# mario-linov/graphs4cfd

Hardware: AMD Instinct MI355X
Metric: rollout timesteps/s (100k-node 2D mesh) (higher is better)
Workload: dtype f32 (MLP products: two-way fp16 split of both operands, 22 significand bits each, 3 partial products on the f16 MFMA pipe, fp32 accumulate; error vs fp64 within that of an fp32 GEMM)

## Files before the change

graphs4cfd_amd/_lib.py:

```python
from __future__ import annotations

import ctypes as C
import os
from typing import Optional

import torch

_HERE = os.path.dirname(os.path.abspath(__file__))
LIB_PATH = os.environ.get("G4C_LIB_PATH") or os.path.join(_HERE, "lib", "libg4c.so")

OK, EINVAL, ELAUNCH, EUNSUPPORTED = 0, -1, -2, -3
ACT_NONE, ACT_SELU, ACT_TANH = 0, 1, 2
MAX_SRC, MAX_LAYERS = 4, 4
MAX_HEADS = 2
NARROW_MAX = 8
KERNEL_MLP_RS = 5
KERNEL_MLP_RS2 = 6
KERNEL_MLP_BX6, KERNEL_MLP_WS = 2, 4
KERNEL_MLP_BX6_CERT, KERNEL_MLP_WS_CERT = 7, 8
KERNEL_MLP_WS_PRE = 9
KERNEL_NAMES = {0: "none", 1: "mlp_split_kernel", 2: "mlp_bx6_kernel", 3: "mlp_bx6i_kernel", 4: "mlp_ws_kernel", 5: "mlp_rs1_kernel", 6: "mlp_rs2_kernel",
                7: "mlp_bx6_kernel", 8: "mlp_ws_kernel", 9: "mlp_ws_kernel"}

TILE_SHAPE_GENERIC, TILE_SHAPE_NODE, TILE_SHAPE_UP, TILE_SHAPE_DOWN = 0, 1, 2, 3

_ACT_CODES = {None: ACT_NONE, "none": ACT_NONE, "selu": ACT_SELU, "tanh": ACT_TANH}


def act_code(activation) -> Optional[int]:
    if activation is None or isinstance(activation, str):
        return _ACT_CODES[activation]
    if activation is torch.tanh or activation is torch.nn.functional.tanh:
        return ACT_TANH
    if activation is torch.nn.functional.selu or activation is torch.selu:
        return ACT_SELU
    return None


class g4c_src_t(C.Structure):
    _fields_ = [("ptr", C.c_void_p), ("idx", C.c_void_p), ("width", C.c_int32), ("ld", C.c_int32),
                ("col0", C.c_int32), ("pre_act", C.c_int32), ("additive", C.c_int32), ("seg_mean", C.c_int32),
                ("w", C.c_void_p), ("seg_off", C.c_void_p), ("seg_perm", C.c_void_p), ("dtype", C.c_int32)]


class g4c_mlp_t(C.Structure):
    _fields_ = [("n_layers", C.c_int32), ("k_pad", C.c_int32 * MAX_LAYERS), ("n_pad", C.c_int32 * MAX_LAYERS),
                ("w", C.c_void_p * MAX_LAYERS), ("b", C.c_void_p * MAX_LAYERS),
                ("ln_gamma", C.c_void_p), ("ln_beta", C.c_void_p), ("ln_eps", C.c_float), ("n_out", C.c_int32), ("w_format", C.c_int32),
                ("range_slot", C.c_int32), ("range_certified", C.c_int32)]


WFMT_FP32, WFMT_F16X2, WFMT_BF16X3, WFMT_BF16_RS, WFMT_BF16_RS2, WFMT_BF16_RS2N, WFMT_BF16 = 0, 1, 2, 3, 4, 5, 6
DTYPE_F32, DTYPE_BF16 = 0, 1


class g4c_mlp_io_t(C.Structure):
    _fields_ = [("size", C.c_int32), ("act", C.c_int32), ("row_begin", C.c_int64), ("row_count", C.c_int64),
                ("out", C.c_void_p), ("out_ld", C.c_int32), ("out_dtype", C.c_int32), ("out_idx", C.c_void_p),
                ("resid", C.c_void_p), ("resid_ld", C.c_int32), ("resid_col0", C.c_int32),
                ("n_heads", C.c_int32), ("head_ld", C.c_int32), ("head_dtype", C.c_int32), ("head_out", C.c_void_p * MAX_HEADS),
                ("tile_rows", C.c_void_p), ("tile_seg", C.c_void_p), ("seg_off", C.c_void_p), ("n_tiles", C.c_int32),
                ("agg", C.c_void_p), ("agg_ld", C.c_int32), ("agg_mode", C.c_int32),
                ("n_save", C.c_int32), ("save", C.c_void_p * MAX_LAYERS), ("save_ld", C.c_int32),
                ("mul", C.c_void_p * MAX_LAYERS), ("mul_ld", C.c_int32),
                ("upd", C.POINTER(g4c_mlp_t)), ("v", C.c_void_p), ("v_ld", C.c_int32), ("v_act", C.c_int32),
                ("v_out", C.c_void_p), ("v_out_ld", C.c_int32), ("range_flag", C.c_void_p),
                ("save_dtype", C.c_int32), ("mul_dtype", C.c_int32)]

    def __init__(self, **kw):
        super().__init__(size=C.sizeof(g4c_mlp_io_t), **kw)


REC_SQ_ERR, REC_ABS_ERR, REC_MAX_ABS_ERR, REC_TGT_SUM, REC_TGT_SQ_SUM, REC_ABS_ERR_MASK, REC_NSTAT = range(7)
REC_MAX_NF = 8


class g4c_rollout_rec_t(C.Structure):
    _fields_ = [("max_steps", C.c_int32), ("snap", C.c_void_p), ("every", C.c_int32), ("n_snap", C.c_int32),
                ("probe_rows", C.c_void_p), ("n_probe", C.c_int32), ("probe_out", C.c_void_p),
                ("target", C.c_void_p), ("target_ld", C.c_int32), ("mask", C.c_void_p), ("stats", C.c_void_p),
                ("scratch", C.c_void_p)]


class g4c_rollout_moments_t(C.Structure):
    _fields_ = [("max_steps", C.c_int32), ("stride", C.c_int32), ("window", C.c_void_p), ("sub", C.c_void_p), ("sub_ld", C.c_int32),
                ("plane_ld", C.c_int64), ("pivot", C.c_void_p), ("sum", C.c_void_p), ("sum2", C.c_void_p), ("lo", C.c_void_p),
                ("hi", C.c_void_p)]


SPECTRUM_MAX_BINS = 64


class g4c_rollout_spectrum_t(C.Structure):
    _fields_ = [("max_steps", C.c_int32), ("stride", C.c_int32), ("n_samples", C.c_int32), ("n_bins", C.c_int32), ("window", C.c_void_p),
                ("tw", C.c_void_p), ("x_ld", C.c_int32), ("x_step", C.c_int32), ("plane_ld", C.c_int64), ("pivot", C.c_void_p),
                ("sum", C.c_void_p), ("re", C.c_void_p), ("im", C.c_void_p)]


DERIVED_MAX_COLS, DERIVED_MAX_TERMS = 8, 3
DERIVED_SQ, DERIVED_ABS, DERIVED_MAX_ABS, DERIVED_NSTAT = range(4)


class g4c_derived_program_t(C.Structure):
    _fields_ = [("nd", C.c_int32), ("n_terms", C.c_int32 * DERIVED_MAX_COLS),
                ("field", (C.c_int32 * DERIVED_MAX_TERMS) * DERIVED_MAX_COLS), ("axis", (C.c_int32 * DERIVED_MAX_TERMS) * DERIVED_MAX_COLS),
                ("coef", (C.c_float * DERIVED_MAX_TERMS) * DERIVED_MAX_COLS)]


class g4c_mesh_derived_t(C.Structure):
    _fields_ = [("dim", C.c_int32), ("nf", C.c_int32), ("x_ld", C.c_int32), ("g", C.c_void_p), ("src", C.c_void_p), ("off", C.c_void_p),
                ("cur", C.c_void_p), ("step", C.c_void_p), ("every", C.c_int32), ("n_snap", C.c_int32), ("max_steps", C.c_int32),
                ("snap", C.c_void_p), ("stats", C.c_void_p), ("scratch", C.c_void_p)]


_SIGNATURES = {
    "g4c_version": (C.c_int, []),
    "g4c_device_info": (C.c_int, [C.c_void_p, C.POINTER(C.c_int32), C.POINTER(C.c_int32)]),
    "g4c_last_error": (C.c_char_p, []),
    "g4c_plan_csr": (C.c_int, [C.c_void_p, C.c_int64, C.c_int64, C.c_void_p, C.c_void_p]),
    "g4c_plan_pool_edge": (C.c_int64, [C.c_void_p, C.c_int64, C.c_void_p, C.c_int64, C.c_void_p, C.c_void_p,
                                       C.c_void_p, C.c_void_p]),
    "g4c_plan_pool_edge_ordered": (C.c_int64, [C.c_void_p, C.c_int64, C.c_void_p, C.c_int64, C.c_int32, C.c_void_p, C.c_void_p,
                                               C.c_void_p, C.c_void_p]),
    "g4c_segment_reduce": (C.c_int, [C.c_void_p, C.c_int32, C.c_void_p, C.c_void_p, C.c_int32, C.c_int32, C.c_int32,
                                     C.c_int32, C.c_int32, C.c_void_p, C.c_int32, C.c_void_p]),
    "g4c_weighted_segment_mean": (C.c_int, [C.c_void_p, C.c_int32, C.c_void_p, C.c_void_p, C.c_void_p, C.c_int32,
                                            C.c_int32, C.c_void_p, C.c_int32, C.c_void_p, C.c_void_p]),
    "g4c_mlp_pack_layer": (C.c_int, [C.c_void_p, C.c_int32, C.c_int32, C.c_void_p, C.c_void_p, C.c_int32, C.c_int32, C.c_void_p,
                                     C.c_int32, C.c_int32, C.c_void_p]),
    "g4c_mlp_run": (C.c_int, [C.POINTER(g4c_mlp_t), C.POINTER(g4c_src_t), C.c_int32, C.c_int64, C.POINTER(g4c_mlp_io_t), C.c_void_p]),
    "g4c_plan_tiles": (C.c_int64, [C.c_void_p, C.c_int32, C.c_int32, C.c_void_p, C.c_void_p, C.c_int64]),
    "g4c_mlp_bx6i_enable": (C.c_int, [C.c_int]),
    "g4c_mlp_ws_enable": (C.c_int, [C.c_int]),
    "g4c_mlp_small_launch_tiles": (C.c_int, [C.c_int]),
    "g4c_layer_norm": (C.c_int, [C.c_void_p, C.c_int32, C.c_int64, C.c_int32, C.c_void_p, C.c_void_p, C.c_float, C.c_int32, C.c_void_p, C.c_int32, C.c_void_p]),
    "g4c_debug_mean_div": (C.c_int, [C.c_void_p, C.c_void_p, C.c_void_p, C.c_int64, C.c_void_p]),
    "g4c_mlp_last_kernel": (C.c_int, []),
    "g4c_mlp_shapes_enable": (C.c_int, [C.c_int]),
    "g4c_mlp_last_shape": (C.c_int, []),
    "g4c_project_to_edges": (C.c_int, [C.c_void_p, C.c_int32, C.c_void_p, C.c_void_p, C.c_int64, C.c_int32,
                                       C.c_void_p, C.c_int32, C.c_void_p]),
    "g4c_edge_scalar_to_node_vector": (C.c_int, [C.c_void_p, C.c_int32, C.c_void_p, C.c_int32, C.c_int64, C.c_int32,
                                                 C.c_void_p, C.c_int32, C.c_void_p]),
    "g4c_knn_grid": (C.c_int, [C.c_void_p, C.c_void_p, C.c_void_p, C.c_void_p, C.c_int64, C.c_int32, C.c_void_p,
                               C.c_void_p, C.c_float, C.c_int32, C.c_void_p, C.c_void_p]),
    "g4c_knn_grid_query": (C.c_int, [C.c_void_p, C.c_void_p, C.c_void_p, C.c_int64, C.c_int32, C.c_void_p, C.c_void_p,
                                     C.c_float, C.c_void_p, C.c_void_p, C.c_int64, C.c_int32, C.c_void_p, C.c_void_p]),
    "g4c_rollout_advance": (C.c_int, [C.c_void_p, C.c_int32, C.c_void_p, C.c_int32, C.c_void_p, C.c_int32,
                                      C.c_void_p, C.c_int64, C.c_void_p]),
    "g4c_rollout_record_scratch_doubles": (C.c_int64, [C.c_int64, C.c_int32]),
    "g4c_rollout_advance_record": (C.c_int, [C.c_void_p, C.c_int32, C.c_void_p, C.c_int32, C.POINTER(g4c_rollout_rec_t),
                                             C.c_void_p, C.c_int64, C.c_void_p]),
    "g4c_rollout_moments": (C.c_int, [C.c_void_p, C.c_int32, C.POINTER(g4c_rollout_moments_t), C.c_void_p, C.c_int64, C.c_void_p]),
    "g4c_rollout_spectrum": (C.c_int, [C.c_void_p, C.c_int32, C.POINTER(g4c_rollout_spectrum_t), C.c_void_p, C.c_int64, C.c_void_p]),
    "g4c_mesh_gradient_weights": (C.c_int, [C.c_void_p, C.c_void_p, C.c_void_p, C.c_void_p, C.c_int32, C.c_int32, C.c_int64, C.c_int64,
                                            C.c_void_p, C.c_void_p, C.c_void_p, C.c_void_p]),
    "g4c_mesh_derived_scratch_doubles": (C.c_int64, [C.c_int64, C.c_int32]),
    "g4c_mesh_derived": (C.c_int, [C.c_void_p, C.POINTER(g4c_mesh_derived_t), C.POINTER(g4c_derived_program_t), C.c_int64, C.c_void_p]),
    "g4c_activation_inplace": (C.c_int, [C.c_void_p, C.c_int64, C.c_int32, C.c_void_p]),
    "g4c_add_cols": (C.c_int, [C.c_void_p, C.c_int32, C.c_int32, C.c_void_p, C.c_int32, C.c_void_p, C.c_int32,
                               C.c_int32, C.c_int64, C.c_void_p]),
    "g4c_copy_cols": (C.c_int, [C.c_void_p, C.c_int32, C.c_int32, C.c_void_p, C.c_void_p, C.c_int32, C.c_int32,
                                C.c_int32, C.c_int64, C.c_void_p]),
    "g4c_train_gather": (C.c_int, [C.c_void_p, C.c_int32, C.c_int32, C.c_void_p, C.c_int32, C.c_int32, C.c_void_p, C.c_int32,
                                   C.c_int32, C.c_int32, C.c_int64, C.c_int32, C.c_void_p]),
    "g4c_act_grad": (C.c_int, [C.c_void_p, C.c_int32, C.c_void_p, C.c_int32, C.c_int32, C.c_int32, C.c_void_p, C.c_int32,
                               C.c_int32, C.c_int64, C.c_void_p]),
    "g4c_act_grad_ref16": (C.c_int, [C.c_void_p, C.c_int32, C.c_void_p, C.c_int32, C.c_int32, C.c_int32, C.c_void_p, C.c_int32,
                                     C.c_int32, C.c_int64, C.c_void_p]),
    "g4c_layernorm_grad_partials": (C.c_int32, [C.c_int64]),
    "g4c_layernorm_grad": (C.c_int, [C.c_void_p, C.c_int32, C.c_void_p, C.c_void_p, C.c_int32, C.c_void_p, C.c_int32,
                                     C.c_void_p, C.c_int32, C.c_int64, C.c_float, C.c_void_p]),
    "g4c_layernorm_grad_z16": (C.c_int, [C.c_void_p, C.c_int32, C.c_void_p, C.c_void_p, C.c_int32, C.c_void_p, C.c_int32,
                                         C.c_void_p, C.c_int32, C.c_int64, C.c_float, C.c_void_p]),
    "g4c_colsum_partials": (C.c_int32, [C.c_int64]),
    "g4c_colsum": (C.c_int, [C.c_void_p, C.c_int32, C.c_int32, C.c_int64, C.c_void_p, C.c_void_p, C.c_void_p]),
    "g4c_weight_grad_partials": (C.c_int32, [C.c_int64]),
    "g4c_weight_grad_scratch_floats": (C.c_int64, [C.c_int64]),
    "g4c_weight_grad": (C.c_int, [C.c_void_p, C.c_int32, C.c_void_p, C.c_int32, C.c_int64, C.c_void_p, C.c_void_p, C.c_int32,
                                  C.c_void_p]),
    "g4c_weight_grad_bf16": (C.c_int, [C.c_void_p, C.c_int32, C.c_void_p, C.c_int32, C.c_int64, C.c_void_p, C.c_void_p, C.c_int32,
                                       C.c_void_p]),
    "g4c_weight_grad_bf16_a16": (C.c_int, [C.c_void_p, C.c_int32, C.c_void_p, C.c_int32, C.c_int64, C.c_void_p, C.c_void_p, C.c_int32,
                                           C.c_void_p]),
    "g4c_segment_broadcast": (C.c_int, [C.c_void_p, C.c_int32, C.c_void_p, C.c_void_p, C.c_int32, C.c_int32, C.c_int32,
                                        C.c_void_p, C.c_int32, C.c_void_p]),
}

EXPORTED_SYMBOLS = tuple(_SIGNATURES)

_lib = None


def load() -> C.CDLL:
    global _lib
    if _lib is None:
        if not os.path.exists(LIB_PATH):
            raise RuntimeError(
                f"graphs4cfd_amd: HIP library not found at {LIB_PATH}. Build it with "
                "`python -c 'import __graft_entry__ as g; g.build()'` (hipcc --offload-arch=gfx950). "
                "There is no CPU fallback.")
        lib = C.CDLL(LIB_PATH)
        for name, (res, args) in _SIGNATURES.items():
            fn = getattr(lib, name)
            fn.restype, fn.argtypes = res, args
        _lib = lib
    return _lib


def check(code: int) -> None:
    if code == OK:
        return
    msg = load().g4c_last_error().decode("utf-8", "replace")
    if code == EINVAL:
        raise ValueError(msg)
    if code == EUNSUPPORTED:
        raise NotImplementedError(msg)
    raise RuntimeError(msg)


# ... 22 lines not shown
```

graphs4cfd_amd/csrc/error.cpp:

```cpp
#include "g4c_common.h"
#include <atomic>

namespace g4c {
static thread_local char g_err[512] = "";

void set_error(const char *fmt, ...) {
    va_list ap;
    va_start(ap, fmt);
    vsnprintf(g_err, sizeof(g_err), fmt, ap);
    va_end(ap);
}

int visible_devices() {
    static const int n = [] {
        int c = 0;
        if (hipGetDeviceCount(&c) != hipSuccess) { (void)hipGetLastError(); c = 0; }
        return c;
    }();
    return n;
}

int cu_count() {
    constexpr int MAXD = 64;
    static std::atomic<int> cached[MAXD];
    int dev = 0;
    if (hipGetDevice(&dev) != hipSuccess) { (void)hipGetLastError(); return 256; }
    int n = (dev >= 0 && dev < MAXD) ? cached[dev].load(std::memory_order_relaxed) : 0;
    if (n > 0) return n;
    if (hipDeviceGetAttribute(&n, hipDeviceAttributeMultiprocessorCount, dev) != hipSuccess || n <= 0) { (void)hipGetLastError(); n = 256; }
    if (dev >= 0 && dev < MAXD) cached[dev].store(n, std::memory_order_relaxed);
    return n;
}
}

extern "C" int g4c_version(void) { return 3; }
extern "C" int g4c_device_info(const void *device_ptr, int32_t *device, int32_t *cu_count) {
    G4C_REQUIRE(device_ptr && device && cu_count, G4C_EINVAL, "g4c_device_info: null pointer");
    g4c::DeviceGuard on_device(device_ptr);
    int dev = -1;
    if (hipGetDevice(&dev) != hipSuccess) { (void)hipGetLastError(); g4c::set_error("g4c_device_info: hipGetDevice failed"); return G4C_ELAUNCH; }
    *device = dev;
    *cu_count = g4c::cu_count();
    return G4C_OK;
}
extern "C" const char *g4c_last_error(void) { return g4c::g_err; }
```

graphs4cfd_amd/csrc/g4c_common.h:

```cpp
#pragma once
#include <hip/hip_runtime.h>
#include <cstdarg>
#include <cstdio>
#include <cstdint>

#include "../../include/g4c.h"

namespace g4c {

void set_error(const char *fmt, ...);

inline int check_launch(const char *what) {
    hipError_t e = hipGetLastError();
    if (e != hipSuccess) {
        set_error("%s: %s", what, hipGetErrorString(e));
        return G4C_ELAUNCH;
    }
    return G4C_OK;
}

int visible_devices();
int cu_count();
struct DeviceGuard {
    int prev = -1;
    explicit DeviceGuard(const void *device_ptr) {
        if (visible_devices() <= 1 || !device_ptr) return;
        hipPointerAttribute_t attr;
        int cur = 0;
        if (hipPointerGetAttributes(&attr, device_ptr) != hipSuccess || hipGetDevice(&cur) != hipSuccess) {
            (void)hipGetLastError();
            return;
        }
        if (attr.device != cur && hipSetDevice(attr.device) == hipSuccess) prev = cur;
    }
    ~DeviceGuard() {
        if (prev >= 0) (void)hipSetDevice(prev);
    }
    DeviceGuard(const DeviceGuard &) = delete;
    DeviceGuard &operator=(const DeviceGuard &) = delete;
};

#define G4C_REQUIRE(cond, code, ...)      \
    do {                                  \
        if (!(cond)) {                    \
            g4c::set_error(__VA_ARGS__);  \
            return (code);                \
        }                                 \
    } while (0)

constexpr int MEAN_DIV_MAX_COUNT = 4096;
typedef float mean_f32x4 __attribute__((ext_vector_type(4)));
__device__ __forceinline__ mean_f32x4 mean_div4(mean_f32x4 a, int count) {
    const float c = (float)count;
    const float y0 = __builtin_amdgcn_rcpf(c);
    const float y = fmaf(fmaf(-c, y0, 1.f), y0, y0);
    mean_f32x4 q;
    bool rare = count > MEAN_DIV_MAX_COUNT;
#pragma unroll
    for (int e = 0; e < 4; ++e) {
        const float q0 = a[e] * y;
        q[e] = fmaf(fmaf(-c, q0, a[e]), y, q0);
        rare |= (__builtin_bit_cast(unsigned, a[e]) != 0u) && !(fabsf(q[e]) >= 0x1p-100f);
    }
    if (__builtin_amdgcn_ballot_w64(rare) != 0ull) {
#pragma unroll
        for (int e = 0; e < 4; ++e) q[e] = a[e] / c;
    }
    return q;
}

__device__ __forceinline__ float selu_f(float x) {
    const float alpha = 1.6732632423543772848170429916717f;
    const float scale = 1.0507009873554804934193349852946f;
    const float e = __builtin_amdgcn_fmed3f(__builtin_amdgcn_exp2f(x * 1.4426950408889634f), 0.f, 1.f);
    return fmaf(fmaxf(x, 0.f), scale, fmaf(scale * alpha, e, -scale * alpha));
}

__device__ __forceinline__ float tanh_f(float x) {
    const float ax = fminf(fabsf(x), 20.f);
    const float t = __builtin_amdgcn_exp2f(ax * 2.8853900817779268f);
    const float r = 1.f - 2.f * __builtin_amdgcn_rcpf(t + 1.f);
    return copysignf(r, x);
}

__device__ __forceinline__ float apply_act(float x, int act) {
    const float s = selu_f(x), t = tanh_f(x);
    return act == G4C_ACT_SELU ? s : (act == G4C_ACT_TANH ? t : x);
}

template <int ACT>
__device__ __forceinline__ float act_t(float x) {
    if (ACT == G4C_ACT_SELU) return selu_f(x);
    if (ACT == G4C_ACT_TANH) return tanh_f(x);
    return x;
}

}
```

graphs4cfd_amd/csrc/mlp_common.h:

```cpp
#pragma once
#include "g4c_common.h"
#include <type_traits>

#ifndef G4C_ABLATE
#define G4C_ABLATE 0
#endif

namespace g4cm {

constexpr int KC = 32;
constexpr int XS = KC + 2;
constexpr int HS = 128 + 4;
constexpr int NP = 128;
constexpr int CHUNK_FLOATS = KC * NP;

typedef float f32x16 __attribute__((ext_vector_type(16)));
typedef float f32x8 __attribute__((ext_vector_type(8)));
typedef float f32x4 __attribute__((ext_vector_type(4)));
typedef float f32x2 __attribute__((ext_vector_type(2)));

struct Src {
    const float *ptr;
    const int *idx;
    int width, wpad, ld, col0, vec, pre_act;
    const int *seg_off;
    int seg_mean;
    const int *seg_perm;
    int bf16;
};

struct NarSrc {
    const float *ptr;
    const float *w;
    int width, ld;
};

struct AddSrc {
    const float *ptr;
    const int *idx;
    int width, ld;
    int bf16;
};

struct Params {
    Src src[G4C_MAX_SRC];
    int n_src;
    AddSrc add[G4C_MAX_SRC];
    int n_add;
    int n_layers;
    int chunks0;
    const float *w;
    const float *b;
    const float *gamma, *beta;
    float eps;
    int n_out;
    long long M;
    float *out;
    int out_ld;
    int out_bf16;
    const int *out_idx;
    int act;
    const float *resid;
    int resid_ld, resid_col0;
    int n_tiles;
    long long row_base;
    int n_heads;
    float *head_out[G4C_MAX_HEADS];
    int head_ld;
    int head_bf16;
    const int *tile_rows, *tile_seg, *seg_off;
    float *agg;
    int agg_ld, agg_mean;
    int agg_deg;
    int agg_bf16;
    NarSrc nar[G4C_MAX_SRC];
    int n_nar;
    float *save[G4C_MAX_LAYERS];
    int save_ld;
    int save_bf16;
    const float *mul[G4C_MAX_LAYERS];
    int mul_ld;
    int mul_bf16;
    int *range_flag;
    int range_slot;
    int range_certified;
};

struct TileShapeGeneric {
    static constexpr int ID = G4C_TILE_SHAPE_GENERIC;
};
template <int ID_, int NS, bool IDX0_, int NNAR, int NL, int NH>
struct TileShape {
    static constexpr int ID = ID_, N_SRC = NS, N_NAR = NNAR, N_LAYERS = NL, N_HEADS = NH;
    static constexpr bool IDX0 = IDX0_;
    static_assert(ID_ != G4C_TILE_SHAPE_GENERIC && NS >= 1 && NS <= 2 && (NL == 2 || NL == 3) && (NH == 0 || NH == 2), "tile shape out of range");
};
template <int NL, int NH> using TileShapeNode = TileShape<G4C_TILE_SHAPE_NODE, 2, false, 0, NL, NH>;
template <int NL, int NH> using TileShapeUp = TileShape<G4C_TILE_SHAPE_UP, 2, true, 1, NL, NH>;
template <int NL> using TileShapeDown = TileShape<G4C_TILE_SHAPE_DOWN, 1, false, 1, NL, 0>;

struct NodeParams {
    const float *v;
    int v_ld;
    const float *w;
    const float *b;
    const float *gamma, *beta;
    float eps;
    int act;
    float *out;
    int out_ld;
    int n_heads;
    float *head_out[G4C_MAX_HEADS];
    int head_ld;
    int *range_flag;
    int range_slot;
};

typedef __bf16 bf16x8 __attribute__((ext_vector_type(8)));
typedef __bf16 bf16x4 __attribute__((ext_vector_type(4)));
constexpr int HB = 128 + 8;
constexpr int STEP6 = 3 * 512;
constexpr int BLOCK6 = 4 * 8 * STEP6;

typedef unsigned u32x4 __attribute__((ext_vector_type(4)));
__device__ __forceinline__ bf16x8 ldw(__amdgpu_buffer_rsrc_t rs, unsigned voff_bytes, unsigned soff_bytes) {
    const u32x4 v = __builtin_amdgcn_raw_buffer_load_b128(rs, voff_bytes, soff_bytes, 0);
    return __builtin_bit_cast(bf16x8, v);
}

__device__ __forceinline__ f32x4 selu4(f32x4 x) {
    f32x4 y;
#pragma unroll
    for (int e = 0; e < 4; ++e) y[e] = g4c::selu_f(x[e]);
    return y;
}
__device__ __forceinline__ f32x2 selu2(f32x2 x) {
    f32x2 y;
    y[0] = g4c::selu_f(x[0]); y[1] = g4c::selu_f(x[1]);
    return y;
}

typedef __bf16 bf16x2 __attribute__((ext_vector_type(2)));
__device__ __forceinline__ unsigned pack_bf16(f32x2 x, f32x2 &back) {
    bf16x2 b;
    b[0] = (__bf16)x[0]; b[1] = (__bf16)x[1];
    const unsigned u = __builtin_bit_cast(unsigned, b);
    back[0] = __builtin_bit_cast(float, u << 16);
    back[1] = __builtin_bit_cast(float, u & 0xffff0000u);
    return u;
}
typedef _Float16 f16x8 __attribute__((ext_vector_type(8)));
typedef _Float16 f16x2 __attribute__((ext_vector_type(2)));
constexpr float F16_LO_SCALE = 2048.f, F16_LO_UNSCALE = 1.f / 2048.f;
__device__ __forceinline__ f32x16 mfma_f16(bf16x8 a, bf16x8 b, f32x16 c) {
    return __builtin_amdgcn_mfma_f32_32x32x16_f16(__builtin_bit_cast(f16x8, a), __builtin_bit_cast(f16x8, b), c, 0, 0, 0);
}
#ifndef G4C_F16_SATURATE
// ... 44 lines not shown
        const float c = -F16_LO_SCALE;
        asm("v_fma_mixlo_f16 %0, %1, %2, %3 op_sel_hi:[1,0,0]" : "=v"(lu) : "v"(hu), "s"(c), "v"(ys[0]));
        asm("v_fma_mixhi_f16 %0, %1, %2, %3 op_sel:[1,0,0] op_sel_hi:[1,0,0]" : "+v"(lu) : "v"(hu), "s"(c), "v"(ys[1]));
    } else {
        f32x2 hf, lf;
        hf[0] = (float)b[0]; hf[1] = (float)b[1];
        lu = pack_f16((y - hf) * F16_LO_SCALE, lf);
    }
}
template <class R>
__device__ __forceinline__ void split_pair_f16(f32x2 y, unsigned &hu, unsigned &lu, R &rng) {
    range_track(rng, y);
    split_pair_f16(y, hu, lu);
}
template <class R>
__device__ __forceinline__ void split2x4(f32x4 x, bf16x4 &h, bf16x4 &l, R &rng) {
    range_track(rng, x);
    unsigned hu[2], lu[2];
#pragma unroll
    for (int j = 0; j < 2; ++j) {
        f32x2 v;
        v[0] = x[2 * j]; v[1] = x[2 * j + 1];
        split_pair_f16(v, hu[j], lu[j]);
    }
    typedef unsigned u32x2 __attribute__((ext_vector_type(2)));
    u32x2 hh, ll;
    hh[0] = hu[0]; hh[1] = hu[1]; ll[0] = lu[0]; ll[1] = lu[1];
    h = __builtin_bit_cast(bf16x4, hh); l = __builtin_bit_cast(bf16x4, ll);
}
__device__ __forceinline__ void split2(float x, __bf16 &h, __bf16 &l) {
    const _Float16 a = (_Float16)x;
    const _Float16 b = (_Float16)((x - (float)a) * F16_LO_SCALE);
    h = __builtin_bit_cast(__bf16, a); l = __builtin_bit_cast(__bf16, b);
}

template <int SP, class R> __device__ __forceinline__ void split3x4(f32x4 x, bf16x4 &h, bf16x4 &m, bf16x4 &l, R &rng);
template <int SP = 3>
__device__ __forceinline__ void split3x4(f32x4 x, bf16x4 &h, bf16x4 &m, bf16x4 &l) { RangeNone none; split3x4<SP>(x, h, m, l, none); }
template <int SP, class R>
__device__ __forceinline__ void split3x4(f32x4 x, bf16x4 &h, bf16x4 &m, bf16x4 &l, R &rng) {
    if (SP == 2) { split2x4(x, h, m, rng); l = m; return; }
    if (SP == 1 || (G4C_ABLATE & 512)) {
#pragma unroll
        for (int e = 0; e < 4; ++e) { h[e] = (__bf16)x[e]; m[e] = h[e]; l[e] = h[e]; }
        return;
    }
    unsigned hu[2], mu[2], lu[2];
#pragma unroll
    for (int j = 0; j < 2; ++j) {
        f32x2 v, hf, mf, lf;
        v[0] = x[2 * j]; v[1] = x[2 * j + 1];
        hu[j] = pack_bf16(v, hf);
        const f32x2 r1 = v - hf;
        mu[j] = pack_bf16(r1, mf);
        const f32x2 r2 = r1 - mf;
        lu[j] = pack_bf16(r2, lf);
    }
    typedef unsigned u32x2 __attribute__((ext_vector_type(2)));
    u32x2 hh, mm, ll;
    hh[0] = hu[0]; hh[1] = hu[1]; mm[0] = mu[0]; mm[1] = mu[1]; ll[0] = lu[0]; ll[1] = lu[1];
    h = __builtin_bit_cast(bf16x4, hh); m = __builtin_bit_cast(bf16x4, mm); l = __builtin_bit_cast(bf16x4, ll);
}

__device__ __forceinline__ void split3(float x, __bf16 &h, __bf16 &m, __bf16 &l) {
    h = (__bf16)x;
    const float r1 = x - (float)h;
    m = (__bf16)r1;
    l = (__bf16)(r1 - (float)m);
}

struct Launch {
    Params p;
    NodeParams node;
    bool has_node;
    int fmt;
    bool round1, f16x2, bx6, row_split;
    bool agg, save;
    bool pre;
    bool all_vec;
    long long row_begin, row_count;
    int io_n_tiles;
    bool deep_ring, shapes;
};
struct Ran { int kernel = G4C_KERNEL_NONE, shape = G4C_TILE_SHAPE_GENERIC; };

inline bool message_form(const Launch &L) {
    const Params &p = L.p;
    const Src &s = p.src[0];
    if (L.save || p.n_src != 1 || p.n_nar != 0 || (p.n_add != 0 && p.n_add != 2) || p.n_heads || p.n_out != NP || p.resid) return false;
    if (p.out_idx && (L.agg || !p.out)) return false;
    if (s.width != NP || !s.vec || s.seg_off) return false;
    for (int a = 0; a < p.n_add; ++a)
        if (p.add[a].width != NP || (p.add[a].ld & 3) || ((uintptr_t)p.add[a].ptr & (p.add[a].bf16 ? 7 : 15))) return false;
    if (p.out && !p.out_bf16 && ((p.out_ld & 3) || ((uintptr_t)p.out & 15))) return false;
    if (p.gamma && (((uintptr_t)p.gamma & 15) || ((uintptr_t)p.beta & 15))) return false;
    return ((uintptr_t)p.b & 15) == 0 && p.M < (1LL << 31);
}

bool split_takes(const Launch &L);
int split_launch(const Launch &L, hipStream_t st, Ran &ran);
bool tile_takes(const Launch &L);
int tile_launch(const Launch &L, hipStream_t st, Ran &ran);
bool bx6i_takes(const Launch &L);
int bx6i_launch(const Launch &L, hipStream_t st, Ran &ran);
bool ws_takes(const Launch &L);
bool ws_pre_takes(const Launch &L);
int ws_launch(const Launch &L, hipStream_t st, Ran &ran);
bool rs_takes(const Launch &L);
int rs_launch(const Launch &L, hipStream_t st, Ran &ran);
bool rs2_takes(const Launch &L);
int rs2_launch(const Launch &L, hipStream_t st, Ran &ran);

typedef unsigned u32x2 __attribute__((ext_vector_type(2)));
__device__ __forceinline__ f32x4 widen_bf16x4(u32x2 w) {
    f32x4 x;
    x[0] = __builtin_bit_cast(float, w[0] << 16); x[1] = __builtin_bit_cast(float, w[0] & 0xffff0000u);
    x[2] = __builtin_bit_cast(float, w[1] << 16); x[3] = __builtin_bit_cast(float, w[1] & 0xffff0000u);
    return x;
}


}
```

graphs4cfd_amd/csrc/mlp_run.hip:

```cpp
#include "mlp_common.h"
#include <atomic>
#include <climits>
using namespace g4cm;

namespace {

std::atomic<int> g_ws_mode{1};
std::atomic<int> g_bx6i_mode{1};
std::atomic<int> g_deep_tiles{512};
#ifndef G4C_TILE_SHAPES_DEFAULT
#define G4C_TILE_SHAPES_DEFAULT 1
#endif
std::atomic<int> g_shapes{G4C_TILE_SHAPES_DEFAULT};

constexpr long long WS_MIN_ROWS = 20000;
constexpr long long BX6I_MIN_ROWS = 400000;

int knob(std::atomic<int> &k, int value, int max_value) {
    const int prev = k.load(std::memory_order_relaxed);
    if (value >= 0) k.store(value > max_value ? max_value : value, std::memory_order_relaxed);
    return prev;
}

thread_local Ran g_last;

int stage_call(const g4c_mlp_t *mlp, const g4c_src_t *srcs, int32_t n_src, int64_t n_rows, const g4c_mlp_io_t *io, Launch &L) {
    G4C_REQUIRE(io && io->size == (int32_t)sizeof(g4c_mlp_io_t), G4C_EINVAL,
                "g4c_mlp_run: io->size %d, this library's g4c_mlp_io_t has %d bytes (a binding out of step with g4c.h)", io ? io->size : 0,
                (int)sizeof(g4c_mlp_io_t));
    G4C_REQUIRE(mlp && srcs, G4C_EINVAL, "g4c_mlp_run: null pointer");
    const int fmt = L.fmt = mlp->w_format;
    G4C_REQUIRE(fmt >= G4C_WFMT_FP32 && fmt <= G4C_WFMT_BF16, G4C_EINVAL, "g4c_mlp_run: unknown w_format %d", fmt);
    L.row_split = fmt == G4C_WFMT_BF16_RS || fmt == G4C_WFMT_BF16_RS2 || fmt == G4C_WFMT_BF16_RS2N;
    L.round1 = fmt == G4C_WFMT_BF16 || L.row_split;
    L.f16x2 = fmt == G4C_WFMT_F16X2;
    L.bx6 = fmt != G4C_WFMT_FP32;
    L.agg = io->agg != nullptr; L.save = io->n_save != 0; L.has_node = io->upd != nullptr;
    L.row_begin = io->row_begin; L.row_count = io->row_count; L.io_n_tiles = io->n_tiles;
    G4C_REQUIRE(L.row_begin >= 0 && L.row_count >= 0 && L.row_begin + L.row_count <= n_rows && L.row_begin % 32 == 0, G4C_EINVAL,
                "g4c_mlp_run: bad row range [%lld, +%lld) of %lld (row_begin must be a multiple of 32)", L.row_begin, L.row_count,
                (long long)n_rows);
    G4C_REQUIRE(n_src >= 1 && n_src <= G4C_MAX_SRC, G4C_EUNSUPPORTED, "g4c_mlp_run: %d sources (max %d)", n_src, G4C_MAX_SRC);
    G4C_REQUIRE(mlp->n_layers >= 1 && mlp->n_layers <= G4C_MAX_LAYERS, G4C_EUNSUPPORTED,
                "g4c_mlp_run: %d layers (supported 1..%d)", mlp->n_layers, G4C_MAX_LAYERS);
    G4C_REQUIRE(n_rows >= 0 && n_rows < (1LL << 31), G4C_EINVAL, "g4c_mlp_run: n_rows %lld out of range", (long long)n_rows);
    G4C_REQUIRE(io->act >= 0 && io->act <= 2, G4C_EINVAL, "g4c_mlp_run: bad activation %d", io->act);
    G4C_REQUIRE(io->n_heads >= 0 && io->n_heads <= G4C_MAX_HEADS, G4C_EINVAL, "g4c_mlp_run: bad heads (n=%d)", io->n_heads);
    G4C_REQUIRE((L.row_begin == 0 && L.row_count == n_rows) || (!L.agg && !L.save && !L.has_node && !io->n_heads && !io->out_dtype),
                G4C_EUNSUPPORTED, "g4c_mlp_run: a row sub-range needs a plain launch (no heads / aggregation / save / upd / out_dtype)");
    G4C_REQUIRE(!L.agg || (io->tile_rows && io->tile_seg && io->seg_off && io->n_tiles >= 0 && io->agg_ld >= NP), G4C_EINVAL,
                "g4c_mlp_run: bad aggregation plan");
    G4C_REQUIRE(io->out_dtype == G4C_DTYPE_F32 || io->out_dtype == G4C_DTYPE_BF16 || io->out_dtype == G4C_DTYPE_BF16_SELU, G4C_EINVAL,
                "g4c_mlp_run: unknown out_dtype %d", io->out_dtype);
    G4C_REQUIRE(io->out_dtype != G4C_DTYPE_BF16_SELU || (L.agg && io->act == G4C_ACT_NONE), G4C_EINVAL,
                "g4c_mlp_run: G4C_DTYPE_BF16_SELU needs the fused aggregation and no output activation");
    G4C_REQUIRE(io->head_dtype == G4C_DTYPE_F32 || io->head_dtype == G4C_DTYPE_BF16, G4C_EINVAL, "g4c_mlp_run: unknown head_dtype %d", io->head_dtype);
    G4C_REQUIRE(!io->range_flag || (mlp->range_slot >= 0 && (!L.has_node || io->upd->range_slot >= 0)), G4C_EINVAL,
                "g4c_mlp_run: negative range_slot (mlp %d, upd %d)", mlp->range_slot, L.has_node ? io->upd->range_slot : 0);
    return G4C_OK;
}

int stage_sources(const g4c_src_t *srcs, int32_t n_src, int32_t k_pad0, Launch &L) {
    Params &p = L.p;
    const bool bx6 = L.bx6, round1 = L.round1;
    int kp = 0, nk = 0;
    L.all_vec = true;
    for (int s = 0; s < n_src; ++s) {
        const g4c_src_t &g = srcs[s];
        G4C_REQUIRE(g.ptr && g.width > 0 && g.ld >= g.col0 + g.width && g.col0 >= 0, G4C_EINVAL,
                    "g4c_mlp_run: bad source %d (width=%d ld=%d col0=%d)", s, g.width, g.ld, g.col0);
        if (g.additive == 2) {
            G4C_REQUIRE(bx6, G4C_EUNSUPPORTED, "g4c_mlp_run: narrow sources (additive == 2) need a split-operand w_format");
            G4C_REQUIRE(g.width <= G4C_NARROW_MAX && !g.idx && g.pre_act == G4C_ACT_NONE && g.w && ((uintptr_t)g.w & 15) == 0, G4C_EINVAL,
                        "g4c_mlp_run: bad narrow source %d (width %d <= %d, no index, no pre_act, 16-byte aligned weights)", s,
                        g.width, G4C_NARROW_MAX);
            NarSrc &a = p.nar[p.n_nar++];
            a.ptr = g.ptr + g.col0; a.w = g.w; a.width = g.width; a.ld = g.ld;
            continue;
        }
        if (g.additive) {
            G4C_REQUIRE(g.pre_act == G4C_ACT_NONE && g.width <= NP && (g.dtype == G4C_DTYPE_F32 || g.dtype == G4C_DTYPE_BF16), G4C_EINVAL,
                        "g4c_mlp_run: bad additive source %d", s);
            AddSrc &a = p.add[p.n_add++];
            a.idx = g.idx; a.width = g.width; a.ld = g.ld; a.bf16 = g.dtype == G4C_DTYPE_BF16;
            if (a.bf16) {
                G4C_REQUIRE(round1 && g.width == NP && g.ld % 4 == 0 && g.col0 % 4 == 0 && (uintptr_t)g.ptr % 8 == 0, G4C_EUNSUPPORTED,
                            "g4c_mlp_run: bf16 additive rows need the rounded-bf16 mode (w_format G4C_WFMT_BF16*) and a 128-wide, 8-byte aligned block");
                a.ptr = reinterpret_cast<const float *>(reinterpret_cast<const __bf16 *>(g.ptr) + g.col0);
            } else {
                a.ptr = g.ptr + g.col0;
            }
            continue;
        }
        G4C_REQUIRE(g.pre_act == G4C_ACT_NONE || g.pre_act == G4C_ACT_SELU, G4C_EUNSUPPORTED,
                    "g4c_mlp_run: source %d pre_act %d (only NONE / SELU can be applied on load)", s, g.pre_act);
        Src &d = p.src[nk++];
        if (bx6) G4C_REQUIRE(g.width <= NP, G4C_EUNSUPPORTED, "g4c_mlp_run: input block %d is %d wide (max 128 in a split-operand w_format)", s, g.width);
        d.ptr = g.ptr; d.idx = g.idx; d.width = g.width; d.wpad = bx6 ? NP : (g.width + KC - 1) / KC * KC; d.ld = g.ld; d.col0 = g.col0;
        d.pre_act = g.pre_act;
        d.bf16 = g.dtype == G4C_DTYPE_BF16;
        if (d.bf16)
            G4C_REQUIRE(round1 && g.width == NP && !g.seg_off && g.ld % 4 == 0 && g.col0 % 4 == 0 && (uintptr_t)g.ptr % 8 == 0, G4C_EUNSUPPORTED,
                        "g4c_mlp_run: bf16 rows need the rounded-bf16 mode (w_format G4C_WFMT_BF16*) and a 128-wide, 8-byte aligned block");
        else
            G4C_REQUIRE(g.dtype == G4C_DTYPE_F32, G4C_EINVAL, "g4c_mlp_run: source %d has unknown dtype %d", s, g.dtype);
        d.seg_off = g.seg_off; d.seg_mean = g.seg_mean; d.seg_perm = g.seg_off ? g.seg_perm : nullptr;
        if (g.seg_off)
            G4C_REQUIRE(bx6 && !g.idx && g.width == NP && g.ld % 4 == 0 && g.col0 % 4 == 0 && (uintptr_t)g.ptr % 16 == 0, G4C_EUNSUPPORTED,
                        "g4c_mlp_run: aggregation on load needs a split-operand w_format and a 128-wide aligned block without gather index");
        d.vec = (g.width % 4 == 0) && (g.ld % 4 == 0) && (g.col0 % 4 == 0) && ((uintptr_t)g.ptr % (d.bf16 ? 8 : 16) == 0);
        L.all_vec = L.all_vec && d.vec;
        kp += d.wpad;
    }
    L.pre = nk == 0 && p.n_nar == 0 && p.n_add >= 1;
    G4C_REQUIRE(nk >= 1 || p.n_nar >= 1 || L.pre, G4C_EINVAL, "g4c_mlp_run: no input block goes through the weights");
    p.n_src = nk;
    if (nk == 0) p.src[0] = Src{nullptr, nullptr, 0, 0, 0, 0, 1, 0, nullptr, 0, nullptr, 0};
    for (int s = (nk ? nk : 1); s < G4C_MAX_SRC; ++s) p.src[s] = p.src[0];
    G4C_REQUIRE(kp == k_pad0, G4C_EINVAL, "g4c_mlp_run: sources give %d padded columns, layer 1 packed for %d", kp, k_pad0);
    p.chunks0 = kp / KC;
    return G4C_OK;
}

int check_contiguous(const g4c_mlp_t *m, int wbytes, const char *w_text, const char *b_text) {
    for (int l = 1; l < m->n_layers; ++l) {
        G4C_REQUIRE((const char *)m->w[l] == (const char *)m->w[l - 1] + (size_t)m->k_pad[l - 1] * NP * wbytes, G4C_EINVAL, w_text, l);
        G4C_REQUIRE((const float *)m->b[l] == (const float *)m->b[l - 1] + NP, G4C_EINVAL, b_text, l);
    }
    return G4C_OK;
}

int stage_stream(const g4c_mlp_t *mlp, Launch &L) {
    Params &p = L.p;
    p.n_layers = mlp->n_layers;
    for (int l = 0; l < mlp->n_layers; ++l) {
        G4C_REQUIRE(mlp->n_pad[l] == NP, G4C_EINVAL, "g4c_mlp_run: layer %d n_pad %d (must be 128)", l, mlp->n_pad[l]);
        if (l > 0) G4C_REQUIRE(mlp->k_pad[l] == NP, G4C_EINVAL, "g4c_mlp_run: layer %d k_pad %d (must be 128)", l, mlp->k_pad[l]);
    }
    if (const int rc = check_contiguous(mlp, L.bx6 ? 6 : 4, "g4c_mlp_run: packed layers must be contiguous (layer %d)",
                                        "g4c_mlp_run: padded biases must be contiguous (layer %d)"))
        return rc;
    p.w = (const float *)mlp->w[0]; p.b = (const float *)mlp->b[0];
    G4C_REQUIRE(p.w && p.b, G4C_EINVAL, "g4c_mlp_run: null weights");
    p.gamma = mlp->ln_gamma; p.beta = mlp->ln_beta; p.eps = mlp->ln_eps;
    G4C_REQUIRE((p.gamma == nullptr) == (p.beta == nullptr), G4C_EINVAL, "g4c_mlp_run: LayerNorm needs both gamma and beta");
    p.n_out = mlp->n_out;
    return G4C_OK;
}

int stage_outputs(const g4c_mlp_io_t *io, Launch &L) {
    Params &p = L.p;
    p.out = (float *)io->out; p.out_ld = io->out_ld; p.out_idx = io->out_idx; p.act = io->act;
    G4C_REQUIRE(p.out || L.agg, G4C_EINVAL, "g4c_mlp_run: null output");
    G4C_REQUIRE(p.n_out > 0 && p.n_out <= NP && p.out_ld >= p.n_out, G4C_EINVAL, "g4c_mlp_run: n_out=%d out_ld=%d", p.n_out, p.out_ld);
    p.resid = io->resid; p.resid_ld = io->resid_ld; p.resid_col0 = io->resid_col0;
    p.row_base = L.row_begin;
    p.M = L.row_begin + L.row_count;
    if (L.agg) {
        G4C_REQUIRE(L.bx6 && p.n_out == NP && !p.out_idx && !p.resid, G4C_EUNSUPPORTED,
                    "g4c_mlp_run: the fused aggregation needs a split-operand w_format and a plain 128-wide output");
        const int32_t mode = io->agg_mode;
        p.tile_rows = io->tile_rows; p.tile_seg = io->tile_seg; p.seg_off = io->seg_off;
        p.agg = (float *)io->agg; p.agg_ld = io->agg_ld; p.agg_mean = mode & 1; p.agg_deg = (mode >> 8) & 0xff; p.agg_bf16 = (mode >> 16) & 1;
        const bool rs_fmt = L.fmt == G4C_WFMT_BF16_RS;
        G4C_REQUIRE((mode >> 17) == 0 && (!p.agg_bf16 || rs_fmt) && p.agg_deg <= 32 && (p.agg_deg == 0 || L.row_count % p.agg_deg == 0), G4C_EINVAL,
                    "fused aggregation: agg_mode = %d is not 0 / 1 [| G4C_AGG_UNIFORM(k), 1 <= k <= 32, k dividing the %lld rows]", mode,
                    L.row_count);
        G4C_REQUIRE(p.agg_deg == 0 || L.row_begin == 0, G4C_EINVAL,
                    "g4c_mlp_run: uniform segments (G4C_AGG_UNIFORM) need the whole row range, got rows [%lld, %lld)", L.row_begin, p.M);
    }
    if (io->out_dtype) {
        G4C_REQUIRE(L.round1 && !p.resid && !p.out_idx && p.n_out == NP && (!p.out || ((p.out_ld & 3) == 0 && ((uintptr_t)p.out & 7) == 0)), G4C_EUNSUPPORTED,
                    "g4c_mlp_run: bf16 output rows need the rounded-bf16 mode, a plain 128-wide output, out_ld a multiple of 4 and an 8-byte aligned out");
        p.out_bf16 = io->out_dtype;
    }
    return G4C_OK;
}

int stage_save(const g4c_mlp_io_t *io, Launch &L) {
    Params &p = L.p;
    const int n_layers = p.n_layers;
    if (!L.save) return G4C_OK;
    G4C_REQUIRE(L.bx6 && (!L.round1 || L.fmt == G4C_WFMT_BF16) && !io->out_dtype && !L.agg && !io->n_heads && !p.out_idx && io->save_ld >= NP &&
                    (io->save_ld & 3) == 0,
                G4C_EUNSUPPORTED,
                "g4c_mlp_run: save needs w_format BF16X3 / F16X2 / BF16 without heads / aggregation / output index / bf16 rows, save_ld >= 128 "
                "and a multiple of 4");
    G4C_REQUIRE(io->n_save == n_layers, G4C_EINVAL, "g4c_mlp_run: n_save %d for %d layers", io->n_save, n_layers);
    G4C_REQUIRE((io->save_dtype == G4C_DTYPE_F32 || io->save_dtype == G4C_DTYPE_BF16) &&
                    (io->mul_dtype == G4C_DTYPE_F32 || io->mul_dtype == G4C_DTYPE_BF16),
                G4C_EINVAL, "g4c_mlp_run: save_dtype %d / mul_dtype %d (G4C_DTYPE_F32 or G4C_DTYPE_BF16)", io->save_dtype, io->mul_dtype);
    G4C_REQUIRE((!io->save_dtype && !io->mul_dtype) || L.fmt == G4C_WFMT_BF16, G4C_EINVAL,
                "g4c_mlp_run: bf16 save / mul rows need w_format G4C_WFMT_BF16 (the plain rounded-bf16 stream); w_format %d keeps fp32 rows",
                L.fmt);
    bool mul = false;
    for (int l = 0; l < n_layers; ++l) {
        G4C_REQUIRE(((uintptr_t)io->save[l] & 15) == 0, G4C_EINVAL, "g4c_mlp_run: save[%d] is not 16-byte aligned", l);
        p.save[l] = static_cast<float *>(io->save[l]);
        if (l + 1 == n_layers) break;
        G4C_REQUIRE(((uintptr_t)io->mul[l] & 15) == 0, G4C_EINVAL, "g4c_mlp_run: mul[%d] is not 16-byte aligned", l);
        p.mul[l] = static_cast<const float *>(io->mul[l]);
        mul = mul || io->mul[l];
    }
    p.save_bf16 = io->save_dtype == G4C_DTYPE_BF16;
    p.mul_bf16 = io->mul_dtype == G4C_DTYPE_BF16;
    p.save_ld = io->save_ld;
    G4C_REQUIRE(!mul || (io->mul_ld >= NP && (io->mul_ld & 3) == 0), G4C_EINVAL, "g4c_mlp_run: mul_ld=%d", io->mul_ld);
    p.mul_ld = io->mul_ld;
    return G4C_OK;
}

void stage_range(const g4c_mlp_t *mlp, const g4c_mlp_io_t *io, Launch &L) {
    L.p.range_certified = (L.f16x2 && mlp->range_certified && !L.save && (!L.has_node || io->upd->range_certified)) ? 1 : 0;
    L.p.range_flag = (L.f16x2 && !L.p.range_certified) ? io->range_flag : nullptr;
    L.p.range_slot = mlp->range_slot;
}

int stage_heads(const g4c_mlp_io_t *io, Launch &L) {
    Params &p = L.p;
    const int n_heads = io->n_heads;
    for (int hd = 0; hd < n_heads; ++hd) G4C_REQUIRE(io->head_out[hd], G4C_EINVAL, "g4c_mlp_run: null head output %d", hd);
    if (L.has_node || !n_heads) return G4C_OK;
    p.n_heads = n_heads; p.head_ld = io->head_ld;
    for (int hd = 0; hd < n_heads; ++hd) p.head_out[hd] = (float *)io->head_out[hd];
    if (io->head_dtype) {
        G4C_REQUIRE(L.round1 && (p.head_ld & 1) == 0, G4C_EUNSUPPORTED, "g4c_mlp_run: bf16 head rows need the rounded-bf16 mode and an even head_ld");
        for (int hd = 0; hd < n_heads; ++hd)
            G4C_REQUIRE(((uintptr_t)io->head_out[hd] & 3) == 0, G4C_EINVAL, "g4c_mlp_run: head output %d is not 4-byte aligned", hd);
        p.head_bf16 = 1;
    }
    G4C_REQUIRE(!L.agg, G4C_EUNSUPPORTED, "g4c_mlp_run: heads with the fused aggregation");
    G4C_REQUIRE((p.head_ld & 3) == 0 || !L.bx6, G4C_EINVAL, "g4c_mlp_run: head outputs need a leading dimension that is a multiple of 4");
    G4C_REQUIRE(p.n_out == NP && !p.resid && !p.out_idx && p.head_ld >= NP, G4C_EINVAL,
                "g4c_mlp_run: heads need a 128-wide output without residual / output index (n_out=%d)", p.n_out);
    return G4C_OK;
}

int stage_node(const g4c_mlp_io_t *io, Launch &L) {
    if (!L.has_node) return G4C_OK;
    const g4c_mlp_t *u = io->upd;
    const int n_heads = io->n_heads;
    G4C_REQUIRE(L.f16x2 && L.agg && u->w_format == G4C_WFMT_F16X2 && io->act == G4C_ACT_NONE, G4C_EUNSUPPORTED,
                "g4c_mlp_run: the fused node update needs the f16x3 format (G4C_WFMT_F16X2) for both MLPs, the aggregation plan and act NONE");
    G4C_REQUIRE(u->n_layers == L.p.n_layers && u->k_pad[0] == 2 * NP && u->n_out == NP && u->w[0] && u->b[0], G4C_EUNSUPPORTED,
                "g4c_mlp_run: upd must have the message MLP's depth (%d), two 128-wide input blocks and a 128-wide output", L.p.n_layers);
    for (int l = 0; l < u->n_layers; ++l)
        G4C_REQUIRE(u->n_pad[l] == NP && (l == 0 || u->k_pad[l] == NP), G4C_EUNSUPPORTED, "g4c_mlp_run: upd layer %d is not 128 wide", l);
    const char *const text = "g4c_mlp_run: upd's packed layers / biases must be contiguous (layer %d)";
    if (const int rc = check_contiguous(u, 6, text, text)) return rc;
    G4C_REQUIRE((u->ln_gamma == nullptr) == (u->ln_beta == nullptr), G4C_EINVAL, "g4c_mlp_run: upd's LayerNorm needs both gamma and beta");
    G4C_REQUIRE(!u->ln_gamma || (((uintptr_t)u->ln_gamma & 15) == 0 && ((uintptr_t)u->ln_beta & 15) == 0), G4C_EINVAL,
                "g4c_mlp_run: upd's LayerNorm parameters must be 16-byte aligned");
    G4C_REQUIRE(io->v && io->v_out && (io->v_ld & 3) == 0 && io->v_ld >= NP && (io->v_out_ld & 3) == 0 && io->v_out_ld >= NP &&
                ((uintptr_t)io->v & 15) == 0 && ((uintptr_t)io->v_out & 15) == 0 && (io->agg_ld & 3) == 0 && ((uintptr_t)io->agg & 15) == 0,
                G4C_EINVAL, "g4c_mlp_run: v / v_out / agg need 16-byte aligned rows of at least 128 columns");
    G4C_REQUIRE(io->v_act >= 0 && io->v_act <= 2, G4C_EINVAL, "g4c_mlp_run: bad v_act %d", io->v_act);
    NodeParams &q = L.node;
    q.v = io->v; q.v_ld = io->v_ld; q.w = (const float *)u->w[0]; q.b = (const float *)u->b[0];
    q.gamma = u->ln_gamma; q.beta = u->ln_beta; q.eps = u->ln_eps; q.act = io->v_act;
    q.out = io->v_out; q.out_ld = io->v_out_ld; q.n_heads = n_heads; q.head_ld = io->head_ld;
    q.range_flag = L.p.range_certified ? nullptr : io->range_flag; q.range_slot = u->range_slot;
    if (n_heads) {
        G4C_REQUIRE(io->head_dtype == G4C_DTYPE_F32 && (io->head_ld & 3) == 0 && io->head_ld >= NP, G4C_EINVAL,
                    "g4c_mlp_run: upd's heads need fp32 rows, head_ld a multiple of 4 and >= 128");
        for (int hd = 0; hd < n_heads; ++hd) {
            G4C_REQUIRE(((uintptr_t)io->head_out[hd] & 15) == 0, G4C_EINVAL, "g4c_mlp_run: bad head output %d", hd);
            q.head_out[hd] = (float *)io->head_out[hd];
        }
    }
    return G4C_OK;
}

typedef int (*LaunchFn)(const Launch &, hipStream_t, Ran &);

bool at_size(const std::atomic<int> &mode_knob, long long min_rows, const Launch &L) {
    const int mode = mode_knob.load(std::memory_order_relaxed);
    return mode == 2 || (mode == 1 && L.row_count >= min_rows);
}

LaunchFn choose(Launch &L) {
    L.deep_ring = L.p.n_tiles <= g_deep_tiles.load(std::memory_order_relaxed);
    L.shapes = g_shapes.load(std::memory_order_relaxed) != 0;
    if (L.pre) {
        G4C_REQUIRE(!L.has_node, nullptr, "g4c_mlp_run: every source additive (first layer precomputed) with upd: the fused MP layer has no such form");
        G4C_REQUIRE(L.f16x2, nullptr, "g4c_mlp_run: every source additive (first layer precomputed) needs the f16x3 format (G4C_WFMT_F16X2), got w_format %d", L.fmt);
        G4C_REQUIRE(L.p.n_layers == 3, nullptr, "g4c_mlp_run: every source additive (first layer precomputed) needs three layers (two left), got %d", L.p.n_layers);
        G4C_REQUIRE(L.agg && !L.save, nullptr, "g4c_mlp_run: every source additive (first layer precomputed) needs the fused aggregation and no save");
        G4C_REQUIRE(ws_pre_takes(L), nullptr,
                    "g4c_mlp_run: every source additive (first layer precomputed) is outside the weight-stationary kernel's envelope (three aligned "
                    "128-wide fp32 additive blocks — the first direct, two through indices —, a plain fp32 128-wide output, no heads / residual "
                    "/ output index / out_dtype)");
        return ws_launch;
    }
    if (L.has_node) {
        G4C_REQUIRE(ws_takes(L), nullptr,
                    "g4c_mlp_run: the message launch of the fused MP layer is outside the weight-stationary kernel's envelope (one 128-wide "
                    "weighted block, two 128-wide additive blocks, two or three 128-wide layers, aligned rows)");
        return ws_launch;
    }
    if (L.fmt == G4C_WFMT_BF16_RS) {
        G4C_REQUIRE(!L.save && rs_takes(L), nullptr,
                    "g4c_mlp_run: weights packed for the row-split kernel (G4C_WFMT_BF16_RS), launch outside its envelope");
        return rs_launch;
    }
    if (L.row_split) {
        G4C_REQUIRE(!L.save && !L.agg && rs2_takes(L), nullptr,
                    "g4c_mlp_run: weights packed for the row-split update kernel (G4C_WFMT_BF16_RS2), launch outside its envelope");
        return rs2_launch;
    }
    if (at_size(g_ws_mode, WS_MIN_ROWS, L) && ws_takes(L)) return ws_launch;
    if (at_size(g_bx6i_mode, BX6I_MIN_ROWS, L) && bx6i_takes(L)) return bx6i_launch;
    return tile_takes(L) ? tile_launch : split_launch;
}

}

extern "C" int g4c_mlp_run(const g4c_mlp_t *mlp, const g4c_src_t *srcs, int32_t n_src, int64_t n_rows, const g4c_mlp_io_t *io,
                           void *stream) {
    g_last = Ran{};
    Launch L{};
    int rc;
    if ((rc = stage_call(mlp, srcs, n_src, n_rows, io, L))) return rc;
    if (n_rows == 0) return G4C_OK;
    g4c::DeviceGuard on_device(mlp->w[0]);
    if ((rc = stage_sources(srcs, n_src, mlp->k_pad[0], L))) return rc;
    if ((rc = stage_stream(mlp, L))) return rc;
    if ((rc = stage_outputs(io, L))) return rc;
    if ((rc = stage_save(io, L))) return rc;
    stage_range(mlp, io, L);
    if ((rc = stage_heads(io, L))) return rc;
    if (L.row_count == 0) return G4C_OK;
    if ((rc = stage_node(io, L))) return rc;
    L.p.n_tiles = (L.agg && !L.row_split) ? L.io_n_tiles : (int)((L.row_count + 31) / 32);
    const LaunchFn launch = choose(L);
    if (!launch) return G4C_EUNSUPPORTED;
    if (L.p.n_tiles == 0) return G4C_OK;
    return launch(L, (hipStream_t)stream, g_last);
}

extern "C" int g4c_mlp_ws_enable(int on) { return knob(g_ws_mode, on, 2); }
extern "C" int g4c_mlp_bx6i_enable(int on) { return knob(g_bx6i_mode, on, 2); }
extern "C" int g4c_mlp_small_launch_tiles(int n_tiles) { return knob(g_deep_tiles, n_tiles, INT_MAX); }
extern "C" int g4c_mlp_shapes_enable(int on) { return knob(g_shapes, on, 1); }
extern "C" int g4c_mlp_last_kernel(void) { return g_last.kernel; }
extern "C" int g4c_mlp_last_shape(void) { return g_last.shape; }
```

graphs4cfd_amd/csrc/mlp_ws.hip:

```cpp
#include "mlp_common.h"
#include <cstdlib>
using namespace g4cm;

#ifdef G4C_WS_TIMING
__device__ unsigned long long g4c_ws_stamps[256 * 32];
extern "C" int g4c_ws_read_stamps(unsigned long long *host, int n) {
    return (int)hipMemcpyFromSymbol(host, HIP_SYMBOL(g4c_ws_stamps), sizeof(unsigned long long) * n);
}
#define WS_STAMP(k) do { if (it == 1 && tid == 0 && blockIdx.x < 256) g4c_ws_stamps[blockIdx.x * 32 + (k)] = __builtin_readcyclecounter(); } while (0)
#define WS_STAMP_T(k) do { if (its == 1 && tid == 0 && blockIdx.x < 256) { asm volatile("s_waitcnt lgkmcnt(0)" ::: "memory"); g4c_ws_stamps[blockIdx.x * 32 + (k)] = __builtin_readcyclecounter(); } } while (0)
#define WS_STAMP_ONCE(k, v) do { if (tid == 0 && blockIdx.x < 256) g4c_ws_stamps[blockIdx.x * 32 + (k)] = (v); } while (0)
#else
#define WS_STAMP(k) do {} while (0)
#define WS_STAMP_T(k) do {} while (0)
#define WS_STAMP_ONCE(k, v) do {} while (0)
#endif

#ifndef G4C_WS_ABLATE
#define G4C_WS_ABLATE 0
#endif

namespace {

constexpr int PS = 128;
// ... 386 lines not shown
                    __syncthreads();
                    store_head(1, fB, r0 + 32, nB);
                } else {
                    other_all<SP, 3, false>(accB, accB1, va, oB, rngN);
                    __syncthreads();
                    store_head(0, fB, r0 + 32, nB);
                }
            }
            __syncthreads();
            continue;
        }
        other_all<SP, 2, false>(accA, accA1, ga, oA, rngN);
        other_all<SP, 2, false>(accA, accA1, va, oB, rngN);
        bias_n(accA, accA1, 0);
        __syncthreads();
        m_block<SP, 0>(paA, Wa, accA, accA1, accA, accA1, ga, oA, rngN);
        ld_block(Wa, 2);
        m_block<SP, 0>(paB, Wb, accA, accA1, accA, accA1, ga, oA, rngN);
        ld_block(Wb, 3);
        __syncthreads();
        other_all<SP, 1, false>(accA, accA1, ga, oA, rngN);
        bias_n(accA, accA1, 1);
        __syncthreads();
        m_block<SP, 0>(paA, Wa, accA, accA1, accA, accA1, ga, oA, rngN);
        if constexpr (NL == 3) {
            ld_block(Wa, 4);
            other_all<SP, 1, false>(accA, accA1, ga, oB, rngN);
            bias_n(accA, accA1, 2);
            __syncthreads();
            m_block<SP, 0>(paB, Wb, accA, accA1, accA, accA1, ga, oA, rngN);
            ld_block(Wb, 5);
        } else {
            ld_block(Wa, 4);
        }
        other_all<SP, 3, false>(accA, accA1, ga, oA, rngN);
        __syncthreads();
        finish_rows(fA, r0, nr);
        if (q.n_heads) {
            __syncthreads();
            f32x4 xh[2];
#pragma unroll
            for (int hh = 0; hh < 2; ++hh) xh[hh] = *reinterpret_cast<const f32x4 *>(fA + (prow + 16 * hh) * HS + pc);
            other_all<SP, 2, false>(accA, accA1, xh, oA, rngN);
            bias_n(accA, accA1, -1);
            bias_n(accB, accB1, -1);
            __syncthreads();
            m_block<SP, 0>(paA, H0, accA, accA1, accA, accA1, ga, oA, rngN);
            if (q.n_heads > 1) m_block<SP, 0>(paA, H1, accB, accB1, accA, accA1, ga, oA, rngN);
            other_all<SP, 3, false>(accA, accA1, ga, oB, rngN);
            other_all<SP, 3, false>(accB, accB1, ga, oA, rngN);
            __syncthreads();
            store_head(0, fB, r0, nr);
            if (q.n_heads > 1) store_head(1, fA, r0, nr);
        }
        __syncthreads();
    }
    if constexpr (TRACK) {
        if (G4C_WS_SCALED && !(G4C_WS_ABLATE & 48)) rngN.m *= F16_LO_UNSCALE;
        if (q.range_flag && range_hit(rngN)) {
            if ((threadIdx.x & 63) == 0) q.range_flag[q.range_slot] = 1;
        }
    }
}

struct WsArgs {
    const float *x;
    const int *x_idx;
    int x_ld, x_pact;
    const float *add_ptr[2];
    const int *add_idx[2];
    int add_ld[2];
    const float *w, *b, *gamma, *beta;
    float eps;
    int act;
    float *out;
    const int *out_idx;
    int out_ld, out_bf16;
    const int *tile_rows, *tile_seg, *seg_off;
    float *agg;
    int agg_ld, agg_mean, agg_deg;
    int M, row_base, n_tiles;
    int *range_flag;
    int range_slot;
};
struct WsKernArgs {
    WsArgs a;
    int n_pairs;
    NodeParams q;
};
__device__ __forceinline__ NodeParams node_params_now() {
    typedef const WsKernArgs __attribute__((address_space(4))) *KernArgPtr;
    KernArgPtr k = (KernArgPtr)__builtin_amdgcn_kernarg_segment_ptr();
    asm volatile("" : "+s"(k));
    NodeParams q;
    q.v = k->q.v; q.v_ld = k->q.v_ld; q.w = k->q.w; q.b = k->q.b; q.gamma = k->q.gamma; q.beta = k->q.beta; q.eps = k->q.eps; q.act = k->q.act;
    q.out = k->q.out; q.out_ld = k->q.out_ld; q.n_heads = k->q.n_heads; q.head_ld = k->q.head_ld;
#pragma unroll
    for (int hd = 0; hd < G4C_MAX_HEADS; ++hd) q.head_out[hd] = k->q.head_out[hd];
    q.range_flag = k->q.range_flag; q.range_slot = k->q.range_slot;
    return q;
}
__device__ __forceinline__ int *range_word_now() {
    typedef const WsKernArgs __attribute__((address_space(4))) *KernArgPtr;
    KernArgPtr k = (KernArgPtr)__builtin_amdgcn_kernarg_segment_ptr();
    asm volatile("" : "+s"(k));
    int *const flag = k->a.range_flag;
    return flag ? flag + k->a.range_slot : nullptr;
}

constexpr int G4C_WS_SP1_MINW = 2;
template <bool AGG, bool DIRECT, bool ADDS, int SP, int NL, bool XB16, bool AB16, bool NODE, bool DENSE, bool TRACK, bool PRE>
__device__ __forceinline__ void ws_body(const WsKernArgs &ka) {
    const WsArgs &p = ka.a;
    const int n_pairs = ka.n_pairs;
    static_assert((SP == 1 || SP == 2) && (NL == 2 || NL == 3) && (SP == 1 || !XB16) && (SP == 1 || !AB16) && (ADDS || !AB16) &&
                  (!NODE || (AGG && SP == 2)) && (TRACK || SP == 2), "mlp_ws_kernel: unsupported instantiation");
    static_assert(!PRE || (AGG && DIRECT && ADDS && SP == 2 && NL == 3 && !NODE && TRACK), "mlp_ws_pre_kernel: unsupported instantiation");
    typedef typename std::conditional<AB16, u32x2, f32x4>::type AddV;
    __shared__ __attribute__((aligned(16))) __bf16 sP[2 * TILE_BF16];
    __shared__ __attribute__((aligned(16))) float sF[2 * FIN];
    __shared__ int sIdx[2][2 * 3 * 32];
    __shared__ int sSeg[4][2 * (SEGCAP + 1)];
    __shared__ __attribute__((aligned(16))) float sBias[3 * NP];
    __shared__ __attribute__((aligned(16))) float sGB[2 * NP];
    __shared__ __attribute__((aligned(16))) float sZero[NP];
    __shared__ __attribute__((aligned(16))) float sCarry[NP];
    __shared__ __attribute__((aligned(16))) float sBiasN[NODE ? 3 * NP : 4];
    __shared__ __attribute__((aligned(16))) float sGBN[NODE ? 2 * NP : 4];

    const int tid = threadIdx.x, lane = tid & 63;
    const int wave = __builtin_amdgcn_readfirstlane(tid >> 6);
    const int n = lane & 15, g = lane >> 4;
    const int fcol = 16 * wave + 4 * g;
    const int prow = tid >> 5, pc = (tid & 31) * 4;

    static_assert((AGG || !DENSE) && !(NODE && DENSE), "dense pairs belong to the fused aggregation of a plain message launch");
    const int KU = DENSE ? p.agg_deg : 0;
    int p_begin, p_end, R0 = 0, R1 = 0;
    {
        const int G = gridDim.x, b = blockIdx.x;
        const int slot = (G & 7) ? b : (b & 7) * (G >> 3) + (b >> 3);
        if constexpr (DENSE) {
            const int n_seg = p.M / KU;
            R0 = __builtin_amdgcn_readfirstlane((int)(((long long)slot * n_seg) / G) * KU);
            R1 = __builtin_amdgcn_readfirstlane((int)(((long long)(slot + 1) * n_seg) / G) * KU);
            p_begin = 0; p_end = (R1 - R0 + 63) >> 6;
        } else {
            p_begin = __builtin_amdgcn_readfirstlane((int)(((long long)slot * n_pairs) / G));
            p_end = __builtin_amdgcn_readfirstlane((int)(((long long)(slot + 1) * n_pairs) / G));
        }
    }
    if (p_begin >= p_end) return;
    WS_STAMP_ONCE(12, __builtin_readcyclecounter());
    WS_STAMP_ONCE(14, (unsigned long long)(p_end - p_begin));

    auto load_meta = [&](int pair) __attribute__((always_inline)) {
        Meta m;
        if constexpr (DENSE) {
            if (pair > p_end - 1) pair = p_end - 1;
            const int r0 = R0 + 64 * pair, nr = (R1 - r0) < 64 ? (R1 - r0) : 64;
            m.r0[0] = r0; m.n[0] = nr < 32 ? nr : 32; m.r0[1] = r0 + 32; m.n[1] = nr - m.n[0];
            m.s0[0] = m.s1[0] = m.s0[1] = m.s1[1] = 0;
            if (m.n[1] == 0) m.r0[1] = m.r0[0];
            return m;
        }
        if (pair > n_pairs - 1) pair = n_pairs - 1;
        const int t0 = 2 * pair;
        if (AGG) {
            const int t1 = t0 + 1 < p.n_tiles ? t0 + 1 : p.n_tiles, t2 = t0 + 2 < p.n_tiles ? t0 + 2 : p.n_tiles;
            const int r0 = p.tile_rows[t0], r1 = p.tile_rows[t1], r2 = p.tile_rows[t2];
            const int q0 = p.tile_seg[t0], q1 = p.tile_seg[t1], q2 = p.tile_seg[t2];
            m.r0[0] = r0; m.n[0] = r1 - r0; m.r0[1] = r1; m.n[1] = r2 - r1;
            m.s0[0] = q0; m.s1[0] = q1; m.s0[1] = q1; m.s1[1] = q2;
        } else {
#pragma unroll
            for (int t = 0; t < 2; ++t) {
                const int tile = t0 + t;
                m.s0[t] = 0; m.s1[t] = 0;
                if (tile >= p.n_tiles) { m.r0[t] = 0; m.n[t] = 0; }
                else { m.r0[t] = p.row_base + tile * 32; const int lim = p.M - m.r0[t]; m.n[t] = lim < 32 ? lim : 32; }
            }
        }
        if (m.n[1] == 0) m.r0[1] = m.r0[0];
        return m;
    };
    auto fix_meta = [&](const Meta &r) __attribute__((always_inline)) {
        Meta m;
#pragma unroll
        for (int t = 0; t < 2; ++t) {
            m.r0[t] = __builtin_amdgcn_readfirstlane(r.r0[t]); m.n[t] = __builtin_amdgcn_readfirstlane(r.n[t]);
            m.s0[t] = __builtin_amdgcn_readfirstlane(r.s0[t]); m.s1[t] = __builtin_amdgcn_readfirstlane(r.s1[t]);
        }
        return m;
    };
    const int *const dummy = reinterpret_cast<const int *>(p.x);
    auto load_tables = [&](const Meta &m) __attribute__((always_inline)) {
        const int *ix0 = DIRECT ? nullptr : p.x_idx, *ix1 = ADDS ? p.add_idx[0] : nullptr, *ix2 = ADDS ? p.add_idx[1] : nullptr;
        const int tt = tid < 192 ? tid : 0;
        const int t = tt / 96, k = (tt % 96) >> 5, r = tt & 31;
        const int nn = m.n[t] > 0 ? m.n[t] : m.n[0];
        const int gr = m.r0[t] + (r < nn ? r : nn - 1);
        const int *ix = (k == 0) ? ix0 : (k == 1 ? ix1 : ix2);
        const int *addr = ix ? ix + gr : dummy;
        int j = 0, ts = 0;
        if (AGG && !DENSE) {
            const int q = tid - 256;
            const bool is_seg = q >= 0 && q < 2 * (SEGCAP + 1);
            ts = is_seg && q >= SEGCAP + 1 ? 1 : 0;
            j = is_seg ? q - ts * (SEGCAP + 1) : 0;
            int sg = m.s0[ts] + j;
            if (sg > m.s1[ts]) sg = m.s1[ts];
            if (is_seg) addr = p.seg_off + sg;
        }
        const int v = *addr;
        return (tid < 192 && !ix) ? gr : v;
    };
    auto store_tables = [&](int v, int it) __attribute__((always_inline)) {
        if (tid < 192) sIdx[it & 1][tid] = v;
        if (AGG && !DENSE && tid >= 256 && tid < 256 + 2 * (SEGCAP + 1)) sSeg[it & 3][tid - 256] = v;
    };
    auto gather_x = [&](const Meta &m, int ring, int t, f32x4 (&xt)[2], unsigned (&raw)[2][2]) __attribute__((always_inline)) {
        {
            const int nn = m.n[t] > 0 ? m.n[t] : m.n[0];
#pragma unroll
            for (int hh = 0; hh < 2; ++hh) {
                const int r = prow + 16 * hh;
                const int gr = DIRECT ? m.r0[t] + (r < nn ? r : nn - 1) : sIdx[ring][t * 96 + r];
                if constexpr (XB16) {
                    typedef unsigned u32x2 __attribute__((ext_vector_type(2)));
                    const u32x2 w = *reinterpret_cast<const u32x2 *>(reinterpret_cast<const __bf16 *>(p.x) + (long long)gr * p.x_ld + pc);
                    raw[hh][0] = w[0]; raw[hh][1] = w[1];
                } else
                xt[hh] = *reinterpret_cast<const f32x4 *>(p.x + (long long)gr * p.x_ld + pc);
            }
        }
    };
    auto widen_x = [&](f32x4 (&xt)[2], const unsigned (&raw)[2][2]) __attribute__((always_inline)) {
        if constexpr (XB16) {
#pragma unroll
            for (int hh = 0; hh < 2; ++hh) {
                xt[hh][0] = __builtin_bit_cast(float, raw[hh][0] << 16); xt[hh][1] = __builtin_bit_cast(float, raw[hh][0] & 0xffff0000u);
                xt[hh][2] = __builtin_bit_cast(float, raw[hh][1] << 16); xt[hh][3] = __builtin_bit_cast(float, raw[hh][1] & 0xffff0000u);
            }
        }
    };
    auto gather_adds = [&](int t, int ring, AddV (&ad)[2][2]) __attribute__((always_inline)) {
        if (ADDS) {
#pragma unroll
            for (int rb = 0; rb < 2; ++rb) {
                const int r = n + 16 * rb;
                if constexpr (AB16) {
                    ad[rb][0] = *reinterpret_cast<const u32x2 *>(reinterpret_cast<const __bf16 *>(p.add_ptr[0]) + (long long)sIdx[ring][t * 96 + 32 + r] * p.add_ld[0] + fcol);
                    ad[rb][1] = *reinterpret_cast<const u32x2 *>(reinterpret_cast<const __bf16 *>(p.add_ptr[1]) + (long long)sIdx[ring][t * 96 + 64 + r] * p.add_ld[1] + fcol);
                } else {
                    ad[rb][0] = *reinterpret_cast<const f32x4 *>(p.add_ptr[0] + (long long)sIdx[ring][t * 96 + 32 + r] * p.add_ld[0] + fcol);
                    ad[rb][1] = *reinterpret_cast<const f32x4 *>(p.add_ptr[1] + (long long)sIdx[ring][t * 96 + 64 + r] * p.add_ld[1] + fcol);
                }
            }
        }
    };

    const __amdgpu_buffer_rsrc_t rs = __builtin_amdgcn_make_buffer_rsrc(const_cast<float *>(p.w), 0, 0x7fffffff, 0x00020000);
    const unsigned lo_b = 2u * (unsigned)((wave >> 1) * 8 * STEP6 + (g >> 1) * STEP6 + ((g & 1) * 32 + 16 * (wave & 1) + n) * 8);
    bf16x8 W[NL][4][SP];
    if (SP == 2) f16_range_mode();
    typename std::conditional<TRACK, RangeV, RangeNone>::type rng;

    Meta m0 = fix_meta(load_meta(p_begin)), m1 = fix_meta(load_meta(p_begin + 1)), m2 = fix_meta(load_meta(p_begin + 2));
    auto meta_at = [&](int pair_, const Meta &carried) __attribute__((always_inline)) {
        if constexpr (DENSE) { asm volatile("" : "+s"(pair_)); return load_meta(pair_); }
        else return carried;
    };
    {
        const int v0 = load_tables(m0), v1 = load_tables(m1);
        store_tables(v0, 0);
        store_tables(v1, 1);
    }
#pragma unroll
    for (int l = PRE ? 1 : 0; l < NL; ++l)
#pragma unroll
        for (int ks = 0; ks < 4; ++ks)
#pragma unroll
            for (int pl = 0; pl < SP; ++pl) W[l][ks][pl] = ldw(rs, lo_b + 1024u * pl, (unsigned)(l - (PRE ? 1 : 0)) * 2u * BLOCK6 + (unsigned)ks * 4u * STEP6);
    if (tid < NL * NP) sBias[tid] = p.b[tid];
    if (tid < NP) sZero[tid] = 0.f;
    if (tid < 2 * NP) sGB[tid] = p.gamma ? (tid < NP ? p.gamma[tid] : p.beta[tid - NP]) : 0.f;
    if constexpr (NODE) {
        const NodeParams &q = ka.q;
        if (tid < NL * NP) sBiasN[tid] = q.b[tid];
        if (tid < 2 * NP) sGBN[tid] = q.gamma ? (tid < NP ? q.gamma[tid] : q.beta[tid - NP]) : 0.f;
    }
    __syncthreads();

    const bool pact = p.x_pact != 0;
    __bf16 *const sA = sP, *const sB = sP + TILE_BF16;
    float *const fA = sF, *const fB = sF + FIN;
    Other oA, oB;
    {
        const int l32 = tid & 31;
        const int acc_off = n * PS + 8 * ((2 * wave + (g >> 1)) ^ n) + 4 * (g & 1);
        const int park_off = prow * PS + 8 * ((l32 >> 1) ^ prow) + 4 * (l32 & 1);
        oA.plane_acc = sA + acc_off; oA.plane_park = sA + park_off; oA.fin = fA + n * HS + fcol;
        oB.plane_acc = sB + acc_off; oB.plane_park = sB + park_off; oB.fin = fB + n * HS + fcol;
    }
    const __bf16 *paA[4], *paB[4];
#pragma unroll
    for (int ks = 0; ks < 4; ++ks) { paA[ks] = sA + n * PS + 8 * ((4 * ks + g) ^ n); paB[ks] = paA[ks] + TILE_BF16; }

    f32x4 accA[2], accB[2], accA1[2], accB1[2];
    f32x4 xr[2][2];
    auto bias_init = [&](f32x4 (&acc)[2], f32x4 (&acc1)[2], int l) __attribute__((always_inline)) {
        const f32x4 b4 = *reinterpret_cast<const f32x4 *>(sBias + l * NP + fcol);
        acc[0] = b4; acc[1] = b4;
        acc1[0] = f32x4{0.f, 0.f, 0.f, 0.f}; acc1[1] = f32x4{0.f, 0.f, 0.f, 0.f};
    };
    auto start_values = [&](f32x4 (&acc)[2], f32x4 (&acc1)[2], const AddV (&a)[2][2]) __attribute__((always_inline)) {
        bias_init(acc, acc1, 0);
        if (ADDS) {
#pragma unroll
            for (int rb = 0; rb < 2; ++rb) {
                f32x4 a0, a1;
                if constexpr (AB16) { a0 = widen_bf16x4(a[rb][0]); a1 = widen_bf16x4(a[rb][1]); }
                else { a0 = a[rb][0]; a1 = a[rb][1]; }
#pragma unroll
                for (int e = 0; e < 4; ++e) acc[rb][e] = (acc[rb][e] + a0[e]) + a1[e];
            }
        }
    };
    auto gather_t = [&](const Meta &m, int t, f32x4 (&tv)[2]) __attribute__((always_inline)) {
        const int nn = m.n[t] > 0 ? m.n[t] : m.n[0];
#pragma unroll
        for (int rb = 0; rb < 2; ++rb) {
            const int r = n + 16 * rb;
            tv[rb] = *reinterpret_cast<const f32x4 *>(p.x + (long long)(m.r0[t] + (r < nn ? r : nn - 1)) * p.x_ld + fcol);
        }
    };
    auto start_values_pre = [&](f32x4 (&sv)[2], const f32x4 (&tv)[2], const AddV (&a)[2][2]) __attribute__((always_inline)) {
        if constexpr (PRE) {
#pragma unroll
            for (int rb = 0; rb < 2; ++rb)
#pragma unroll
                for (int e = 0; e < 4; ++e) sv[rb][e] = (tv[rb][e] + a[rb][0][e]) + a[rb][1][e];
        }
    };
    auto ln_tail = [&](const Meta &mm, const int its) __attribute__((always_inline)) {
        {
            const int row = wave * 4 + g;
            constexpr bool rows16 = SP == 1;
            const int cq[2] = {rows16 ? n * 8 : n * 4, rows16 ? n * 8 + 4 : 64 + n * 4};
            float *const rowp[2] = {fA + row * HS, fB + row * HS};
            float x[2][8];
#pragma unroll
            for (int t = 0; t < 2; ++t)
#pragma unroll
                for (int c = 0; c < 8; c += 4) {
                    const f32x4 v = *reinterpret_cast<const f32x4 *>(rowp[t] + cq[c >> 2]);
                    x[t][c] = v[0]; x[t][c + 1] = v[1]; x[t][c + 2] = v[2]; x[t][c + 3] = v[3];
                }
            WS_STAMP_T(17);
            if (p.gamma) {
                float sum[2], mean[2], var[2], rstd[2];
#pragma unroll
                for (int t = 0; t < 2; ++t) {
                    sum[t] = 0.f;
#pragma unroll
                    for (int c = 0; c < 8; ++c) sum[t] += x[t][c];
                }
                row16_sum2(sum[0], sum[1]);
#pragma unroll
// ... 55 lines not shown
            const int c4 = (tid & 31) * 4;
            const int *sg_tab = sSeg[itp & 3];
            const int nsA = mm.s1[0] - mm.s0[0], nsB = mm.s1[1] - mm.s0[1];
            auto reduce_rows = [&](const float *sH, int b, int e, int sg) __attribute__((always_inline)) {
                f32x4 a = {0.f, 0.f, 0.f, 0.f};
                WS_STAMP_T(20);
                for (int r0 = b; r0 < e; r0 += 8) {
                    f32x4 v[8];
                    if constexpr (SP == 1) {
#pragma unroll
                        for (int u = 0; u < 8; ++u) v[u] = *reinterpret_cast<const f32x4 *>((r0 + u < e ? sH + __umul24((unsigned)(r0 + u), (unsigned)HS) : sZero) + c4);
#pragma unroll
                        for (int u = 0; u < 8; ++u)
#pragma unroll
                            for (int el = 0; el < 4; ++el) a[el] += v[u][el];
                    } else {
#pragma unroll
                        for (int u = 0; u < 8; ++u) v[u] = *reinterpret_cast<const f32x4 *>(sH + (r0 + u < e ? r0 + u : e - 1) * HS + c4);
#pragma unroll
                        for (int u = 0; u < 8; ++u) {
                            const bool on = r0 + u < e;
#pragma unroll
                            for (int el = 0; el < 4; ++el) a[el] += on ? v[u][el] : 0.f;
                        }
                    }
                }
                WS_STAMP_T(21);
                if (p.agg_mean) {
                    if (G4C_WS_MEAN_DIV) {
                        a = g4c::mean_div4(a, (e - b) > 1 ? (e - b) : 1);
                    } else {
                        const float cnt = (float)((e - b) > 1 ? (e - b) : 1);
#pragma unroll
                        for (int el = 0; el < 4; ++el) a[el] /= cnt;
                    }
                }
                WS_STAMP_T(22);
                *reinterpret_cast<f32x4 *>(p.agg + (long long)sg * p.agg_ld + c4) = a;
            };
            auto reduce_uniform = [&](auto KC) __attribute__((always_inline)) {
                constexpr int K = decltype(KC)::value;
                constexpr float cK = (float)K, yK = 1.0f / (float)K;
                const int r0 = mm.r0[0], nr = mm.n[0] + mm.n[1], j0 = (int)((unsigned)r0 / (unsigned)K);
                const int lead = (j0 * K < r0) ? (j0 * K + K - r0) : 0;
                const int nfull = (nr - lead) / K, rest = nr - lead - nfull * K;
                const int jf = j0 + (lead ? 1 : 0);
                auto mean4 = [&](f32x4 a) __attribute__((always_inline)) {
                    if (p.agg_mean) {
#pragma unroll
                        for (int el = 0; el < 4; ++el) {
                            const float q0 = a[el] * yK;
                            a[el] = fmaf(fmaf(-cK, q0, a[el]), yK, q0);
                        }
                    }
                    return a;
                };
                for (int q = tid >> 5; q < nfull; q += 16) {
                    const float *base = fA + __umul24((unsigned)(lead + q * K), (unsigned)HS) + c4;
                    f32x4 v[K];
                    WS_STAMP_T(20);
#pragma unroll
                    for (int u = 0; u < K; ++u) v[u] = *reinterpret_cast<const f32x4 *>(base + u * HS);
                    f32x4 a = {0.f, 0.f, 0.f, 0.f};
#pragma unroll
                    for (int u = 0; u < K; ++u) a += v[u];
                    WS_STAMP_T(21);
                    a = mean4(a);
                    WS_STAMP_T(22);
                    *reinterpret_cast<f32x4 *>(p.agg + (long long)(jf + q) * p.agg_ld + c4) = a;
                }
                if (wave == 7 && (lead | rest)) {
                    const bool hi = lane >= 32;
                    const int b = hi ? nr - rest : 0, cnt = hi ? rest : lead;
                    f32x4 v[K - 1];
#pragma unroll
                    for (int u = 0; u < K - 1; ++u) v[u] = *reinterpret_cast<const f32x4 *>((u < cnt ? fA + __umul24((unsigned)(b + u), (unsigned)HS) : sZero) + c4);
                    f32x4 a = *reinterpret_cast<const f32x4 *>((hi || !lead ? sZero : sCarry) + c4);
#pragma unroll
                    for (int u = 0; u < K - 1; ++u) a += v[u];
                    if (!hi && lead) *reinterpret_cast<f32x4 *>(p.agg + (long long)j0 * p.agg_ld + c4) = mean4(a);
                    if (hi && rest) *reinterpret_cast<f32x4 *>(sCarry + c4) = a;
                }
            };
            if constexpr (DENSE) {
                typedef std::integral_constant<int, 4> K4; typedef std::integral_constant<int, 5> K5; typedef std::integral_constant<int, 6> K6;
                typedef std::integral_constant<int, 7> K7; typedef std::integral_constant<int, 8> K8;
                if (KU == 6) reduce_uniform(K6{});
                else if (KU == 5) reduce_uniform(K5{});
                else if (KU == 4) reduce_uniform(K4{});
                else if (KU == 7) reduce_uniform(K7{});
                else reduce_uniform(K8{});
                return;
            }
            for (int q = tid >> 5; q < nsA + nsB; q += 16) {
                const int t = q >= nsA ? 1 : 0, j = q - (t ? nsA : 0);
                if (j < SEGCAP) {
                    const int b = sg_tab[t * (SEGCAP + 1) + j] - mm.r0[t], e = sg_tab[t * (SEGCAP + 1) + j + 1] - mm.r0[t];
                    reduce_rows(t ? fB : fA, b, e, mm.s0[t] + j);
                }
            }
            if (nsA > SEGCAP || nsB > SEGCAP) {
                for (int q = tid >> 5; q < nsA + nsB; q += 16) {
                    const int t = q >= nsA ? 1 : 0, j = q - (t ? nsA : 0);
                    if (j >= SEGCAP) {
                        const int sg = mm.s0[t] + j;
                        reduce_rows(t ? fB : fA, p.seg_off[sg] - mm.r0[t], p.seg_off[sg + 1] - mm.r0[t], sg);
                    }
                }
            }
    };
    AddV adB[2][2];
    unsigned rawB[2][2] = {{0u, 0u}, {0u, 0u}};
    if constexpr (PRE) {
        AddV adA[2][2];
        f32x4 tA[2], tB[2], sA0[2];
        gather_t(m0, 0, tA);
        gather_t(m0, 1, tB);
        gather_adds(0, 0, adA);
        gather_adds(1, 0, adB);
        start_values_pre(sA0, tA, adA);
        other_all<SP, 5, false>(accA, accA1, sA0, oA, rng);
        start_values_pre(accB, tB, adB);
    } else {
        AddV adA[2][2];
        unsigned rawA[2][2] = {{0u, 0u}, {0u, 0u}};
        gather_x(m0, 0, 0, xr[0], rawA);
        gather_x(m0, 0, 1, xr[1], rawB);
        gather_adds(0, 0, adA);
        gather_adds(1, 0, adB);
        widen_x(xr[0], rawA);
        if (pact) other_all<SP, 2, true>(accA, accA1, xr[0], oA, rng);
        else other_all<SP, 2, false>(accA, accA1, xr[0], oA, rng);
        start_values(accA, accA1, adA);
    }
    __syncthreads();

    if constexpr (PRE) {
        for (int it = 0, pair = p_begin; pair < p_end; ++pair, ++it) {
            WS_STAMP(0);
            Meta m3raw;
            if constexpr (!DENSE) m3raw = load_meta(pair + 3);
            const int tv = load_tables(meta_at(pair + 2, m2));
            f32x4 ntA[2], ntB[2], nsA[2];
            AddV nadA[2][2];
            WS_STAMP(1);
            bias_init(accA, accA1, 1);
            gather_t(meta_at(pair + 1, m1), 0, ntA);
            m_block<SP, 5>(paA, W[1], accA, accA1, accA, accA1, accB, oB, rng);
            bias_init(accB, accB1, 1);
            __syncthreads();
            WS_STAMP(2);
            gather_adds(0, (it + 1) & 1, nadA);
            m_block<SP, 1>(paB, W[1], accB, accB1, accA, accA1, ntA, oA, rng);
            bias_init(accA, accA1, 2);
            __syncthreads();
            WS_STAMP(3);
            gather_t(meta_at(pair + 1, m1), 1, ntB);
            m_block<SP, 1>(paA, W[2], accA, accA1, accB, accB1, ntA, oB, rng);
            bias_init(accB, accB1, 2);
            __syncthreads();
            WS_STAMP(4);
            start_values_pre(nsA, ntA, nadA);
            gather_adds(1, (it + 1) & 1, adB);
            m_block<SP, 6>(paB, W[2], accB, accB1, accA, accA1, nsA, oA, rng);
            other_all<SP, 3, false>(accB, accB1, nsA, oB, rng);
            __syncthreads();
            WS_STAMP(7);
            start_values_pre(accB, ntB, adB);
            asm volatile("" : "+v"(accB[0]), "+v"(accB[1]) :: "memory");
            Meta m3;
            if constexpr (!DENSE) m3 = fix_meta(m3raw);
            store_tables(tv, it + 2);
            WS_STAMP(8);
            if (!(G4C_WS_ABLATE & 256)) ln_tail(meta_at(pair, m0), it);
            WS_STAMP(9);
            __syncthreads();
            WS_STAMP(15);
            if (!(G4C_WS_ABLATE & 128)) agg_tail(meta_at(pair, m0), it);
            WS_STAMP(10);
            if constexpr (!DENSE) { m0 = m1; m1 = m2; m2 = m3; }
        }
    } else
    for (int it = 0, pair = p_begin; pair < p_end; ++pair, ++it) {
        WS_STAMP(0);
        Meta m3raw;
        if constexpr (!DENSE) m3raw = load_meta(pair + 3);
        const int tv = load_tables(meta_at(pair + 2, m2));
        WS_STAMP(1);
        widen_x(xr[1], rawB);
        if (pact) m_block<SP, 2, true>(paA, W[0], accA, accA1, accA, accA1, xr[1], oB, rng);
        else m_block<SP, 2, false>(paA, W[0], accA, accA1, accA, accA1, xr[1], oB, rng);
        start_values(accB, accB1, adB);
        __syncthreads();
        WS_STAMP(2);
        f32x4 nxa[2];
        AddV nadA[2][2];
        unsigned nraw[2][2] = {{0u, 0u}, {0u, 0u}};
        gather_x(meta_at(pair + 1, m1), (it + 1) & 1, 0, nxa, nraw);
        m_block<SP, 1>(paB, W[0], accB, accB1, accA, accA1, xr[1], oA, rng);
        bias_init(accA, accA1, 1);
        __syncthreads();
        WS_STAMP(3);
        gather_adds(0, (it + 1) & 1, nadA);
        m_block<SP, 1>(paA, W[1], accA, accA1, accB, accB1, xr[1], oB, rng);
        bias_init(accB, accB1, 1);
        __syncthreads();
        WS_STAMP(4);
        if constexpr (NL == 3) {
            m_block<SP, 1>(paB, W[1], accB, accB1, accA, accA1, xr[1], oA, rng);
            bias_init(accA, accA1, 2);
            __syncthreads();
            WS_STAMP(5);
            m_block<SP, 1>(paA, W[2], accA, accA1, accB, accB1, xr[1], oB, rng);
            bias_init(accB, accB1, 2);
            __syncthreads();
            WS_STAMP(6);
        }
        widen_x(nxa, nraw);
        if (pact) m_block<SP, 4, true>(paB, W[NL - 1], accB, accB1, accA, accA1, nxa, oA, rng);
        else m_block<SP, 4, false>(paB, W[NL - 1], accB, accB1, accA, accA1, nxa, oA, rng);
        other_all<SP, 3, false>(accB, accB1, xr[1], oB, rng);
        __syncthreads();
        WS_STAMP(7);
        start_values(accA, accA1, nadA);
        asm volatile("" : "+v"(accA[0]), "+v"(accA[1]) :: "memory");
        Meta m3;
        if constexpr (!DENSE) m3 = fix_meta(m3raw);
        gather_x(meta_at(pair + 1, m1), (it + 1) & 1, 1, xr[1], rawB);
        store_tables(tv, it + 2);
        WS_STAMP(8);

        if (!(G4C_WS_ABLATE & 256)) ln_tail(meta_at(pair, m0), it);
        if constexpr (SP == 1) gather_adds(1, (it + 1) & 1, adB);
        WS_STAMP(9);
        if (AGG) {
            __syncthreads();
            WS_STAMP(15);
            if (!(G4C_WS_ABLATE & 128)) agg_tail(meta_at(pair, m0), it);
        }
        WS_STAMP(16);
        if constexpr (SP != 1) gather_adds(1, (it + 1) & 1, adB);
        WS_STAMP(10);
        if constexpr (!DENSE) { m0 = m1; m1 = m2; m2 = m3; }
    }

    if constexpr (NODE) {
        __builtin_amdgcn_fence(__ATOMIC_RELEASE, "workgroup");
        __syncthreads();
        __builtin_amdgcn_fence(__ATOMIC_ACQUIRE, "workgroup");
        NodeCtx nc;
        nc.tid = tid; nc.wave = wave; nc.n = n; nc.g = g; nc.fcol = fcol; nc.prow = prow; nc.pc = pc; nc.lo_b = lo_b;
        nc.sBiasN = sBiasN; nc.sGBN = sGBN; nc.fA = fA; nc.fB = fB; nc.oA = oA; nc.oB = oB;
#pragma unroll
        for (int ks = 0; ks < 4; ++ks) { nc.paA[ks] = paA[ks]; nc.paB[ks] = paB[ks]; }
        const int t1 = 2 * p_end < p.n_tiles ? 2 * p_end : p.n_tiles;
        const int S0 = __builtin_amdgcn_readfirstlane(p.tile_seg[2 * p_begin]), S1 = __builtin_amdgcn_readfirstlane(p.tile_seg[t1]);
        const NodeParams q = node_params_now();
        node_phase<SP, NL, TRACK>(nc, p.agg, p.agg_ld, q, S0, S1);
    }
    WS_STAMP_ONCE(13, __builtin_readcyclecounter());
    if constexpr (SP == 2 && TRACK) {
        if (G4C_WS_SCALED && !(G4C_WS_ABLATE & 48)) rng.m *= F16_LO_UNSCALE;
        if (range_hit(rng)) {
            int *const word = range_word_now();
            if (word && (threadIdx.x & 63) == 0) *word = 1;
        }
    }
}


template <bool AGG, bool DIRECT, bool ADDS, int SP, int NL, bool XB16, bool AB16 = false, bool NODE = false, bool DENSE = false, bool TRACK = true>
__global__ __launch_bounds__(512, SP == 1 ? G4C_WS_SP1_MINW : 2) void mlp_ws_kernel(const WsKernArgs ka) {
    ws_body<AGG, DIRECT, ADDS, SP, NL, XB16, AB16, NODE, DENSE, TRACK, false>(ka);
}
template <bool DENSE>
__global__ __launch_bounds__(512, 2) void mlp_ws_pre_kernel(const WsKernArgs ka) {
    ws_body<true, true, true, 2, 3, false, false, false, DENSE, true, true>(ka);
}

#if defined(G4C_WS_ISA_ONLY) && G4C_WS_ISA_ONLY == 2
template __global__ void mlp_ws_pre_kernel<true>(const WsKernArgs);
template __global__ void mlp_ws_pre_kernel<false>(const WsKernArgs);
#elif defined(G4C_WS_ISA_ONLY)
template __global__ void mlp_ws_kernel<true, true, true, 2, 3, false, false, false, true, true>(const WsKernArgs);
template __global__ void mlp_ws_kernel<true, true, true, 2, 3, false, false, false, true, false>(const WsKernArgs);
template __global__ void mlp_ws_kernel<true, true, true, 2, 3, false, false, true, false, true>(const WsKernArgs);
template __global__ void mlp_ws_kernel<true, true, true, 2, 3, false, false, true, false, false>(const WsKernArgs);
#endif

}

#ifndef G4C_WS_ISA_ONLY
namespace g4cm {

bool ws_takes(const Launch &L) {
    const Params &p = L.p;
    const bool round1 = L.round1;
    if (!(L.f16x2 || round1) || !message_form(L)) return false;
    if ((round1 && p.n_add != 2) || (p.n_layers != 3 && p.n_layers != 2)) return false;
    if (p.out_bf16 && (!round1 || (p.out_ld & 7) || ((uintptr_t)p.out & 15))) return false;
    if (p.src[0].bf16 && !round1) return false;
    for (int a = 0; a < p.n_add; ++a)
        if (p.add[a].bf16 != p.add[0].bf16 || (p.add[a].bf16 && !round1)) return false;
    return true;
}

bool ws_pre_takes(const Launch &L) {
    const Params &p = L.p;
    if (!L.f16x2 || !L.agg || L.save || L.has_node || p.n_layers != 3) return false;
    if (p.n_src != 0 || p.n_nar != 0 || p.n_add != 3 || p.n_heads || p.n_out != NP || p.resid || p.out_idx || p.out_bf16) return false;
    if (p.add[0].idx || !p.add[1].idx || !p.add[2].idx) return false;
    for (int a = 0; a < 3; ++a)
        if (p.add[a].width != NP || p.add[a].bf16 || (p.add[a].ld & 3) || ((uintptr_t)p.add[a].ptr & 15)) return false;
    if (p.out && ((p.out_ld & 3) || ((uintptr_t)p.out & 15))) return false;
    if (p.gamma && (((uintptr_t)p.gamma & 15) || ((uintptr_t)p.beta & 15))) return false;
    return ((uintptr_t)p.b & 15) == 0 && p.M < (1LL << 31);
}

int ws_launch(const Launch &L, hipStream_t st, Ran &ran) {
    const Params &p = L.p;
    if (L.pre) {
        const bool dense = p.agg_deg >= 4 && p.agg_deg <= 8;
        const int n_pairs = dense ? (int)((p.M + 63) / 64) : (p.n_tiles + 1) / 2;
        const int n_wg = g4c::cu_count();
        const dim3 grid(n_pairs < n_wg ? n_pairs : n_wg), blk(512);
        ran.kernel = G4C_KERNEL_MLP_WS_PRE;
        WsArgs a{};
        a.x = p.add[0].ptr; a.x_idx = nullptr; a.x_ld = p.add[0].ld; a.x_pact = 0;
        for (int j = 0; j < 2; ++j) { a.add_ptr[j] = p.add[1 + j].ptr; a.add_idx[j] = p.add[1 + j].idx; a.add_ld[j] = p.add[1 + j].ld; }
        a.w = p.w; a.b = p.b; a.gamma = p.gamma; a.beta = p.beta; a.eps = p.eps; a.act = p.act;
        a.out = p.out; a.out_idx = nullptr; a.out_ld = p.out_ld; a.out_bf16 = 0;
        a.tile_rows = p.tile_rows; a.tile_seg = p.tile_seg; a.seg_off = p.seg_off;
        a.agg = p.agg; a.agg_ld = p.agg_ld; a.agg_mean = p.agg_mean; a.agg_deg = p.agg_deg;
        a.M = (int)p.M; a.row_base = (int)p.row_base; a.n_tiles = p.n_tiles;
        a.range_flag = p.range_certified ? nullptr : p.range_flag; a.range_slot = p.range_slot;
        const WsKernArgs ka{a, n_pairs, L.node};
        if (dense) mlp_ws_pre_kernel<true><<<grid, blk, 0, st>>>(ka);
        else mlp_ws_pre_kernel<false><<<grid, blk, 0, st>>>(ka);
        return g4c::check_launch("g4c_mlp_run (ws, first layer precomputed)");
    }
    const bool agg = L.agg, round1 = L.round1, node = L.has_node;
    const bool dense = agg && !node && p.agg_deg >= 4 && p.agg_deg <= 8;
    const int n_pairs = dense ? (int)((p.M + 63) / 64) : (p.n_tiles + 1) / 2;
    ran.kernel = G4C_KERNEL_MLP_WS;
    const int n_wg = g4c::cu_count() * (round1 ? G4C_WS_SP1_MINW / 2 : 1);
    const dim3 grid(n_pairs < n_wg ? n_pairs : n_wg), blk(512);
    const bool direct = p.src[0].idx == nullptr, adds = p.n_add == 2, two = p.n_layers == 2, xb16 = p.src[0].bf16 != 0;
    const bool ab16 = adds && p.add[0].bf16 != 0;
    const bool cert = p.range_certified && !round1 && adds;
    if (cert) ran.kernel = G4C_KERNEL_MLP_WS_CERT;
    WsArgs a{};
    const Src &s = p.src[0];
    a.x = s.bf16 ? reinterpret_cast<const float *>(reinterpret_cast<const __bf16 *>(s.ptr) + s.col0) : s.ptr + s.col0;
    a.x_idx = s.idx; a.x_ld = s.ld; a.x_pact = s.pre_act;
    for (int j = 0; j < 2; ++j) { a.add_ptr[j] = adds ? p.add[j].ptr : nullptr; a.add_idx[j] = adds ? p.add[j].idx : nullptr; a.add_ld[j] = adds ? p.add[j].ld : 0; }
    a.w = p.w; a.b = p.b; a.gamma = p.gamma; a.beta = p.beta; a.eps = p.eps; a.act = p.act;
    a.out = p.out; a.out_idx = p.out_idx; a.out_ld = p.out_ld; a.out_bf16 = p.out_bf16;
    a.tile_rows = p.tile_rows; a.tile_seg = p.tile_seg; a.seg_off = p.seg_off;
    a.agg = p.agg; a.agg_ld = p.agg_ld; a.agg_mean = p.agg_mean; a.agg_deg = p.agg_deg;
    a.M = (int)p.M; a.row_base = (int)p.row_base; a.n_tiles = p.n_tiles;
    a.range_flag = p.range_certified ? nullptr : p.range_flag; a.range_slot = p.range_slot;
    const WsKernArgs ka{a, n_pairs, L.node};
    if (node) {
        G4C_REQUIRE(agg && !round1 && adds, G4C_EUNSUPPORTED, "g4c_mlp_run (upd): needs the hoisted f16x3 message launch with the fused aggregation");
#define G4C_WS_NODE(DIRECT, NL)                                                                                                        \
    do { if (cert) mlp_ws_kernel<true, DIRECT, true, 2, NL, false, false, true, false, false><<<grid, blk, 0, st>>>(ka);    \
         else mlp_ws_kernel<true, DIRECT, true, 2, NL, false, false, true><<<grid, blk, 0, st>>>(ka); } while (0)
        if (direct) { if (two) G4C_WS_NODE(true, 2); else G4C_WS_NODE(true, 3); }
        else { if (two) G4C_WS_NODE(false, 2); else G4C_WS_NODE(false, 3); }
#undef G4C_WS_NODE
        return g4c::check_launch("g4c_mlp_run (ws, upd)");
    }
#define G4C_WS_GO(AGG, DIRECT, ADDS, SP, NL, XB16)                                                                                      \
    do { if (AGG && dense) mlp_ws_kernel<AGG, DIRECT, ADDS, SP, NL, XB16, false, false, AGG><<<grid, blk, 0, st>>>(ka);       \
         else mlp_ws_kernel<AGG, DIRECT, ADDS, SP, NL, XB16><<<grid, blk, 0, st>>>(ka); } while (0)
#define G4C_WS_GOC(AGG, DIRECT, NL)                                           \
    do { if (AGG && dense) mlp_ws_kernel<AGG, DIRECT, true, 2, NL, false, false, false, AGG, false><<<grid, blk, 0, st>>>(ka);       \
         else mlp_ws_kernel<AGG, DIRECT, true, 2, NL, false, false, false, false, false><<<grid, blk, 0, st>>>(ka); } while (0)
#define G4C_WS_GO1(AGG, DIRECT, NL, XB16)                                                                                               \
    do { if (AGG && dense) { if (ab16) mlp_ws_kernel<AGG, DIRECT, true, 1, NL, XB16, true, false, AGG><<<grid, blk, 0, st>>>(ka);       \
                             else mlp_ws_kernel<AGG, DIRECT, true, 1, NL, XB16, false, false, AGG><<<grid, blk, 0, st>>>(ka); }        \
         else if (ab16) mlp_ws_kernel<AGG, DIRECT, true, 1, NL, XB16, true><<<grid, blk, 0, st>>>(ka);                        \
         else mlp_ws_kernel<AGG, DIRECT, true, 1, NL, XB16, false><<<grid, blk, 0, st>>>(ka); } while (0)
#define G4C_WS_SHAPE(AGG, DIRECT)                                                                    \
    do {                                                                                             \
        if (round1) {                                                                                \
            if (two) { if (xb16) G4C_WS_GO1(AGG, DIRECT, 2, true); else G4C_WS_GO1(AGG, DIRECT, 2, false); }      \
            else { if (xb16) G4C_WS_GO1(AGG, DIRECT, 3, true); else G4C_WS_GO1(AGG, DIRECT, 3, false); }          \
        } else if (cert) {                                                                           \
            if (two) G4C_WS_GOC(AGG, DIRECT, 2); else G4C_WS_GOC(AGG, DIRECT, 3);                    \
        } else if (two) {                                                                            \
            if (adds) G4C_WS_GO(AGG, DIRECT, true, 2, 2, false); else G4C_WS_GO(AGG, DIRECT, false, 2, 2, false);                 \
        } else {                                                                                     \
            if (adds) G4C_WS_GO(AGG, DIRECT, true, 2, 3, false); else G4C_WS_GO(AGG, DIRECT, false, 2, 3, false);                 \
        }                                                                                            \
    } while (0)
    if (agg) { if (direct) G4C_WS_SHAPE(true, true); else G4C_WS_SHAPE(true, false); }
    else { if (direct) G4C_WS_SHAPE(false, true); else G4C_WS_SHAPE(false, false); }
#undef G4C_WS_SHAPE
#undef G4C_WS_GO1
#undef G4C_WS_GOC
#undef G4C_WS_GO
    return g4c::check_launch("g4c_mlp_run (ws)");
}

}
#endif
```

graphs4cfd_amd/csrc/plan.cpp:

```cpp
#include <algorithm>
#include <cstdint>
#include <numeric>
#include <vector>

#include "g4c_common.h"

extern "C" int g4c_plan_csr(const int64_t *keys, int64_t n, int64_t n_seg, int32_t *perm, int32_t *off) {
    G4C_REQUIRE(n >= 0 && n_seg >= 0 && n < (1LL << 31) && n_seg < (1LL << 31), G4C_EINVAL,
                "g4c_plan_csr: sizes out of int32 range (n=%lld n_seg=%lld)", (long long)n, (long long)n_seg);
    G4C_REQUIRE((keys || n == 0) && off && (perm || n == 0), G4C_EINVAL, "g4c_plan_csr: null pointer");
    std::fill(off, off + n_seg + 1, 0);
    for (int64_t p = 0; p < n; ++p) {
        const int64_t k = keys[p];
        G4C_REQUIRE(k >= 0 && k < n_seg, G4C_EINVAL, "g4c_plan_csr: key %lld at %lld outside [0, %lld)",
                    (long long)k, (long long)p, (long long)n_seg);
        off[k + 1]++;
    }
    for (int64_t s = 0; s < n_seg; ++s) off[s + 1] += off[s];
    std::vector<int32_t> cur(off, off + n_seg);
    for (int64_t p = 0; p < n; ++p) perm[cur[keys[p]]++] = (int32_t)p;
    return G4C_OK;
}

extern "C" int64_t g4c_plan_tiles(const int32_t *off, int32_t n_seg, int32_t max_rows, int32_t *tile_rows, int32_t *tile_seg,
                                  int64_t capacity) {
    G4C_REQUIRE(off && tile_rows && tile_seg && n_seg >= 0 && max_rows > 0 && capacity >= 1, G4C_EINVAL, "g4c_plan_tiles: bad arguments");
    int64_t nt = 0;
    int32_t s = 0;
    tile_rows[0] = off[0];
    tile_seg[0] = 0;
    while (s < n_seg) {
        const int32_t r0 = off[s];
        int32_t e = s;
        while (e < n_seg && off[e + 1] - r0 <= max_rows) ++e;
        if (e == s) return -1;
        G4C_REQUIRE(nt + 1 < capacity, G4C_EINVAL, "g4c_plan_tiles: capacity %lld too small", (long long)capacity);
        ++nt;
        tile_rows[nt] = off[e];
        tile_seg[nt] = e;
        s = e;
    }
    return nt;
}

extern "C" int64_t g4c_plan_pool_edge_ordered(const int64_t *idx_hr_to_lr, int64_t n_hr, const int64_t *edge_index,
                                              int64_t n_edges, int32_t target_major, int64_t *coarse_edge_index, int32_t *perm,
                                              int32_t *off, int64_t *n_kept) {
    G4C_REQUIRE(n_hr >= 0 && n_edges >= 0 && n_edges < (1LL << 31), G4C_EINVAL, "g4c_plan_pool_edge: bad sizes");
    G4C_REQUIRE((idx_hr_to_lr || n_hr == 0) && (edge_index || n_edges == 0) && off && n_kept, G4C_EINVAL,
                "g4c_plan_pool_edge: null pointer");
    int64_t n_lr = 0;
    for (int64_t i = 0; i < n_hr; ++i) {
        G4C_REQUIRE(idx_hr_to_lr[i] >= 0, G4C_EINVAL, "g4c_plan_pool_edge: idx_hr_to_lr[%lld] = %lld is negative", (long long)i,
                    (long long)idx_hr_to_lr[i]);
        n_lr = std::max(n_lr, idx_hr_to_lr[i] + 1);
    }
    G4C_REQUIRE(n_lr < (1LL << 31), G4C_EINVAL, "g4c_plan_pool_edge: %lld coarse nodes do not fit int32", (long long)n_lr);
    std::vector<int32_t> cr, cc, id;
    cr.reserve((size_t)n_edges); cc.reserve((size_t)n_edges); id.reserve((size_t)n_edges);
    const int64_t *row = edge_index, *col = edge_index + n_edges;
    for (int64_t e = 0; e < n_edges; ++e) {
        G4C_REQUIRE(row[e] >= 0 && row[e] < n_hr && col[e] >= 0 && col[e] < n_hr, G4C_EINVAL,
                    "g4c_plan_pool_edge: edge %lld endpoint outside [0, %lld)", (long long)e, (long long)n_hr);
        const int64_t r = idx_hr_to_lr[row[e]], c = idx_hr_to_lr[col[e]];
        if (r != c) { cr.push_back((int32_t)r); cc.push_back((int32_t)c); id.push_back((int32_t)e); }
    }
    const int64_t kept = (int64_t)id.size();
    *n_kept = kept;
    const std::vector<int32_t> &major = target_major ? cc : cr, &minor = target_major ? cr : cc;
    std::vector<int32_t> order((size_t)kept), tmp((size_t)kept);
    std::vector<int64_t> cnt((size_t)n_lr + 1);
    auto pass = [&](const std::vector<int32_t> &key, const int32_t *in, int32_t *out) {
        std::fill(cnt.begin(), cnt.end(), 0);
        for (int64_t p = 0; p < kept; ++p) ++cnt[(size_t)key[(size_t)in[p]] + 1];
        for (int64_t b = 0; b < n_lr; ++b) cnt[(size_t)b + 1] += cnt[(size_t)b];
        for (int64_t p = 0; p < kept; ++p) out[cnt[(size_t)key[(size_t)in[p]]]++] = in[p];
    };
    for (int64_t p = 0; p < kept; ++p) tmp[(size_t)p] = (int32_t)p;
    pass(minor, tmp.data(), order.data());
    pass(major, order.data(), tmp.data());
    int64_t n_coarse = 0;
    for (int64_t p = 0; p < kept; ++p) {
        const int32_t q = tmp[(size_t)p];
        if (p == 0 || cr[(size_t)q] != cr[(size_t)tmp[(size_t)p - 1]] || cc[(size_t)q] != cc[(size_t)tmp[(size_t)p - 1]]) ++n_coarse;
    }
    int64_t s = -1;
    for (int64_t p = 0; p < kept; ++p) {
        const int32_t q = tmp[(size_t)p];
        if (p == 0 || cr[(size_t)q] != cr[(size_t)tmp[(size_t)p - 1]] || cc[(size_t)q] != cc[(size_t)tmp[(size_t)p - 1]]) {
            ++s;
            off[s] = (int32_t)p;
            coarse_edge_index[s] = cr[(size_t)q];
            coarse_edge_index[n_coarse + s] = cc[(size_t)q];
        }
        perm[p] = id[(size_t)q];
    }
    off[n_coarse] = (int32_t)kept;
    return n_coarse;
}

extern "C" int64_t g4c_plan_pool_edge(const int64_t *idx_hr_to_lr, int64_t n_hr, const int64_t *edge_index,
                                      int64_t n_edges, int64_t *coarse_edge_index, int32_t *perm, int32_t *off,
                                      int64_t *n_kept) {
    return g4c_plan_pool_edge_ordered(idx_hr_to_lr, n_hr, edge_index, n_edges, 0, coarse_edge_index, perm, off, n_kept);
}
```

graphs4cfd_amd/ops.py:

```python
from __future__ import annotations

import ctypes as C
import os
from typing import List, Optional, Sequence, Tuple

import torch

from . import _lib
from .plan import CsrPlan

Tensor = torch.Tensor


class KernelTimer:
    active = None

    def __init__(self):
        self.records = []

    def __enter__(self):
        KernelTimer.active = self
        return self

    def __exit__(self, *exc):
        KernelTimer.active = None
        return False

    def launch(self, kind: str, flops: float, nbytes: float, fn):
        a, b = torch.cuda.Event(enable_timing=True), torch.cuda.Event(enable_timing=True)
        a.record()
        out = fn()
        b.record()
        if kind.startswith("mlp_"):
            kind = _lib.KERNEL_NAMES.get(int(_lib.load().g4c_mlp_last_kernel()), kind)
        self.records.append((kind, flops, nbytes, a, b))
        return out

    def summary(self):
        out = {}
        for kind, flops, nbytes, a, b in self.records:
            d = out.setdefault(kind, {"launches": 0, "seconds": 0.0, "flops": 0.0, "bytes": 0.0})
            d["launches"] += 1
            d["seconds"] += a.elapsed_time(b) * 1e-3
            d["flops"] += flops
            d["bytes"] += nbytes
        return out


def _timed(kind: str, flops: float, nbytes: float, fn):
    kt = KernelTimer.active
    return fn() if kt is None else kt.launch(kind, flops, nbytes, fn)


class StaticCache:
    active: Optional["StaticCache"] = None

    def __init__(self):
        self.store = {}
        self.hits = self.misses = 0
        self._prev = None

    def __enter__(self):
        self._prev, StaticCache.active = StaticCache.active, self
        prec = mlp_precision()
        for name in [n for n, hit in self.store.items() if hit[0][1] != prec]:
            del self.store[name]
        return self

    def __exit__(self, *exc):
        StaticCache.active = self._prev
        return False

    def get(self, name: str, inputs: Sequence[Tensor], fn):
        key = (weights_epoch(), mlp_precision()) + tuple((t.data_ptr(), t._version, tuple(t.shape), t.dtype) for t in inputs)
        hit = self.store.get(name)
        global _last_bounds
        if hit is not None and hit[0] == key:
            self.hits += 1
            _last_bounds = hit[3]
            return hit[1]
        self.misses += 1
        val = fn()
        self.store[name] = (key, val, tuple(inputs), _last_bounds)
        return val
# ... 1227 lines not shown
            if n_out > NP:
                raise NotImplementedError(f"layer width {n_out} > 128 is outside the fused-MLP kernel envelope")
            if l == 0:
                segs, negs = list(seg_widths), [1 if x else 0 for x in seg_negate]
                self.narrow_w = {}
                if any(narrow):
                    col0s = [sum(seg_widths[:j]) for j in range(len(seg_widths))]
                    W32 = W.detach().to(torch.float32)
                    for j in range(len(seg_widths)):
                        if narrow[j]:
                            rows = torch.zeros((seg_widths[j], NP), dtype=torch.float32, device=dev)
                            rows[:, :n_out] = W32[:, col0s[j]:col0s[j] + seg_widths[j]].T * (-1.0 if seg_negate[j] else 1.0)
                            self.narrow_w[j] = rows.contiguous()
                            self._keep.append(self.narrow_w[j])
                    if wide:
                        W = torch.cat([W32[:, col0s[j]:col0s[j] + seg_widths[j]] for j in wide], dim=1)
                        segs, negs = [seg_widths[j] for j in wide], [1 if seg_negate[j] else 0 for j in wide]
                        k_in = int(W.size(1))
                    else:
                        W = None
            else:
                prev = int(weights[l - 1].size(0))
                if k_in != prev:
                    raise ValueError(f"layer {l + 1} expects {k_in} inputs, previous layer gives {prev}")
                segs, negs = [k_in], [0]
            wptr = stream_buf.data_ptr() + esz * off
            if W is not None:
                pack(W, l, n_out, k_in, segs, negs, wptr, k_pads[l])
            if b is not None:
                bias_buf[l * NP: l * NP + n_out].copy_(b.detach())
            self.desc.k_pad[l], self.desc.n_pad[l] = k_pads[l], NP
            self.desc.w[l], self.desc.b[l] = wptr, bias_buf.data_ptr() + 4 * l * NP
            off += k_pads[l] * NP
        self.n_heads = len(heads)
        for W in heads:
            pack(W, None, NP, NP, [NP], [0], stream_buf.data_ptr() + esz * off, NP)
            off += NP * NP
        self.n_out = int(weights[-1].size(0))
        self.desc.n_out = self.n_out
        self.flops_per_row = float(sum(2 * int(W.size(0)) * int(W.size(1)) for W in list(weights) + list(heads)))
        if ln is not None:
            g, be, eps = ln
            g, be = g.detach().to(torch.float32).contiguous(), be.detach().to(torch.float32).contiguous()
            self.desc.ln_gamma, self.desc.ln_beta, self.desc.ln_eps = g.data_ptr(), be.data_ptr(), float(eps)
            self._keep += [g, be]
        else:
            self.desc.ln_gamma, self.desc.ln_beta, self.desc.ln_eps = None, None, 0.0
        self.seg_widths = tuple(seg_widths)
        self.device = dev
        self.norms = weight_norms(weights, biases, ln, heads, seg_widths, narrow) if self.split == "f16x2" else None
        if self.norms is not None:
            check_weight_range(self.norms, self.site)
        self.params = (list(weights), list(biases), ln)
        self.heads_params = bool(heads)


def _src_array(sources: Sequence[Source]):
    arr = (_lib.g4c_src_t * len(sources))()
    for a, s in zip(arr, sources):
        a.ptr, a.idx, a.width, a.ld, a.col0, a.pre_act = (s.tensor.data_ptr(), _lib.ptr(s.index), s.width, _ld(s.tensor),
                                                          s.col0, s.pre_act)
        a.additive = 1 if s.additive else 0
        a.dtype = 1 if s.tensor.dtype == torch.bfloat16 else 0
        if s.segments is not None:
            a.seg_off, a.seg_mean, a.seg_perm = _lib.ptr(s.segments.off), 1 if s.seg_mean else 0, _lib.ptr(s.segments.perm)
    return arr


def agg_bound(bound: Optional[float], csr: CsrPlan, mean: bool) -> Optional[float]:
    return bound if (bound is None or mean) else bound * max(csr.max_deg, 1)


def _certify(packed: "PackedMLP", sources: Sequence[Source], act: int, residual: bool, tracked: bool) -> LaunchBounds:
    seg_len = max((s_.segments.max_deg for s_ in sources if s_.segments is not None), default=None)
    lb = range_bounds(packed.norms, sources, act, residual, seg_len)
    packed.desc.range_certified = 1 if (RANGE_PROOFS and not tracked and certifies(lb.converted)) else 0
    return lb


def _agg_mode(agg_mean: bool, csr: CsrPlan) -> int:
    return (1 if agg_mean else 0) | (csr.uniform_deg << 8)


def _set_agg(io, csr: CsrPlan, agg_out: Tensor, agg_mean: bool) -> None:
    t_rows, t_seg, nt = csr.tiles()
    io.tile_rows, io.tile_seg, io.seg_off, io.n_tiles = _lib.ptr(t_rows), _lib.ptr(t_seg), _lib.ptr(csr.off), nt
    io.agg, io.agg_ld, io.agg_mode = _lib.ptr(agg_out), _ld(agg_out), _agg_mode(agg_mean, csr)


def _set_heads(io, head_outs: Sequence[Tensor]) -> None:
    io.n_heads, io.head_ld = len(head_outs), _ld(head_outs[0])
    io.head_dtype = 1 if head_outs[0].dtype == torch.bfloat16 else 0
    for j, h in enumerate(head_outs):
        io.head_out[j] = h.data_ptr()


def _run(packed: PackedMLP, arr, n_src: int, n_rows: int, io, dev, flops: float, nbytes: float) -> None:
    if packed.split == "f16x2":
        io.range_flag = _launch_flags(dev).data_ptr()
    kind = "mlp_split_kernel<4>" if packed.precision == "fp32" else "mlp_bx6_kernel"
    _timed(kind, flops, nbytes, lambda: _lib.check(_lib.load().g4c_mlp_run(C.byref(packed.desc), arr, n_src, n_rows, C.byref(io),
                                                                           _lib.stream_handle(dev))))


def mp_layer_forward(msg: PackedMLP, sources: Sequence[Source], n_rows: int, csr: CsrPlan, agg_mean: bool, upd: PackedMLP,
                     v: Tensor, act: int, store_rows: bool = True, head_outs: Optional[Sequence[Tensor]] = None,
                     v_out: Optional[Tensor] = None, v_bound: Optional[float] = None, e_out: Optional[Tensor] = None,
                     agg_out: Optional[Tensor] = None) -> Tuple[Optional[Tensor], Tensor, Optional[Sequence[Tensor]]]:
    global _last_bounds
    _last_bounds = None
    if e_out is not None:
        if not store_rows:
            raise ValueError("e_out: given with store_rows=False (the launch stores no e' rows)")
        _rows_f32(e_out, "e_out", cols=128, min_rows=n_rows)
    if agg_out is not None:
        _rows_f32(agg_out, "agg_out", cols=128, min_rows=csr.n_seg)
    dev = _lib.require_hip(*[s.tensor for s in sources], *[s.index for s in sources], v, v_out, e_out, agg_out)
    if msg.split != "f16x2" or upd.split != "f16x2":
        raise NotImplementedError("mp_layer_forward needs both MLPs packed for the f16x3 arithmetic")
    if csr.tiles() is None or n_rows != csr.n:
        raise ValueError("mp_layer_forward: the rows must be in segment order with segments of at most 32 rows")
    v = _f32_2d(v, "v")
    n_t = csr.n_seg
    if e_out is None and store_rows:
        e_out = torch.empty((n_rows, 128), dtype=torch.float32, device=dev)
    agg = agg_out if agg_out is not None else torch.empty((n_t, 128), dtype=torch.float32, device=dev)
    if v_out is None:
        v_out = torch.empty((n_t, 128), dtype=torch.float32, device=dev)
    n_heads = 0 if head_outs is None else len(head_outs)
    if n_heads and (n_heads != upd.n_heads):
        raise ValueError(f"{n_heads} head outputs for a packing with {upd.n_heads} heads")
    io = _lib.g4c_mlp_io_t(row_count=n_rows, out=_lib.ptr(e_out), out_ld=128 if e_out is None else _ld(e_out), upd=C.pointer(upd.desc),
                           v=_lib.ptr(v), v_ld=_ld(v), v_act=act, v_out=_lib.ptr(v_out), v_out_ld=_ld(v_out))
    _set_agg(io, csr, agg, agg_mean)
    if n_heads:
        _set_heads(io, head_outs)
    in_b = 4.0 * 128 * (n_rows * (2 if store_rows else 1) + n_t * (2 + n_heads))
    lb_msg = _certify(msg, sources, _lib.ACT_NONE, False, False)
    lb_upd = _certify(upd, [Source(agg, bound=agg_bound(lb_msg.out, csr, agg_mean)), Source(v, bound=v_bound)], act, False, False)
    try:
        _run(msg, _src_array(sources), len(sources), n_rows, io, dev, msg.flops_per_row * n_rows + upd.flops_per_row * n_t, in_b)
    finally:
        msg.desc.range_certified = upd.desc.range_certified = 0
    _last_bounds = LaunchBounds(None, lb_upd.out, lb_upd.heads, e=lb_msg.out)
    return e_out, v_out, head_outs


STATIC_FIRST_LAYER = os.environ.get("G4C_STATIC_FIRST_LAYER", "1") != "0"


def mlp_forward_precomputed(packed: PackedMLP, first: Tensor, products: Sequence[Source], n_rows: int,
                            agg: Tuple[CsrPlan, Tensor, bool], act: int = _lib.ACT_NONE, store_rows: bool = True,
                            out: Optional[Tensor] = None) -> Optional[Tensor]:
    global _last_bounds
    _last_bounds = None
    csr, agg_out, agg_mean = agg
    if out is not None:
        if not store_rows:
            raise ValueError("out: given with store_rows=False (the launch stores no rows)")
        _rows_f32(out, "out", cols=128, min_rows=n_rows)
    dev = _lib.require_hip(first, agg_out, out, *[s.tensor for s in products], *[s.index for s in products])
    if dev != packed.device:
        raise RuntimeError(f"MLP weights on {packed.device}, inputs on {dev}")
    if packed.split != "f16x2" or packed.desc.n_layers != 3 or packed.seg_widths != (128,) or packed.n_out != 128 or packed.n_heads:
        raise NotImplementedError("mlp_forward_precomputed: a three-layer 128-wide MLP over one 128-wide block, packed for f16x3, no heads")
    if len(products) != 2 or any(not s.additive or s.index is None or s.width != 128 or s.tensor.dtype != torch.float32 for s in products):
        raise ValueError("mlp_forward_precomputed: two additive 128-wide fp32 sources gathered through an index")
    first = _rows_f32(first, "first", cols=128, min_rows=n_rows)
    if csr.tiles() is None or n_rows != csr.n:
        raise ValueError("mlp_forward_precomputed: the rows must be in segment order with segments of at most 32 rows")
    if agg_out.dtype != torch.float32:
        raise TypeError(f"aggregate: expected float32, got {agg_out.dtype}")
    if out is None and store_rows:
        out = torch.empty((n_rows, 128), dtype=torch.float32, device=dev)
    desc = _lib.g4c_mlp_t()
    C.memmove(C.byref(desc), C.byref(packed.desc), C.sizeof(desc))
    desc.k_pad[0], desc.w[0], desc.range_certified = 0, packed.desc.w[1], 0
    srcs = [Source(first, additive=True)] + list(products)
    io = _lib.g4c_mlp_io_t(act=act, row_count=n_rows, out=_lib.ptr(out), out_ld=128 if out is None else _ld(out))
    _set_agg(io, csr, agg_out, agg_mean)
    io.range_flag = _launch_flags(dev).data_ptr()
    flops = float(2 * 2 * 128 * 128) * n_rows
    nbytes = 4.0 * 128 * (n_rows * (2 if store_rows else 1) + csr.n_seg)
    arr = _src_array(srcs)
    _timed("mlp_bx6_kernel", flops, nbytes, lambda: _lib.check(_lib.load().g4c_mlp_run(C.byref(desc), arr, 3, n_rows, C.byref(io),
                                                                                       _lib.stream_handle(dev))))
    ln = packed.norms["ln"] if packed.norms is not None else None
    _last_bounds = LaunchBounds(None, act_bound((packed.norms["n_out"] - 1) ** 0.5 * ln[0] + ln[1], act) if ln is not None else None)
    return out


def _rows_dtype(what: str, tensors: Sequence[Tensor]) -> int:
    kinds = {t.dtype for t in tensors}
    if not kinds <= {torch.float32, torch.bfloat16} or len(kinds) > 1:
        raise TypeError(f"{what} tensors must share one dtype, float32 or bfloat16 (got {sorted(str(k) for k in kinds)})")
    return _lib.DTYPE_BF16 if kinds == {torch.bfloat16} else _lib.DTYPE_F32


def mlp_forward(packed: PackedMLP, sources: Sequence[Source], n_rows: int, act: int = _lib.ACT_NONE,
                out: Optional[Tensor] = None, out_idx32: Optional[Tensor] = None,
                resid: Optional[Tensor] = None, resid_col0: int = 0, rows: Optional[Tuple[int, int]] = None,
                head_outs: Optional[Sequence[Tensor]] = None, agg: Optional[Tuple[CsrPlan, Tensor, bool]] = None,
                save: Optional[Sequence[Optional[Tensor]]] = None, mul: Optional[Sequence[Optional[Tensor]]] = None,
                store_rows: bool = True, rows_dtype: Optional[torch.dtype] = None, rows_act: int = _lib.ACT_NONE) -> Optional[Tensor]:
    global _last_bounds
    _last_bounds = None
    if torch.is_grad_enabled():
        from . import autograd as _ag
        if _ag.wants_grad(packed, sources, resid):
            if out is not None or out_idx32 is not None or head_outs is not None or agg is not None or rows is not None or save is not None:
                raise NotImplementedError("out= / heads / fused aggregation are inference-only forms of mlp_forward; "
                                          "call under torch.no_grad() or use the plain form")
            return _ag.mlp(packed, sources, n_rows, act, resid, resid_col0)
    if packed.rs2:
        ok = [isinstance(s.tensor, RsOrderedRows) for s in sources]
        if len(sources) != 2 or not ok[0] or ok[1] != (packed.rs2 == 4) or any(s.tensor.dtype != torch.bfloat16 for s in sources):
            raise ValueError("weights packed for the row-split update kernel: [aggregate | e] as bf16 rows, the aggregate (and, format 4, e) RsOrderedRows")
    elif packed.rs_order and packed.precision == "bf16":
        if any(s.tensor.dtype == torch.bfloat16 and not isinstance(s.tensor, RsOrderedRows) for s in sources):
            raise ValueError("weights packed for the row-split kernel: bf16 rows must be RsOrderedRows (its column order)")
    elif any(isinstance(s.tensor, RsOrderedRows) for s in sources) or any(packed.rs_blocks):
        fixed, j = [], 0
        for s in sources:
            tagged = isinstance(s.tensor, RsOrderedRows)
            ok = (not s.additive) and j < len(packed.rs_blocks) and packed.rs_blocks[j] and s.col0 == 0 and s.width == 128
            if not s.additive:
                if j < len(packed.rs_blocks) and packed.rs_blocks[j] and not tagged:
                    raise ValueError(f"input block {j}: the weights expect rows in the row-split order (ops.RsOrderedRows)")
                j += 1
            fixed.append(s if (not tagged or ok) else
                         Source(rs_rows_to_natural(s.tensor), s.index, s.col0, s.width, s.negate, s.pre_act, s.additive, s.segments, s.seg_mean))
        sources = fixed
    dev = _lib.require_hip(*[s.tensor for s in sources], *[s.index for s in sources], out, out_idx32, resid)
    if dev != packed.device:
        raise RuntimeError(f"MLP weights on {packed.device}, inputs on {dev}")
    if tuple(s.width for s in sources if not s.additive) != packed.seg_widths:
        raise ValueError(f"input blocks {[s.width for s in sources if not s.additive]} do not match packed layout {packed.seg_widths}")
    arr = _src_array(sources)
    if any(packed.narrow):
        j = 0
        for a, src in zip(arr, sources):
            if src.additive:
                continue
            if packed.narrow[j]:
                if src.index is not None or src.pre_act != _lib.ACT_NONE:
                    raise ValueError("a narrow input block cannot be gathered through an index or activated on load")
                a.additive, a.w = 2, packed.narrow_w[j].data_ptr()
            j += 1
    fusable = (agg is not None and FUSE_AGG and packed.precision in ("bf16x6", "bf16") and packed.n_out == 128 and head_outs is None
               and rows is None and out_idx32 is None and resid is None and n_rows == agg[0].n and agg[0].tiles() is not None)
    if not store_rows and not fusable:
        raise ValueError("store_rows=False needs an aggregation the launch can fuse (ops.can_fuse_aggregation)")
    reduce_after = None
    if agg is not None and not fusable:
        reduce_after, agg = agg, None
    rows16 = bool(fusable and store_rows and rows_dtype == torch.bfloat16 and packed.precision == "bf16" and out is None)
    if out is None and store_rows:
        out = torch.empty((n_rows, packed.n_out), dtype=torch.bfloat16 if rows16 else torch.float32, device=dev)
    if out is not None and out.dtype not in (torch.float32, torch.bfloat16):
        raise TypeError(f"out: expected float32 or bfloat16, got {out.dtype}")
    row_begin, row_count = rows if rows is not None else (0, n_rows)
    io = _lib.g4c_mlp_io_t(act=act, row_begin=row_begin, row_count=row_count, out=_lib.ptr(out),
                           out_ld=_ld(out) if out is not None else 128, out_idx=_lib.ptr(out_idx32), resid=_lib.ptr(resid),
                           resid_ld=_ld(resid) if resid is not None else 0, resid_col0=resid_col0)
    if out is not None and out.dtype == torch.bfloat16:
        if agg is None and (packed.precision != "bf16" or out_idx32 is not None or resid is not None):
            raise TypeError("a bf16 `out` needs the rounded-bf16 mode and no output index / residual")
        if rows16 and rows_act not in (_lib.ACT_NONE, _lib.ACT_SELU):
            raise ValueError("rows_act: only ACT_SELU")
        io.out_dtype = 2 if (rows16 and rows_act == _lib.ACT_SELU) else 1
    in_bytes = float(sum(s.width * (2 if s.tensor.dtype == torch.bfloat16 else 4) for s in sources if not s.additive))
    nbytes = (in_bytes + 4.0 * packed.n_out) * row_count
    if head_outs is not None:
        if len(head_outs) != packed.n_heads or packed.n_heads == 0:
            raise ValueError(f"{len(head_outs)} head outputs for a packing with {packed.n_heads} heads")
        if out_idx32 is not None or resid is not None:
            raise NotImplementedError("heads with an output index / residual")
        _lib.require_hip(*head_outs)
        if any(h.dtype == torch.bfloat16 for h in head_outs):
            if packed.precision != "bf16" or any(h.dtype != torch.bfloat16 for h in head_outs):
                raise TypeError("bf16 head outputs need the rounded-bf16 mode, and every head in bf16")
        elif out.dtype != torch.float32:
            raise TypeError("heads stored as fp32 need fp32 output rows (bf16 rows: bf16 heads)")
        _set_heads(io, head_outs)
        if packed.precision == "fp32":
            nbytes = 4.0 * (sum(packed.seg_widths) + packed.n_out * (1 + packed.n_heads)) * n_rows
    if agg is not None:
        csr, agg_out, agg_mean = agg
        _lib.require_hip(agg_out)
        if agg_out.dtype not in (torch.float32, torch.bfloat16):
            raise TypeError(f"aggregate: expected float32 (or bfloat16 on the row-split kernel), got {agg_out.dtype}")
        _set_agg(io, csr, agg_out, agg_mean)
        if agg_out.dtype == torch.bfloat16:
            io.agg_mode |= 1 << 16
        out_b = 0 if not store_rows else packed.n_out * (2 if out.dtype == torch.bfloat16 else 4)
        nbytes = (in_bytes + out_b) * n_rows + 4.0 * packed.n_out * csr.n_seg
    if save is not None:
        live = [t for t in save if t is not None]
        _lib.require_hip(*live)
        if any(t.dim() != 2 or t.size(0) < n_rows or t.size(1) < 128 or t.stride(1) != 1 or _ld(t) != _ld(live[0]) for t in live):
            raise ValueError("save tensors must be [n_rows, >= 128] fp32 (or bf16) with one common leading dimension")
        if len(save) > _lib.MAX_LAYERS:
            raise ValueError(f"{len(save)} save tensors for {packed.desc.n_layers} layers")
        io.n_save, io.save_ld = len(save), _ld(live[0]) if live else 128
        io.save[:len(save)] = [_lib.ptr(t) for t in save]
        io.save_dtype = _rows_dtype("save", live)
        if mul is not None:
            lm = [t for t in mul if t is not None]
            _lib.require_hip(*lm)
            if len(mul) != len(save) or any(t.size(0) < n_rows or t.size(1) < 128 or t.stride(1) != 1 or _ld(t) != _ld(lm[0]) for t in lm):
                raise ValueError("mul tensors must be [n_rows, >= 128] fp32 (or bf16) with one common leading dimension, one entry per layer")
            io.mul[:len(mul)] = [_lib.ptr(t) for t in mul]
            io.mul_ld = _ld(lm[0]) if lm else 128
            io.mul_dtype = _rows_dtype("mul", lm)
        nbytes = (4.0 * (sum(packed.seg_widths) + packed.n_out) + 128.0 * sum(t.element_size() for t in live)) * n_rows
    lb = _certify(packed, sources, act, resid is not None or out_idx32 is not None or rows is not None, save is not None)
    try:
        _run(packed, arr, len(sources), n_rows, io, dev, packed.flops_per_row * row_count, nbytes)
    finally:
        packed.desc.range_certified = 0
    _last_bounds = lb
    if reduce_after is not None:
        segment_reduce(out, reduce_after[0], reduce_after[2], out=reduce_after[1])
    return out
```

graphs4cfd_amd/partition.py:

```python
from __future__ import annotations

from dataclasses import dataclass, field
from typing import Dict, List, Optional, Sequence

import numpy as np
import torch

from . import _lib, ops, plan
from .graph import Graph
from .ops import Source

SELU, TANH, NONE = _lib.ACT_SELU, _lib.ACT_TANH, _lib.ACT_NONE


@dataclass
class LevelPart:
    owned: np.ndarray
    halo: np.ndarray
    halo_owner: np.ndarray
    edge_ids: np.ndarray
    edge_index: np.ndarray
    send_idx: List[np.ndarray] = field(default_factory=list)
    recv_counts: List[int] = field(default_factory=list)

# ... 267 lines not shown
            w = int(v_out.size(1))
            res = mlp.run_with_heads(srcs, n_own, act, nxt, nxt.input_size - 2 * w, [w, w], out=v_out,
                                     head_outs=[pr_out[:n_own], None])
            if res is not None:
                return pr_out, res[1][1]
        mlp.run_coded(srcs, n_own, act, out=v_out)
        return None

    def encode(self, mesh: LocalMesh, v_out: torch.Tensor, next_name: Optional[str] = None, pr_out: Optional[torch.Tensor] = None):
        m = self.m
        e = ops.static_launch("edge_encoder", [mesh.edge_attr],
                              lambda: m.edge_encoder.run_coded([Source(mesh.edge_attr)], int(mesh.edge_attr.size(0)), SELU))
        srcs = [Source(mesh.inputs[k]) for k in ("field", "loc", "glob", "omega") if k in mesh.inputs]
        return e, self._node_launch(m.node_encoder, srcs, mesh.n_own[0], SELU, v_out, next_name, pr_out)

    def hoists(self, n_edges: int) -> bool:
        from .nn import blocks as _blocks
        return n_edges >= _blocks.HOIST_MIN_ROWS and ops.mlp_precision() != "bf16"

    def mp(self, name: str, v: torch.Tensor, e: torch.Tensor, e_pending: int, edge_index: torch.Tensor, n_own: int,
           v_out: torch.Tensor, products=None, next_name: Optional[str] = None, pr_out: Optional[torch.Tensor] = None,
           overlap=None):
        blk = getattr(self.m, name)
        ep, csr = plan.edge_csr(edge_index, n_own)
        mean = blk.aggr == "mean"
        if overlap is not None:
            start, wait, sub = overlap
            handle = start()
            e_new = torch.empty((ep.n_edges, blk.edge_mlp.output_size), dtype=torch.float32, device=e.device)
            for tag in ("int", "bnd"):
                ids, row, col = sub[tag]
                if tag == "bnd":
                    wait(handle)
                if int(ids.numel()):
                    blk.edge_mlp.run_hoisted([Source(e, index=ids, pre_act=e_pending)], [(v, row), (v, col)], int(ids.numel()),
                                             products=products, out=e_new, out_idx32=ids)
            if ops.can_aggregate_on_load(csr, blk.edge_mlp.output_size, [blk.edge_mlp.output_size, int(v.size(1))]):
                agg_src = Source(e_new, segments=csr, seg_mean=mean)
            else:
                agg_src = Source(ops.segment_reduce(e_new, csr, mean))
            return e_new, self._node_launch(blk.node_mlp, [agg_src, Source(v[:n_own])], n_own, SELU, v_out, next_name, pr_out)
        if (not ops.can_fuse_aggregation(csr, blk.edge_mlp.output_size)
                and ops.can_aggregate_on_load(csr, blk.edge_mlp.output_size, [blk.edge_mlp.output_size, int(v.size(1))])):
            e_new = blk.edge_mlp.run_hoisted([Source(e, pre_act=e_pending)], [(v, ep.row), (v, ep.col)], ep.n_edges, products=products)
            agg_src = Source(e_new, segments=csr, seg_mean=mean)
        else:
            agg = torch.empty((csr.n_seg, blk.edge_mlp.output_size), dtype=torch.float32, device=e.device)
            e_new = blk.edge_mlp.run_hoisted([Source(e, pre_act=e_pending)], [(v, ep.row), (v, ep.col)], ep.n_edges,
                                             products=products, agg=(csr, agg, mean))
            agg_src = Source(agg)
        return e_new, self._node_launch(blk.node_mlp, [agg_src, Source(v[:n_own])], n_own, SELU, v_out, next_name, pr_out)

    def down(self, name: str, v_own: torch.Tensor, rel: torch.Tensor, parent: torch.Tensor, n_coarse: int, e: torch.Tensor,
             e_pending: int, pool_csr, v_out: torch.Tensor):
        blk = getattr(self.m, name)
        msg = blk.down_mlp.run_coded([Source(rel), Source(v_own)], int(v_own.size(0)))
        csr = plan.segments_of_sorted(parent, n_coarse)
        ops.segment_reduce(msg, csr, True, TANH, out=v_out)
        return ops.segment_reduce(e, pool_csr, True, src_act=e_pending)

    def up(self, name: str, v_coarse: torch.Tensor, v_old_own: torch.Tensor, rel: torch.Tensor, parent: torch.Tensor,
           v_out: torch.Tensor, next_name: Optional[str] = None, pr_out: Optional[torch.Tensor] = None):
        blk = getattr(self.m, name)
        srcs = [Source(rel, negate=True), Source(v_coarse, plan.index32(parent)), Source(v_old_own)]
        return self._node_launch(blk.up_mlp, srcs, int(v_old_own.size(0)), TANH, v_out, next_name, pr_out)

    def decode(self, v_own: torch.Tensor, field: torch.Tensor, nf: int) -> torch.Tensor:
        return self.m.node_decoder.run_coded([Source(v_own)], int(v_own.size(0)), NONE, resid=field,
                                             resid_col0=int(field.size(1)) - nf)


class MusPartitionedForward:

    def __init__(self, program: Sequence[str], mesh: LocalMesh, impl, exchanger: HaloExchanger, width: int, nf: int):
        self.program, self.mesh, self.impl, self.xch, self.width, self.nf = tuple(program), mesh, impl, exchanger, width, nf
        import os
        self.overlap = os.environ.get("G4C_DIST_OVERLAP", "1") != "0"

    def _buf(self, level: int) -> torch.Tensor:
        m = self.mesh
        return self.impl.new(m.n_own[level - 1] + m.n_halo[level - 1], self.width, m.device)

    def forward(self) -> torch.Tensor:
        m, impl = self.mesh, self.impl
        level = 1
        v = self._buf(1)

        def wants(k: int, lvl: int) -> bool:
            return (k < len(self.program) and self.program[k].startswith("mp")
                    and impl.hoists(m.decision_edges[lvl - 1]))

        w0 = wants(0, 1)
        e, prod = impl.encode(m, v[: m.n_own[0]], self.program[0] if w0 else None, self._buf(1) if w0 else None)
        e_pending = NONE
        stash = []
        for k, name in enumerate(self.program):
            n_own = m.n_own[level - 1]
            if name.startswith("down_mp"):
                prod = None
                stash.append((v, e, e_pending))
                v_c = self._buf(level + 1)
                e = impl.down(name, v[:n_own], m.rel[level - 1], m.parent[level - 1], m.n_own[level], e, e_pending,
                              m.pool_edge_csr(level), v_c[: m.n_own[level]])
                v, e_pending = v_c, NONE
                level += 1
            elif name.startswith("up_mp"):
                v_old, e, e_pending = stash.pop()
                level -= 1
                v_f = self._buf(level)
                wn = wants(k + 1, level)
                prod = impl.up(name, v, v_old[: m.n_own[level - 1]], m.rel[level - 1], m.parent[level - 1], v_f[: m.n_own[level - 1]],
                               self.program[k + 1] if wn else None, self._buf(level) if wn else None)
                v = v_f
            else:
                overlap = None
                if prod is not None and self.overlap and m.world > 1 and getattr(impl, "overlaps", False) and hasattr(self.xch, "exchange_async"):
                    pr = prod[0]
                    overlap = (lambda pr=pr, level=level: self.xch.exchange_async(pr, level), self.xch.wait, m.sub[level - 1])
                elif prod is not None:
                    self.xch.exchange(prod[0], level)
                else:
                    self.xch.exchange(v, level)
                v_new = self._buf(level)
                nxt = self.program[k + 1] if k + 1 < len(self.program) else ""
                want_next = nxt.startswith("mp") and impl.hoists(m.decision_edges[level - 1])
                kw = {"overlap": overlap} if overlap is not None else {}
                e, prod = impl.mp(name, v, e, e_pending, m.edge_index[level - 1], n_own, v_new[:n_own], products=prod,
                                  next_name=nxt if want_next else None, pr_out=self._buf(level) if want_next else None, **kw)
                v, e_pending = v_new, SELU
        return impl.decode(v[: m.n_own[0]], m.inputs["field"], self.nf)


class DistributedRollout:

    def __init__(self, model, graph_cpu: Graph, max_steps: int, rank: int, world: int, device: torch.device, group=None,
                 capture: bool = True):
        import os
        capture = capture and os.environ.get("G4C_DIST_HIPGRAPH", "1") != "0"
        self.model, self.rank, self.world, self.device = model, rank, world, device
        program = model._PROGRAM
        self.n_global = int(graph_cpu.pos.size(0))
        self._perm = None
        self.nf = int(model.num_fields)
        if hasattr(model, "_ENCODERS"):
            from . import partition_remus as PR
            parts = PR.build_remus_partition(graph_cpu, world)
            self.mesh = PR.RemusLocalMesh(graph_cpu, parts[rank], device, rank, world)
            self.fwd = PR.RemusPartitionedForward(program, self.mesh, PR.RemusHipImpl(model, self.mesh), HaloExchanger(self.mesh, group))
        else:
            if self.n_global >= 50_000 and os.environ.get("G4C_REORDER", "1") != "0":
                from .reorder import reorder_nodes
                re = reorder_nodes(graph_cpu)
                if re is not None:
                    graph_cpu, self._perm = re[0], re[1].to(device)
            levels = 1 + sum(1 for n in program if n.startswith("down_mp"))
            parts = build_partition(graph_cpu, levels, world)
            self.mesh = LocalMesh(graph_cpu, levels, parts[rank], device, rank, world)
            self.mesh.decision_edges = uniform_edge_counts(parts)
            width = int(model.node_encoder.output_size)
            self.fwd = MusPartitionedForward(program, self.mesh, HipImpl(model), HaloExchanger(self.mesh, group), width, self.nf)
        self.max_steps = max_steps
        self.field = self.mesh.inputs["field"] = self.mesh.inputs["field"].clone()
        self._out_steps = torch.zeros((max_steps, int(self.mesh.owned_global[0].numel()), self.nf), dtype=torch.float32, device=device)
        self.step_counter = torch.zeros(2, dtype=torch.int32, device=device)
        self.steps_done = 0
        self.capture = capture and device.type == "cuda"
# ... 119 lines not shown
```

graphs4cfd_amd/partition_remus.py:

```python
from __future__ import annotations

from dataclasses import dataclass, field
from typing import Dict, List, Optional

import numpy as np
import torch

from . import _lib, ops, plan
from .graph import Graph
from .ops import Source
from .partition import _rcb

SELU, NONE = _lib.ACT_SELU, _lib.ACT_NONE
SFX = {1: "", 2: "2", 3: "3"}
LEVELS = 3
CH_NODE = {2: 4, 3: 5}


@dataclass
class RemusLevel:
    edge_ids: np.ndarray
    halo_edges: np.ndarray
    halo_owner: np.ndarray
    angle_ids: np.ndarray
# ... 194 lines not shown
        self._turn: Dict[tuple, int] = {}

    def buf(self, kind: str, lvl: int) -> torch.Tensor:
        mesh, key = self.mesh, (kind, lvl)
        if key not in self._bufs:
            rows = mesh.n_edges[lvl] + mesh.n_halo_edges[lvl] if kind == "e" else mesh.n_level_nodes[lvl] + mesh.n_halo_nodes[lvl]
            width = self.width if kind == "e" else 2 * self.width
            self._bufs[key] = [torch.zeros((rows, width), dtype=torch.float32, device=mesh.device) for _ in range(2 if kind == "e" else 1)]
            self._turn[key] = 0
        pair = self._bufs[key]
        self._turn[key] = (self._turn[key] + 1) % len(pair)
        return pair[self._turn[key]]

    def encode(self):
        m, mesh = self.m, self.mesh
        nfeat = int(mesh.inputs["field"].size(1)) // 2
        e, a = {}, {}
        for l in range(1, LEVELS + 1):
            s = SFX[l]
            proj = ops.project_to_edges(mesh.inputs["field"], mesh.col32[l], mesh.unit[l], mesh.n_edges[l], nfeat)
            e[l] = self.buf("e", l)
            getattr(m, f"edge_encoder{s}").run_coded([Source(proj), Source(mesh.inputs["glob"], mesh.col32[l]), Source(mesh.inputs["omega"], mesh.col32[l])],
                                                     mesh.n_edges[l], SELU, out=e[l][: mesh.n_edges[l]])
            a[l] = self._angle_latents(f"angle_encoder{s}", mesh.angle_attr[l])
        ax = {1: self._angle_latents("angle_encoder12", mesh.down_attr[1]), 2: self._angle_latents("angle_encoder23", mesh.down_attr[2])}
        return e, a, ax

    def _angle_latents(self, name: str, att: torch.Tensor) -> torch.Tensor:
        enc = getattr(self.m, name)
        return ops.static_launch(name, [att], lambda: enc.run_coded([Source(att)], int(att.size(0)), SELU))

    def mp(self, name: str, e: torch.Tensor, a: torch.Tensor, a_pending: int, lvl: int):
        from .nn.blocks import _mp_step
        blk, n_own = getattr(self.m, name), self.mesh.n_edges[lvl]
        out = self.buf("e", lvl)
        _, a_new = _mp_step(blk.angle_mlp, blk.edge_mlp, e, a, self.mesh.angle_index[lvl], blk.aggr, SELU, a_pending,
                            n_targets=n_own, v_out=out[:n_own], compact_messages=True)
        return out, a_new

    def down(self, name: str, e_lo: torch.Tensor, e_hi: torch.Tensor, a_x: torch.Tensor, lvl: int):
        from .nn.blocks import _mp_step
        blk, n_own = getattr(self.m, name), self.mesh.n_edges[lvl + 1]
        out = self.buf("e", lvl + 1)
        _mp_step(blk.angle_mlp, blk.edge_mlp, e_hi, a_x, self.mesh.down_index[lvl], "mean", SELU, v_src=e_lo,
                 n_targets=n_own, v_out=out[:n_own])
        return out

    def node_vectors(self, e_lo: torch.Tensor, lo: int) -> torch.Tensor:
        mesh = self.mesh
        nb = self.buf("n", lo)
        n_own = mesh.n_level_nodes[lo]
        if n_own:
            ops.edge_scalar_to_node_vector(e_lo[: mesh.n_edges[lo]], mesh.unit_inv[lo], n_own, mesh.k, out=nb[:n_own])
        return nb

    def up(self, name: str, nodebuf: torch.Tensor, e_hi: torch.Tensor, lo: int):
        mesh, hi = self.mesh, lo - 1
        nfeat = int(nodebuf.size(1)) // 2
        v1 = torch.zeros((mesh.n_nodes, 2 * nfeat), dtype=torch.float32, device=mesh.device) if hi > 1 else \
            torch.empty((mesh.n_nodes, 2 * nfeat), dtype=torch.float32, device=mesh.device)
        csr = plan.segments_of_sorted(mesh.interp_y[lo], mesh.n_level_nodes[hi])
        ops.weighted_segment_mean(nodebuf, mesh.interp_x32[lo], mesh.interp_w[lo], csr, v1, mesh.level_node32[hi] if hi > 1 else None)
        e1 = ops.project_to_edges(v1, mesh.col32[hi], mesh.unit[hi], mesh.n_edges[hi], nfeat)
        out = self.buf("e", hi)
        getattr(self.m, name).up_mlp.run_coded([Source(e1), Source(e_hi)], mesh.n_edges[hi], SELU, out=out[: mesh.n_edges[hi]])
        return out

    def decode(self, e1: torch.Tensor) -> torch.Tensor:
        mesh = self.mesh
        s = self.m.edge_decoder.run_coded([Source(e1)], mesh.n_edges[1], NONE)
        out = ops.edge_scalar_to_node_vector(s, mesh.unit_inv[1], mesh.n_nodes, mesh.k)
        res = torch.empty_like(out)
        f = mesh.inputs["field"]
        ops.add_cols(f, int(f.size(1)) - 2, out, res)
        return res


class RemusPartitionedForward:

    def __init__(self, program, mesh: RemusLocalMesh, impl, exchanger):
        self.program, self.mesh, self.impl, self.xch = program, mesh, impl, exchanger

    def forward(self) -> torch.Tensor:
        impl, x = self.impl, self.xch
        e, a, ax = impl.encode()
        fresh = {l: False for l in e}
        a_pending = {l: NONE for l in e}

        def need_halo(l):
            if not fresh[l]:
                x.exchange(e[l], l)
                fresh[l] = True

        for op, name, lvl in self.program:
            if op == "mp":
                need_halo(lvl)
                e[lvl], a[lvl] = impl.mp(name, e[lvl], a[lvl], a_pending[lvl], lvl)
                from .nn.blocks import pending_act
                a_pending[lvl], fresh[lvl] = pending_act(a[lvl]), False
            elif op == "down":
                need_halo(lvl)
                e[lvl + 1] = impl.down(name, e[lvl], e[lvl + 1], ax[lvl], lvl)
                fresh[lvl + 1] = False
            else:
                nb = impl.node_vectors(e[lvl], lvl)
                x.exchange(nb, CH_NODE[lvl])
                e[lvl - 1] = impl.up(name, nb, e[lvl - 1], lvl)
                fresh[lvl - 1] = False
        return impl.decode(e[1])
```

graphs4cfd_amd/plan.py:

```python
from __future__ import annotations

import collections
import ctypes as C
from dataclasses import dataclass
from typing import Optional, Tuple

import numpy as np
import torch

from . import _lib


@dataclass
class CsrPlan:
    perm: Optional[torch.Tensor]
    off: torch.Tensor
    n: int
    n_seg: int
    max_deg: int
    uniform_deg: int = 0
    _tiles: object = False

    def tiles(self, max_rows: int = 32):
        if self._tiles is False:
            self._tiles = None
            if self.perm is None and self.n > 0 and 0 < self.max_deg <= max_rows:
                lib = _lib.load()
                off = np.ascontiguousarray(_host_i64(self.off).astype(np.int32))
                cap = self.n_seg + 2
                rows, seg = np.empty(cap, np.int32), np.empty(cap, np.int32)
                nt = int(lib.g4c_plan_tiles(off.ctypes.data, self.n_seg, max_rows, rows.ctypes.data, seg.ctypes.data, cap))
                if nt > 0:
                    dev = self.off.device
                    self._tiles = (_upload(rows[: nt + 1].copy(), dev), _upload(seg[: nt + 1].copy(), dev), nt)
        return self._tiles


@dataclass
class EdgePlan:
    row: torch.Tensor
    col: torch.Tensor
    n_edges: int
    csr: dict


@dataclass
class PoolEdgePlan:
    edge_index: torch.Tensor
    csr: CsrPlan
    n_coarse: int


def _host_i64(t: torch.Tensor) -> np.ndarray:
    if t.device.type != "cpu":
        hit = _host_image(t)
        if hit is not None:
            return np.ascontiguousarray(hit, dtype=np.int64)
    return np.ascontiguousarray(t.detach().to("cpu", torch.int64).numpy())


def _host_image(t: torch.Tensor) -> Optional[np.ndarray]:
    hit = _host_copies.get(_Cache.key(t))
    if hit is None:
        return None
    arr, src, version = hit
    if src is not None and src._version != version:
        return None
    return arr


def _upload(arr: np.ndarray, device) -> torch.Tensor:
    return torch.from_numpy(arr).to(device)


def remember_host(dev_tensor: torch.Tensor, host) -> None:
    if dev_tensor.device.type == "cpu" or dev_tensor.dtype.is_floating_point or not _REMEMBER_HOST:
        return
    src = host if torch.is_tensor(host) else None
    arr = host.detach().numpy() if src is not None else np.asarray(host)
    _host_copies.put(_Cache.key(dev_tensor), (dev_tensor,), (arr, src, src._version if src is not None else 0))


def _uniform(deg: np.ndarray) -> int:
    if deg.size == 0:
        return 0
    k = int(deg.max())
    return k if 1 <= k <= 32 and int(deg.min()) == k else 0


def build_csr(keys: torch.Tensor, n_seg: int, device: torch.device, drop_last_segment: bool = False) -> CsrPlan:
    lib = _lib.load()
    k = _host_i64(keys)
    n = int(k.shape[0])
    perm = np.empty(n, dtype=np.int32)
    off = np.empty(n_seg + 1, dtype=np.int32)
    _lib.check(lib.g4c_plan_csr(k.ctypes.data, n, n_seg, perm.ctypes.data, off.ctypes.data))
    if drop_last_segment:
        n_seg -= 1
        off = off[: n_seg + 1]
        perm = perm[: int(off[-1])]
    n_kept = int(perm.shape[0])
    identity = n_kept == n and bool(np.array_equal(perm, np.arange(n, dtype=np.int32)))
    deg = np.diff(off)
    off_h = off.copy()
    out = CsrPlan(
        perm=None if identity else _upload(perm.copy(), device),
        off=_upload(off_h, device),
        n=n_kept, n_seg=n_seg, max_deg=int(deg.max()) if deg.size else 0, uniform_deg=_uniform(deg))
    remember_host(out.off, off_h)
    return out


def _nbytes(obj, depth: int = 0) -> int:
    if torch.is_tensor(obj):
        return obj.numel() * obj.element_size()
    if isinstance(obj, np.ndarray):
        return int(obj.nbytes)
    if depth > 3 or obj is None or isinstance(obj, (int, float, str, bool)):
# ... 211 lines not shown
```

include/g4c.h:

```cpp
#ifndef G4C_H
#define G4C_H

#include <stdint.h>

#ifdef __cplusplus
extern "C" {
#endif

#define G4C_OK 0
#define G4C_EINVAL (-1)
#define G4C_ELAUNCH (-2)
#define G4C_EUNSUPPORTED (-3)

#define G4C_ACT_NONE 0
#define G4C_ACT_SELU 1
#define G4C_ACT_TANH 2

#define G4C_MAX_SRC 4
#define G4C_MAX_LAYERS 4
#define G4C_MAX_HEADS 2
#define G4C_NARROW_MAX 8

int g4c_version(void);
int g4c_device_info(const void *device_ptr, int32_t *device , int32_t *cu_count );
// ... 23 lines not shown

#define G4C_DTYPE_F32 0
#define G4C_DTYPE_BF16 1
#define G4C_DTYPE_BF16_SELU 2

typedef struct {
    const float *ptr;
    const int32_t *idx;
    int32_t width;
    int32_t ld;
    int32_t col0;
    int32_t pre_act;
    int32_t additive;
    int32_t seg_mean;
    const float *w;
    const int32_t *seg_off;
    const int32_t *seg_perm;
    int32_t dtype;
} g4c_src_t;

typedef struct {
    int32_t n_layers;
    int32_t k_pad[G4C_MAX_LAYERS];
    int32_t n_pad[G4C_MAX_LAYERS];
    const float *w[G4C_MAX_LAYERS];
    const float *b[G4C_MAX_LAYERS];
    const float *ln_gamma;
    const float *ln_beta;
    float ln_eps;
    int32_t n_out;
    int32_t w_format;
    int32_t range_slot;
    int32_t range_certified;
} g4c_mlp_t;

#define G4C_WFMT_FP32 0
#define G4C_WFMT_F16X2 1
#define G4C_WFMT_BF16X3 2
#define G4C_WFMT_BF16_RS 3
#define G4C_WFMT_BF16_RS2 4
#define G4C_WFMT_BF16_RS2N 5
#define G4C_WFMT_BF16 6

int g4c_mlp_pack_layer(const float *W, int32_t n_out, int32_t k_in, const int32_t *seg_width ,
                       const int32_t *seg_negate , int32_t n_seg, int32_t w_format, void *packed,
                       int32_t k_pad, int32_t n_pad, void *stream);

#define G4C_AGG_UNIFORM(k) ((int32_t)(k) << 8)
#define G4C_AGG_OUT_BF16 ((int32_t)1 << 16)

typedef struct {
    int32_t size;
    int32_t act;
    int64_t row_begin;
    int64_t row_count;
    void *out;
    int32_t out_ld;
    int32_t out_dtype;
    const int32_t *out_idx;
    const float *resid;
    int32_t resid_ld, resid_col0;
    int32_t n_heads;
    int32_t head_ld;
    int32_t head_dtype;
    void *head_out[G4C_MAX_HEADS];
    const int32_t *tile_rows, *tile_seg, *seg_off;
    int32_t n_tiles;
    void *agg;
    int32_t agg_ld;
    int32_t agg_mode;
    int32_t n_save;
    void *save[G4C_MAX_LAYERS];
    int32_t save_ld;
    const void *mul[G4C_MAX_LAYERS];
    int32_t mul_ld;
    const g4c_mlp_t *upd;
    const float *v;
    int32_t v_ld, v_act;
    float *v_out;
    int32_t v_out_ld;
    int32_t *range_flag;
    int32_t save_dtype;
    int32_t mul_dtype;
} g4c_mlp_io_t;

int g4c_mlp_run(const g4c_mlp_t *mlp , const g4c_src_t *srcs , int32_t n_src, int64_t n_rows,
                const g4c_mlp_io_t *io , void *stream);

int g4c_mlp_bx6i_enable(int on);

int g4c_mlp_ws_enable(int on);

int g4c_mlp_small_launch_tiles(int n_tiles);

#define G4C_KERNEL_NONE 0
#define G4C_KERNEL_MLP_SPLIT 1
#define G4C_KERNEL_MLP_BX6 2
#define G4C_KERNEL_MLP_BX6I 3
#define G4C_KERNEL_MLP_WS 4
#define G4C_KERNEL_MLP_RS 5
#define G4C_KERNEL_MLP_RS2 6
#define G4C_KERNEL_MLP_BX6_CERT 7
#define G4C_KERNEL_MLP_WS_CERT 8
#define G4C_KERNEL_MLP_WS_PRE 9
int g4c_mlp_last_kernel(void);

#define G4C_TILE_SHAPE_GENERIC 0
#define G4C_TILE_SHAPE_NODE 1
#define G4C_TILE_SHAPE_UP 2
#define G4C_TILE_SHAPE_DOWN 3
int g4c_mlp_shapes_enable(int on);
int g4c_mlp_last_shape(void);

int64_t g4c_plan_tiles(const int32_t *off , int32_t n_seg, int32_t max_rows, int32_t *tile_rows ,
                       int32_t *tile_seg , int64_t capacity);

int g4c_layer_norm(const float *x, int32_t x_ld, int64_t n_rows, int32_t width, const float *gamma, const float *beta, float eps,
                   int32_t act, float *out, int32_t out_ld, void *stream);

int g4c_debug_mean_div(const float *a, const int32_t *count, float *out, int64_t n4, void *stream);

int g4c_project_to_edges(const float *v, int32_t v_ld, const int32_t *node, const float *unit,
                         int64_t n_edges, int32_t n_feat, float *out, int32_t out_ld, void *stream);

int g4c_edge_scalar_to_node_vector(const float *e, int32_t e_ld, const float *unit_inv, int32_t k,
                                   int64_t n_nodes, int32_t n_feat, float *out, int32_t out_ld,
                                   void *stream);

int g4c_knn_grid(const float *pos_sorted, const int32_t *cell_sorted, const int32_t *order,
                 const int32_t *cell_start, int64_t n, int32_t dim, const int32_t *n_cells, const float *origin,
                 float cell_size, int32_t k, int64_t *out, void *stream);

int g4c_knn_grid_query(const float *pos_sorted, const int32_t *order, const int32_t *cell_start, int64_t n, int32_t dim,
                       const int32_t *n_cells, const float *origin, float cell_size, const float *q_pos,
                       const int32_t *q_cell, int64_t m, int32_t k, int64_t *out, void *stream);

int g4c_rollout_advance(float *field, int32_t field_cols, const float *pred, int32_t nf,
                        float *outputs, int32_t out_ld, int32_t *step, int64_t n_nodes, void *stream);

typedef struct g4c_rollout_rec {
    int32_t max_steps;
    float  *snap;
    int32_t every, n_snap;
    const int32_t *probe_rows;
    int32_t n_probe;
    float  *probe_out;
    const float *target;
    int32_t target_ld;
    const uint8_t *mask;
    double *stats;
    double *scratch;
} g4c_rollout_rec_t;
enum { G4C_REC_SQ_ERR, G4C_REC_ABS_ERR, G4C_REC_MAX_ABS_ERR, G4C_REC_TGT_SUM, G4C_REC_TGT_SQ_SUM, G4C_REC_ABS_ERR_MASK, G4C_REC_NSTAT };
int64_t g4c_rollout_record_scratch_doubles(int64_t n_nodes, int32_t nf);
int g4c_rollout_advance_record(float *field, int32_t field_cols, const float *pred, int32_t nf, const g4c_rollout_rec_t *rec ,
                               int32_t *step, int64_t n_nodes, void *stream);

typedef struct g4c_rollout_moments {
    int32_t max_steps;
    int32_t stride;
    int32_t *window;
    const float *sub;
    int32_t sub_ld;
    int64_t plane_ld;
    double *pivot, *sum, *sum2, *lo, *hi;
} g4c_rollout_moments_t;
int g4c_rollout_moments(const float *pred, int32_t nf, const g4c_rollout_moments_t *m , const int32_t *step, int64_t n_nodes,
                        void *stream);

typedef struct g4c_rollout_spectrum {
    int32_t max_steps;
    int32_t stride;
    int32_t n_samples;
    int32_t n_bins;
    int32_t *window;
    const double *tw;
    int32_t x_ld;
    int32_t x_step;
    int64_t plane_ld;
    double *pivot, *sum, *re, *im;
} g4c_rollout_spectrum_t;
int g4c_rollout_spectrum(const float *x, int32_t nf, const g4c_rollout_spectrum_t *s , const int32_t *step, int64_t n_nodes,
                         void *stream);

int g4c_mesh_gradient_weights(const int32_t *off, const int32_t *perm , const int32_t *src32, const float *rel, int32_t dim,
                              int32_t power, int64_t n_nodes, int64_t n_edges, float *g, int32_t *src, uint8_t *degenerate, void *stream);

#define G4C_DERIVED_MAX_COLS 8
#define G4C_DERIVED_MAX_TERMS 3
enum { G4C_DERIVED_SQ, G4C_DERIVED_ABS, G4C_DERIVED_MAX_ABS, G4C_DERIVED_NSTAT };
typedef struct g4c_derived_program {
    int32_t nd;
    int32_t n_terms[G4C_DERIVED_MAX_COLS];
    int32_t field[G4C_DERIVED_MAX_COLS][G4C_DERIVED_MAX_TERMS];
    int32_t axis[G4C_DERIVED_MAX_COLS][G4C_DERIVED_MAX_TERMS];
    float coef[G4C_DERIVED_MAX_COLS][G4C_DERIVED_MAX_TERMS];
} g4c_derived_program_t;
typedef struct g4c_mesh_derived {
// ... 62 lines not shown
```

Before: 263.2.

## Add row-range form of weight-stationary fused MLP aggregation for arbitrary segments

Adds a row-range plan that splits rows evenly across one workgroup per CU, with segment boundaries staged in shared memory. A new ANY instantiation of the weight-stationary kernel reduces segments of any length in 64-row pairs and carries partial sums across pair boundaries. This lets aggregation fuse into the MLP even when segments exceed 32 rows or tiles are unavailable, avoiding a separate store-and-reduce pass. It costs extra shared memory, an added per-pair carry path through one wave, and host-side planning, and it is turned off for the partitioned forward paths.

```diff
diff --git a/graphs4cfd_amd/_lib.py b/graphs4cfd_amd/_lib.py
--- a/graphs4cfd_amd/_lib.py
+++ b/graphs4cfd_amd/_lib.py
@@ -65,7 +65,8 @@
                 ("mul", C.c_void_p * MAX_LAYERS), ("mul_ld", C.c_int32),
                 ("upd", C.POINTER(g4c_mlp_t)), ("v", C.c_void_p), ("v_ld", C.c_int32), ("v_act", C.c_int32),
                 ("v_out", C.c_void_p), ("v_out_ld", C.c_int32), ("range_flag", C.c_void_p),
-                ("save_dtype", C.c_int32), ("mul_dtype", C.c_int32)]
+                ("save_dtype", C.c_int32), ("mul_dtype", C.c_int32),
+                ("wg_rows", C.c_void_p), ("wg_seg", C.c_void_p), ("n_wg", C.c_int32), ("wg_pairs", C.c_int32), ("wg_max_seg", C.c_int32)]
 
     def __init__(self, **kw):
         super().__init__(size=C.sizeof(g4c_mlp_io_t), **kw)
@@ -130,12 +131,15 @@
                                      C.c_int32, C.c_int32, C.c_void_p]),
     "g4c_mlp_run": (C.c_int, [C.POINTER(g4c_mlp_t), C.POINTER(g4c_src_t), C.c_int32, C.c_int64, C.POINTER(g4c_mlp_io_t), C.c_void_p]),
     "g4c_plan_tiles": (C.c_int64, [C.c_void_p, C.c_int32, C.c_int32, C.c_void_p, C.c_void_p, C.c_int64]),
+    "g4c_plan_row_ranges": (C.c_int64, [C.c_void_p, C.c_int32, C.c_int32, C.c_void_p, C.c_void_p, C.POINTER(C.c_int32)]),
+    "g4c_mlp_ws_grid": (C.c_int, [C.c_void_p, C.POINTER(C.c_int32)]),
     "g4c_mlp_bx6i_enable": (C.c_int, [C.c_int]),
     "g4c_mlp_ws_enable": (C.c_int, [C.c_int]),
     "g4c_mlp_small_launch_tiles": (C.c_int, [C.c_int]),
     "g4c_layer_norm": (C.c_int, [C.c_void_p, C.c_int32, C.c_int64, C.c_int32, C.c_void_p, C.c_void_p, C.c_float, C.c_int32, C.c_void_p, C.c_int32, C.c_void_p]),
     "g4c_debug_mean_div": (C.c_int, [C.c_void_p, C.c_void_p, C.c_void_p, C.c_int64, C.c_void_p]),
     "g4c_mlp_last_kernel": (C.c_int, []),
+    "g4c_mlp_last_row_ranges": (C.c_int, []),
     "g4c_mlp_shapes_enable": (C.c_int, [C.c_int]),
     "g4c_mlp_last_shape": (C.c_int, []),
     "g4c_project_to_edges": (C.c_int, [C.c_void_p, C.c_int32, C.c_void_p, C.c_void_p, C.c_int64, C.c_int32,
diff --git a/graphs4cfd_amd/csrc/error.cpp b/graphs4cfd_amd/csrc/error.cpp
--- a/graphs4cfd_amd/csrc/error.cpp
+++ b/graphs4cfd_amd/csrc/error.cpp
@@ -1,5 +1,6 @@
 #include "g4c_common.h"
 #include <atomic>
+#include <cstdlib>
 
 namespace g4c {
 static thread_local char g_err[512] = "";
@@ -34,6 +35,22 @@
 }
 
 extern "C" int g4c_version(void) { return 3; }
+namespace g4c {
+int ws_grid() {
+    int n = cu_count();
+    if (const char *cap = std::getenv("G4C_WS_MAX_GRID")) {
+        const int c = std::atoi(cap);
+        if (c >= 1 && c < n) n = c;
+    }
+    return n;
+}
+}
+extern "C" int g4c_mlp_ws_grid(const void *device_ptr, int32_t *n_wg) {
+    G4C_REQUIRE(device_ptr && n_wg, G4C_EINVAL, "g4c_mlp_ws_grid: null pointer");
+    g4c::DeviceGuard on_device(device_ptr);
+    *n_wg = g4c::ws_grid();
+    return G4C_OK;
+}
 extern "C" int g4c_device_info(const void *device_ptr, int32_t *device, int32_t *cu_count) {
     G4C_REQUIRE(device_ptr && device && cu_count, G4C_EINVAL, "g4c_device_info: null pointer");
     g4c::DeviceGuard on_device(device_ptr);
diff --git a/graphs4cfd_amd/csrc/g4c_common.h b/graphs4cfd_amd/csrc/g4c_common.h
--- a/graphs4cfd_amd/csrc/g4c_common.h
+++ b/graphs4cfd_amd/csrc/g4c_common.h
@@ -21,6 +21,7 @@
 
 int visible_devices();
 int cu_count();
+int ws_grid();
 struct DeviceGuard {
     int prev = -1;
     explicit DeviceGuard(const void *device_ptr) {
diff --git a/graphs4cfd_amd/csrc/mlp_common.h b/graphs4cfd_amd/csrc/mlp_common.h
--- a/graphs4cfd_amd/csrc/mlp_common.h
+++ b/graphs4cfd_amd/csrc/mlp_common.h
@@ -73,6 +73,8 @@
     int agg_ld, agg_mean;
     int agg_deg;
     int agg_bf16;
+    const int *wg_rows, *wg_seg;
+    int n_wg, wg_pairs, wg_max_seg;
     NarSrc nar[G4C_MAX_SRC];
     int n_nar;
     float *save[G4C_MAX_LAYERS];
@@ -283,7 +285,7 @@
     int io_n_tiles;
     bool deep_ring, shapes;
 };
-struct Ran { int kernel = G4C_KERNEL_NONE, shape = G4C_TILE_SHAPE_GENERIC; };
+struct Ran { int kernel = G4C_KERNEL_NONE, shape = G4C_TILE_SHAPE_GENERIC, ranges = 0; };
 
 inline bool message_form(const Launch &L) {
     const Params &p = L.p;
@@ -305,6 +307,7 @@
 bool bx6i_takes(const Launch &L);
 int bx6i_launch(const Launch &L, hipStream_t st, Ran &ran);
 bool ws_takes(const Launch &L);
+bool ws_any_takes(const Launch &L);
 bool ws_pre_takes(const Launch &L);
 int ws_launch(const Launch &L, hipStream_t st, Ran &ran);
 bool rs_takes(const Launch &L);
diff --git a/graphs4cfd_amd/csrc/mlp_run.hip b/graphs4cfd_amd/csrc/mlp_run.hip
--- a/graphs4cfd_amd/csrc/mlp_run.hip
+++ b/graphs4cfd_amd/csrc/mlp_run.hip
@@ -48,8 +48,8 @@
     G4C_REQUIRE(io->n_heads >= 0 && io->n_heads <= G4C_MAX_HEADS, G4C_EINVAL, "g4c_mlp_run: bad heads (n=%d)", io->n_heads);
     G4C_REQUIRE((L.row_begin == 0 && L.row_count == n_rows) || (!L.agg && !L.save && !L.has_node && !io->n_heads && !io->out_dtype),
                 G4C_EUNSUPPORTED, "g4c_mlp_run: a row sub-range needs a plain launch (no heads / aggregation / save / upd / out_dtype)");
-    G4C_REQUIRE(!L.agg || (io->tile_rows && io->tile_seg && io->seg_off && io->n_tiles >= 0 && io->agg_ld >= NP), G4C_EINVAL,
-                "g4c_mlp_run: bad aggregation plan");
+    G4C_REQUIRE(!L.agg || (io->seg_off && io->agg_ld >= NP && ((io->tile_rows && io->tile_seg && io->n_tiles >= 0) || (io->wg_rows && !io->tile_rows))),
+                G4C_EINVAL, "g4c_mlp_run: bad aggregation plan");
     G4C_REQUIRE(io->out_dtype == G4C_DTYPE_F32 || io->out_dtype == G4C_DTYPE_BF16 || io->out_dtype == G4C_DTYPE_BF16_SELU, G4C_EINVAL,
                 "g4c_mlp_run: unknown out_dtype %d", io->out_dtype);
     G4C_REQUIRE(io->out_dtype != G4C_DTYPE_BF16_SELU || (L.agg && io->act == G4C_ACT_NONE), G4C_EINVAL,
@@ -168,6 +168,11 @@
                     L.row_count);
         G4C_REQUIRE(p.agg_deg == 0 || L.row_begin == 0, G4C_EINVAL,
                     "g4c_mlp_run: uniform segments (G4C_AGG_UNIFORM) need the whole row range, got rows [%lld, %lld)", L.row_begin, p.M);
+        if (io->wg_rows) {
+            G4C_REQUIRE(io->wg_seg && io->n_wg >= 1 && io->n_wg <= g4c::cu_count() && io->wg_pairs >= 1 && io->wg_max_seg >= 1 && L.row_begin == 0,
+                        G4C_EINVAL, "g4c_mlp_run: bad row ranges (n_wg=%d wg_pairs=%d wg_max_seg=%d)", io->n_wg, io->wg_pairs, io->wg_max_seg);
+            p.wg_rows = io->wg_rows; p.wg_seg = io->wg_seg; p.n_wg = io->n_wg; p.wg_pairs = io->wg_pairs; p.wg_max_seg = io->wg_max_seg;
+        }
     }
     if (io->out_dtype) {
         G4C_REQUIRE(L.round1 && !p.resid && !p.out_idx && p.n_out == NP && (!p.out || ((p.out_ld & 3) == 0 && ((uintptr_t)p.out & 7) == 0)), G4C_EUNSUPPORTED,
@@ -286,6 +291,7 @@
         G4C_REQUIRE(L.f16x2, nullptr, "g4c_mlp_run: every source additive (first layer precomputed) needs the f16x3 format (G4C_WFMT_F16X2), got w_format %d", L.fmt);
         G4C_REQUIRE(L.p.n_layers == 3, nullptr, "g4c_mlp_run: every source additive (first layer precomputed) needs three layers (two left), got %d", L.p.n_layers);
         G4C_REQUIRE(L.agg && !L.save, nullptr, "g4c_mlp_run: every source additive (first layer precomputed) needs the fused aggregation and no save");
+        G4C_REQUIRE(L.p.tile_rows, nullptr, "g4c_mlp_run: every source additive (first layer precomputed) needs the tiles of whole segments");
         G4C_REQUIRE(ws_pre_takes(L), nullptr,
                     "g4c_mlp_run: every source additive (first layer precomputed) is outside the weight-stationary kernel's envelope (three aligned "
                     "128-wide fp32 additive blocks — the first direct, two through indices —, a plain fp32 128-wide output, no heads / residual "
@@ -296,6 +302,13 @@
         G4C_REQUIRE(ws_takes(L), nullptr,
                     "g4c_mlp_run: the message launch of the fused MP layer is outside the weight-stationary kernel's envelope (one 128-wide "
                     "weighted block, two 128-wide additive blocks, two or three 128-wide layers, aligned rows)");
+        G4C_REQUIRE(L.p.tile_rows || ws_any_takes(L), nullptr, "g4c_mlp_run: a fused MP layer without tiles of whole segments is outside the row-range form's envelope");
+        return ws_launch;
+    }
+    if (L.agg && !L.p.tile_rows) {
+        G4C_REQUIRE(!L.row_split && ws_takes(L) && ws_any_takes(L), nullptr,
+                    "g4c_mlp_run: an aggregation plan of row ranges alone needs the weight-stationary kernel's row-range form (f16x3, one direct "
+                    "128-wide weighted block, two 128-wide additive blocks, two or three layers, fp32 rows, ranges within what it stages on chip)");
         return ws_launch;
     }
     if (L.fmt == G4C_WFMT_BF16_RS) {
@@ -331,7 +344,7 @@
     if ((rc = stage_heads(io, L))) return rc;
     if (L.row_count == 0) return G4C_OK;
     if ((rc = stage_node(io, L))) return rc;
-    L.p.n_tiles = (L.agg && !L.row_split) ? L.io_n_tiles : (int)((L.row_count + 31) / 32);
+    L.p.n_tiles = (L.agg && !L.row_split && io->tile_rows) ? L.io_n_tiles : (int)((L.row_count + 31) / 32);
     const LaunchFn launch = choose(L);
     if (!launch) return G4C_EUNSUPPORTED;
     if (L.p.n_tiles == 0) return G4C_OK;
@@ -344,3 +357,4 @@
 extern "C" int g4c_mlp_shapes_enable(int on) { return knob(g_shapes, on, 1); }
 extern "C" int g4c_mlp_last_kernel(void) { return g_last.kernel; }
 extern "C" int g4c_mlp_last_shape(void) { return g_last.shape; }
+extern "C" int g4c_mlp_last_row_ranges(void) { return g_last.ranges; }
diff --git a/graphs4cfd_amd/csrc/mlp_ws.hip b/graphs4cfd_amd/csrc/mlp_ws.hip
--- a/graphs4cfd_amd/csrc/mlp_ws.hip
+++ b/graphs4cfd_amd/csrc/mlp_ws.hip
@@ -492,6 +492,7 @@
     int M, row_base, n_tiles;
     int *range_flag;
     int range_slot;
+    const int *wg_rows, *wg_seg;
 };
 struct WsKernArgs {
     WsArgs a;
@@ -519,13 +520,17 @@
 }
 
 constexpr int G4C_WS_SP1_MINW = 2;
-template <bool AGG, bool DIRECT, bool ADDS, int SP, int NL, bool XB16, bool AB16, bool NODE, bool DENSE, bool TRACK, bool PRE>
+constexpr int WS_ANY_MAX_SEG = 2048;
+constexpr int WS_ANY_MAX_PAIRS = 256;
+template <bool AGG, bool DIRECT, bool ADDS, int SP, int NL, bool XB16, bool AB16, bool NODE, bool DENSE, bool TRACK, bool PRE, bool ANY = false>
 __device__ __forceinline__ void ws_body(const WsKernArgs &ka) {
     const WsArgs &p = ka.a;
     const int n_pairs = ka.n_pairs;
     static_assert((SP == 1 || SP == 2) && (NL == 2 || NL == 3) && (SP == 1 || !XB16) && (SP == 1 || !AB16) && (ADDS || !AB16) &&
                   (!NODE || (AGG && SP == 2)) && (TRACK || SP == 2), "mlp_ws_kernel: unsupported instantiation");
     static_assert(!PRE || (AGG && DIRECT && ADDS && SP == 2 && NL == 3 && !NODE && TRACK), "mlp_ws_pre_kernel: unsupported instantiation");
+    static_assert(!ANY || (AGG && ADDS && SP == 2 && !DENSE && !PRE), "mlp_ws_any_kernel: unsupported instantiation");
+    constexpr bool DP = DENSE || ANY;
     typedef typename std::conditional<AB16, u32x2, f32x4>::type AddV;
     __shared__ __attribute__((aligned(16))) __bf16 sP[2 * TILE_BF16];
     __shared__ __attribute__((aligned(16))) float sF[2 * FIN];
@@ -537,6 +542,8 @@
     __shared__ __attribute__((aligned(16))) float sCarry[NP];
     __shared__ __attribute__((aligned(16))) float sBiasN[NODE ? 3 * NP : 4];
     __shared__ __attribute__((aligned(16))) float sGBN[NODE ? 2 * NP : 4];
+    __shared__ int sOff[ANY ? WS_ANY_MAX_SEG + 2 : 1];
+    __shared__ int sCur[ANY ? WS_ANY_MAX_PAIRS + 2 : 1];
 
     const int tid = threadIdx.x, lane = tid & 63;
     const int wave = __builtin_amdgcn_readfirstlane(tid >> 6);
@@ -550,7 +557,11 @@
     {
         const int G = gridDim.x, b = blockIdx.x;
         const int slot = (G & 7) ? b : (b & 7) * (G >> 3) + (b >> 3);
-        if constexpr (DENSE) {
+        if constexpr (ANY) {
+            R0 = __builtin_amdgcn_readfirstlane(p.wg_rows[slot]);
+            R1 = __builtin_amdgcn_readfirstlane(p.wg_rows[slot + 1]);
+            p_begin = 0; p_end = (R1 - R0 + 63) >> 6;
+        } else if constexpr (DENSE) {
             const int n_seg = p.M / KU;
             R0 = __builtin_amdgcn_readfirstlane((int)(((long long)slot * n_seg) / G) * KU);
             R1 = __builtin_amdgcn_readfirstlane((int)(((long long)(slot + 1) * n_seg) / G) * KU);
@@ -566,7 +577,7 @@
 
     auto load_meta = [&](int pair) __attribute__((always_inline)) {
         Meta m;
-        if constexpr (DENSE) {
+        if constexpr (DP) {
             if (pair > p_end - 1) pair = p_end - 1;
             const int r0 = R0 + 64 * pair, nr = (R1 - r0) < 64 ? (R1 - r0) : 64;
             m.r0[0] = r0; m.n[0] = nr < 32 ? nr : 32; m.r0[1] = r0 + 32; m.n[1] = nr - m.n[0];
@@ -613,7 +624,7 @@
         const int *ix = (k == 0) ? ix0 : (k == 1 ? ix1 : ix2);
         const int *addr = ix ? ix + gr : dummy;
         int j = 0, ts = 0;
-        if (AGG && !DENSE) {
+        if (AGG && !DP) {
             const int q = tid - 256;
             const bool is_seg = q >= 0 && q < 2 * (SEGCAP + 1);
             ts = is_seg && q >= SEGCAP + 1 ? 1 : 0;
@@ -627,7 +638,7 @@
     };
     auto store_tables = [&](int v, int it) __attribute__((always_inline)) {
         if (tid < 192) sIdx[it & 1][tid] = v;
-        if (AGG && !DENSE && tid >= 256 && tid < 256 + 2 * (SEGCAP + 1)) sSeg[it & 3][tid - 256] = v;
+        if (AGG && !DP && tid >= 256 && tid < 256 + 2 * (SEGCAP + 1)) sSeg[it & 3][tid - 256] = v;
     };
     auto gather_x = [&](const Meta &m, int ring, int t, f32x4 (&xt)[2], unsigned (&raw)[2][2]) __attribute__((always_inline)) {
         {
@@ -678,7 +689,7 @@
 
     Meta m0 = fix_meta(load_meta(p_begin)), m1 = fix_meta(load_meta(p_begin + 1)), m2 = fix_meta(load_meta(p_begin + 2));
     auto meta_at = [&](int pair_, const Meta &carried) __attribute__((always_inline)) {
-        if constexpr (DENSE) { asm volatile("" : "+s"(pair_)); return load_meta(pair_); }
+        if constexpr (DP) { asm volatile("" : "+s"(pair_)); return load_meta(pair_); }
         else return carried;
     };
     {
@@ -695,6 +706,19 @@
     if (tid < NL * NP) sBias[tid] = p.b[tid];
     if (tid < NP) sZero[tid] = 0.f;
     if (tid < 2 * NP) sGB[tid] = p.gamma ? (tid < NP ? p.gamma[tid] : p.beta[tid - NP]) : 0.f;
+    if constexpr (ANY) {
+        const int G = gridDim.x, bx = blockIdx.x;
+        const int slot = (G & 7) ? bx : (bx & 7) * (G >> 3) + (bx >> 3);
+        const int SG0 = __builtin_amdgcn_readfirstlane(p.wg_seg[slot]), nseg = __builtin_amdgcn_readfirstlane(p.wg_seg[slot + 1]) - SG0;
+        for (int i = tid; i < nseg; i += 512) {
+            const int b = p.seg_off[SG0 + i] - R0, e = p.seg_off[SG0 + i + 1] - R0;
+            sOff[i] = b;
+            if (i == nseg - 1) sOff[nseg] = e;
+            for (int k = (b + 63) >> 6; (k << 6) < e; ++k)
+                if (k > 0) sCur[k] = i;
+        }
+        if (tid == 0) { sCur[0] = 0; sCur[p_end] = nseg; sCur[WS_ANY_MAX_PAIRS + 1] = SG0; }
+    }
     if constexpr (NODE) {
         const NodeParams &q = ka.q;
         if (tid < NL * NP) sBiasN[tid] = q.b[tid];
@@ -916,6 +940,43 @@
                     if (hi && rest) *reinterpret_cast<f32x4 *>(sCarry + c4) = a;
                 }
             };
+            if constexpr (ANY) {
+                const int base = itp << 6, nr = mm.n[0] + mm.n[1];
+                const int lo = sCur[itp], hi = sCur[itp + 1], sg0 = sCur[WS_ANY_MAX_PAIRS + 1];
+                for (int s = lo + (tid >> 5); s < hi; s += 16) {
+                    const int b = sOff[s] - base, e = sOff[s + 1] - base;
+                    if (b >= 0) reduce_rows(fA, b, e, sg0 + s);
+                }
+                if (wave == 7) {
+                    const bool trail = lane >= 32;
+                    const int s = trail ? hi : lo;
+                    const int b = sOff[s] - base, e = sOff[s + 1] - base;
+                    const bool on = trail ? b < nr : (lo < hi && b < 0);
+                    if (on) {
+                        const int rb = b > 0 ? b : 0, re = trail ? nr : e;
+                        f32x4 a = *reinterpret_cast<const f32x4 *>((b < 0 ? sCarry : sZero) + c4);
+                        for (int r0 = rb; r0 < re; r0 += 8) {
+                            f32x4 v[8];
+#pragma unroll
+                            for (int u = 0; u < 8; ++u) v[u] = *reinterpret_cast<const f32x4 *>(fA + (r0 + u < re ? r0 + u : re - 1) * HS + c4);
+#pragma unroll
+                            for (int u = 0; u < 8; ++u) {
+                                const bool in = r0 + u < re;
+#pragma unroll
+                                for (int el = 0; el < 4; ++el) a[el] += in ? v[u][el] : 0.f;
+                            }
+                        }
+                        if (trail) {
+                            *reinterpret_cast<f32x4 *>(sCarry + c4) = a;
+                        } else {
+                            const int len = sOff[s + 1] - sOff[s];
+                            if (p.agg_mean) a = g4c::mean_div4(a, len > 1 ? len : 1);
+                            *reinterpret_cast<f32x4 *>(p.agg + (long long)(sg0 + s) * p.agg_ld + c4) = a;
+                        }
+                    }
+                }
+                return;
+            }
             if constexpr (DENSE) {
                 typedef std::integral_constant<int, 4> K4; typedef std::integral_constant<int, 5> K5; typedef std::integral_constant<int, 6> K6;
                 typedef std::integral_constant<int, 7> K7; typedef std::integral_constant<int, 8> K8;
@@ -973,7 +1034,7 @@
         for (int it = 0, pair = p_begin; pair < p_end; ++pair, ++it) {
             WS_STAMP(0);
             Meta m3raw;
-            if constexpr (!DENSE) m3raw = load_meta(pair + 3);
+            if constexpr (!DP) m3raw = load_meta(pair + 3);
             const int tv = load_tables(meta_at(pair + 2, m2));
             f32x4 ntA[2], ntB[2], nsA[2];
             AddV nadA[2][2];
@@ -1003,7 +1064,7 @@
             start_values_pre(accB, ntB, adB);
             asm volatile("" : "+v"(accB[0]), "+v"(accB[1]) :: "memory");
             Meta m3;
-            if constexpr (!DENSE) m3 = fix_meta(m3raw);
+            if constexpr (!DP) m3 = fix_meta(m3raw);
             store_tables(tv, it + 2);
             WS_STAMP(8);
             if (!(G4C_WS_ABLATE & 256)) ln_tail(meta_at(pair, m0), it);
@@ -1012,13 +1073,13 @@
             WS_STAMP(15);
             if (!(G4C_WS_ABLATE & 128)) agg_tail(meta_at(pair, m0), it);
             WS_STAMP(10);
-            if constexpr (!DENSE) { m0 = m1; m1 = m2; m2 = m3; }
+            if constexpr (!DP) { m0 = m1; m1 = m2; m2 = m3; }
         }
     } else
     for (int it = 0, pair = p_begin; pair < p_end; ++pair, ++it) {
         WS_STAMP(0);
         Meta m3raw;
-        if constexpr (!DENSE) m3raw = load_meta(pair + 3);
+        if constexpr (!DP) m3raw = load_meta(pair + 3);
         const int tv = load_tables(meta_at(pair + 2, m2));
         WS_STAMP(1);
         widen_x(xr[1], rawB);
@@ -1059,7 +1120,7 @@
         start_values(accA, accA1, nadA);
         asm volatile("" : "+v"(accA[0]), "+v"(accA[1]) :: "memory");
         Meta m3;
-        if constexpr (!DENSE) m3 = fix_meta(m3raw);
+        if constexpr (!DP) m3 = fix_meta(m3raw);
         gather_x(meta_at(pair + 1, m1), (it + 1) & 1, 1, xr[1], rawB);
         store_tables(tv, it + 2);
         WS_STAMP(8);
@@ -1075,7 +1136,7 @@
         WS_STAMP(16);
         if constexpr (SP != 1) gather_adds(1, (it + 1) & 1, adB);
         WS_STAMP(10);
-        if constexpr (!DENSE) { m0 = m1; m1 = m2; m2 = m3; }
+        if constexpr (!DP) { m0 = m1; m1 = m2; m2 = m3; }
     }
 
     if constexpr (NODE) {
@@ -1087,8 +1148,15 @@
         nc.sBiasN = sBiasN; nc.sGBN = sGBN; nc.fA = fA; nc.fB = fB; nc.oA = oA; nc.oB = oB;
 #pragma unroll
         for (int ks = 0; ks < 4; ++ks) { nc.paA[ks] = paA[ks]; nc.paB[ks] = paB[ks]; }
-        const int t1 = 2 * p_end < p.n_tiles ? 2 * p_end : p.n_tiles;
-        const int S0 = __builtin_amdgcn_readfirstlane(p.tile_seg[2 * p_begin]), S1 = __builtin_amdgcn_readfirstlane(p.tile_seg[t1]);
+        int S0, S1;
+        if constexpr (ANY) {
+            const int G = gridDim.x, bx = blockIdx.x;
+            const int slot = (G & 7) ? bx : (bx & 7) * (G >> 3) + (bx >> 3);
+            S0 = __builtin_amdgcn_readfirstlane(p.wg_seg[slot]); S1 = __builtin_amdgcn_readfirstlane(p.wg_seg[slot + 1]);
+        } else {
+            const int t1 = 2 * p_end < p.n_tiles ? 2 * p_end : p.n_tiles;
+            S0 = __builtin_amdgcn_readfirstlane(p.tile_seg[2 * p_begin]); S1 = __builtin_amdgcn_readfirstlane(p.tile_seg[t1]);
+        }
         const NodeParams q = node_params_now();
         node_phase<SP, NL, TRACK>(nc, p.agg, p.agg_ld, q, S0, S1);
     }
@@ -1112,7 +1180,21 @@
     ws_body<true, true, true, 2, 3, false, false, false, DENSE, true, true>(ka);
 }
 
-#if defined(G4C_WS_ISA_ONLY) && G4C_WS_ISA_ONLY == 2
+template <int NL, bool NODE, bool TRACK>
+__global__ __launch_bounds__(512, 2) void mlp_ws_any_kernel(const WsKernArgs ka) {
+    ws_body<true, true, true, 2, NL, false, false, NODE, false, TRACK, false, true>(ka);
+}
+
+#if defined(G4C_WS_ISA_ONLY) && G4C_WS_ISA_ONLY == 3
+template __global__ void mlp_ws_any_kernel<3, false, true>(const WsKernArgs);
+template __global__ void mlp_ws_any_kernel<3, false, false>(const WsKernArgs);
+template __global__ void mlp_ws_any_kernel<3, true, true>(const WsKernArgs);
+template __global__ void mlp_ws_any_kernel<3, true, false>(const WsKernArgs);
+template __global__ void mlp_ws_any_kernel<2, false, true>(const WsKernArgs);
+template __global__ void mlp_ws_any_kernel<2, false, false>(const WsKernArgs);
+template __global__ void mlp_ws_any_kernel<2, true, true>(const WsKernArgs);
+template __global__ void mlp_ws_any_kernel<2, true, false>(const WsKernArgs);
+#elif defined(G4C_WS_ISA_ONLY) && G4C_WS_ISA_ONLY == 2
 template __global__ void mlp_ws_pre_kernel<true>(const WsKernArgs);
 template __global__ void mlp_ws_pre_kernel<false>(const WsKernArgs);
 #elif defined(G4C_WS_ISA_ONLY)
@@ -1151,12 +1233,19 @@
     return ((uintptr_t)p.b & 15) == 0 && p.M < (1LL << 31);
 }
 
+bool ws_any_takes(const Launch &L) {
+    const Params &p = L.p;
+    if (!L.f16x2 || !L.agg || L.pre || !p.wg_rows || !p.wg_seg || p.src[0].idx || p.n_add != 2 || p.out_bf16) return false;
+    if (p.agg_deg >= 4 && p.agg_deg <= 8) return false;
+    return p.n_wg >= 1 && p.wg_pairs >= 1 && p.wg_pairs <= WS_ANY_MAX_PAIRS && p.wg_max_seg >= 1 && p.wg_max_seg <= WS_ANY_MAX_SEG;
+}
+
 int ws_launch(const Launch &L, hipStream_t st, Ran &ran) {
     const Params &p = L.p;
     if (L.pre) {
         const bool dense = p.agg_deg >= 4 && p.agg_deg <= 8;
         const int n_pairs = dense ? (int)((p.M + 63) / 64) : (p.n_tiles + 1) / 2;
-        const int n_wg = g4c::cu_count();
+        const int n_wg = g4c::ws_grid();
         const dim3 grid(n_pairs < n_wg ? n_pairs : n_wg), blk(512);
         ran.kernel = G4C_KERNEL_MLP_WS_PRE;
         WsArgs a{};
@@ -1174,10 +1263,11 @@
         return g4c::check_launch("g4c_mlp_run (ws, first layer precomputed)");
     }
     const bool agg = L.agg, round1 = L.round1, node = L.has_node;
+    G4C_REQUIRE(!agg || p.tile_rows || ws_any_takes(L), G4C_EUNSUPPORTED, "g4c_mlp_run (ws): the fused aggregation without tiles of whole segments");
     const bool dense = agg && !node && p.agg_deg >= 4 && p.agg_deg <= 8;
     const int n_pairs = dense ? (int)((p.M + 63) / 64) : (p.n_tiles + 1) / 2;
     ran.kernel = G4C_KERNEL_MLP_WS;
-    const int n_wg = g4c::cu_count() * (round1 ? G4C_WS_SP1_MINW / 2 : 1);
+    const int n_wg = g4c::ws_grid() * (round1 ? G4C_WS_SP1_MINW / 2 : 1);
     const dim3 grid(n_pairs < n_wg ? n_pairs : n_wg), blk(512);
     const bool direct = p.src[0].idx == nullptr, adds = p.n_add == 2, two = p.n_layers == 2, xb16 = p.src[0].bf16 != 0;
     const bool ab16 = adds && p.add[0].bf16 != 0;
@@ -1195,6 +1285,19 @@
     a.M = (int)p.M; a.row_base = (int)p.row_base; a.n_tiles = p.n_tiles;
     a.range_flag = p.range_certified ? nullptr : p.range_flag; a.range_slot = p.range_slot;
     const WsKernArgs ka{a, n_pairs, L.node};
+    if (ws_any_takes(L)) {
+        WsKernArgs kr = ka;
+        kr.a.wg_rows = p.wg_rows; kr.a.wg_seg = p.wg_seg;
+        const dim3 grid_r(p.n_wg);
+        ran.ranges = p.n_wg;
+#define G4C_WS_ANY(NL, NODE)                                                                                   \
+    do { if (cert) mlp_ws_any_kernel<NL, NODE, false><<<grid_r, blk, 0, st>>>(kr);                             \
+         else mlp_ws_any_kernel<NL, NODE, true><<<grid_r, blk, 0, st>>>(kr); } while (0)
+        if (node) { if (two) G4C_WS_ANY(2, true); else G4C_WS_ANY(3, true); }
+        else { if (two) G4C_WS_ANY(2, false); else G4C_WS_ANY(3, false); }
+#undef G4C_WS_ANY
+        return g4c::check_launch(node ? "g4c_mlp_run (ws, upd, row ranges)" : "g4c_mlp_run (ws, row ranges)");
+    }
     if (node) {
         G4C_REQUIRE(agg && !round1 && adds, G4C_EUNSUPPORTED, "g4c_mlp_run (upd): needs the hoisted f16x3 message launch with the fused aggregation");
 #define G4C_WS_NODE(DIRECT, NL)                                                                                                        \
diff --git a/graphs4cfd_amd/csrc/plan.cpp b/graphs4cfd_amd/csrc/plan.cpp
--- a/graphs4cfd_amd/csrc/plan.cpp
+++ b/graphs4cfd_amd/csrc/plan.cpp
@@ -41,6 +41,59 @@
         s = e;
     }
     return nt;
+}
+
+extern "C" int64_t g4c_plan_row_ranges(const int32_t *off, int32_t n_seg, int32_t n_wg, int32_t *wg_rows, int32_t *wg_seg,
+                                       int32_t *max_seg) {
+    G4C_REQUIRE(off && wg_rows && wg_seg && max_seg && n_seg >= 0 && n_wg >= 1 && off[0] == 0, G4C_EINVAL, "g4c_plan_row_ranges: bad arguments");
+    for (int32_t s = 0; s < n_seg; ++s)
+        G4C_REQUIRE(off[s + 1] >= off[s], G4C_EINVAL, "g4c_plan_row_ranges: offsets decrease at segment %d", s);
+    const int64_t rows = off[n_seg];
+    *max_seg = 0;
+    if (rows == 0) {
+        for (int32_t i = 0; i <= n_wg; ++i) { wg_rows[i] = 0; wg_seg[i] = i == 0 ? 0 : n_seg; }
+        *max_seg = n_seg;
+        return 0;
+    }
+    std::vector<int32_t> nxt((size_t)n_seg + 1), need((size_t)n_seg + 1);
+    auto count = [&](int64_t cap) -> int64_t {
+        int32_t e = n_seg;
+        need[(size_t)n_seg] = 0; nxt[(size_t)n_seg] = n_seg;
+        for (int32_t s = n_seg - 1; s >= 0; --s) {
+            while ((int64_t)off[e] - off[s] > cap) --e;
+            if (e == s) { if (off[s + 1] - off[s] > cap) return -1; }
+            nxt[(size_t)s] = off[e] == off[n_seg] ? n_seg : e;
+            need[(size_t)s] = off[s] == off[n_seg] ? 0 : 1 + need[(size_t)nxt[(size_t)s]];
+        }
+        return need[0];
+    };
+    int64_t lo = (rows + 64LL * n_wg - 1) / (64LL * n_wg), hi = (rows + 63) / 64;
+    while (lo < hi) {
+        const int64_t mid = (lo + hi) / 2, c = count(64 * mid);
+        if (c >= 0 && c <= n_wg) hi = mid; else lo = mid + 1;
+    }
+    const int64_t P = lo, cap = 64 * P;
+    count(cap);
+    int32_t s = 0;
+    wg_rows[0] = 0; wg_seg[0] = 0;
+    for (int32_t i = 0; i < n_wg; ++i) {
+        const int32_t left = n_wg - i;
+        int32_t e;
+        if (off[s] == off[n_seg]) e = n_seg;
+        else if (left == 1) e = n_seg;
+        else {
+            const int64_t want = off[s] + (rows - off[s] + left - 1) / left;
+            e = (int32_t)(std::lower_bound(off + s, off + n_seg + 1, (int32_t)want) - off);
+            if (e > s && off[e] > want && want - off[e - 1] <= off[e] - want && off[e - 1] > off[s]) --e;
+            if (e > nxt[(size_t)s]) e = nxt[(size_t)s];
+            while (off[e] == off[s] || need[(size_t)e] > left - 1) ++e;
+            if (off[e] == off[n_seg]) e = n_seg;
+        }
+        wg_rows[i + 1] = off[e]; wg_seg[i + 1] = e;
+        *max_seg = std::max(*max_seg, e - s);
+        s = e;
+    }
+    return P;
 }
 
 extern "C" int64_t g4c_plan_pool_edge_ordered(const int64_t *idx_hr_to_lr, int64_t n_hr, const int64_t *edge_index,
diff --git a/graphs4cfd_amd/ops.py b/graphs4cfd_amd/ops.py
--- a/graphs4cfd_amd/ops.py
+++ b/graphs4cfd_amd/ops.py
@@ -1,5 +1,6 @@
 from __future__ import annotations
 
+import contextlib
 import ctypes as C
 import os
 from typing import List, Optional, Sequence, Tuple
@@ -1393,10 +1394,48 @@
     return (1 if agg_mean else 0) | (csr.uniform_deg << 8)
 
 
-def _set_agg(io, csr: CsrPlan, agg_out: Tensor, agg_mean: bool) -> None:
-    t_rows, t_seg, nt = csr.tiles()
-    io.tile_rows, io.tile_seg, io.seg_off, io.n_tiles = _lib.ptr(t_rows), _lib.ptr(t_seg), _lib.ptr(csr.off), nt
+DENSE_ANY = os.environ.get("G4C_DENSE_ANY", "1") != "0"
+
+
+@contextlib.contextmanager
+def dense_any(on: bool):
+    global DENSE_ANY
+    was, DENSE_ANY = DENSE_ANY, DENSE_ANY and on
+    try:
+        yield
+    finally:
+        DENSE_ANY = was
+
+
+def ws_grid(t: Tensor) -> int:
+    n = C.c_int32(0)
+    _lib.check(_lib.load().g4c_mlp_ws_grid(t.data_ptr(), C.byref(n)))
+    return int(n.value)
+
+
+def _ranges_only(packed: "PackedMLP", sources: Sequence["Source"], csr: CsrPlan, agg_out: Tensor) -> bool:
+    if not (DENSE_ANY and packed.split == "f16x2" and packed.desc.n_layers in (2, 3) and packed.seg_widths == (128,) and len(sources) == 3):
+        return False
+    x, adds = sources[0], sources[1:]
+    if x.additive or x.index is not None or x.segments is not None or x.tensor.dtype != torch.float32 or x.col0 % 4 or _ld(x.tensor) % 4 or x.tensor.data_ptr() % 16:
+        return False
+    if any(not s.additive or s.width != 128 or s.tensor.dtype != torch.float32 or s.col0 % 4 or _ld(s.tensor) % 4 or s.tensor.data_ptr() % 16 for s in adds):
+        return False
+    return csr.perm is None and agg_out.dtype == torch.float32 and csr.row_ranges(ws_grid(agg_out)) is not None
+
+
+def _set_agg(io, csr: CsrPlan, agg_out: Tensor, agg_mean: bool, ranges: bool = False) -> None:
+    tiles = csr.tiles()
+    if tiles is not None:
+        io.tile_rows, io.tile_seg, io.n_tiles = _lib.ptr(tiles[0]), _lib.ptr(tiles[1]), tiles[2]
+    elif not (ranges and DENSE_ANY and csr.row_ranges(ws_grid(agg_out)) is not None):
+        raise ValueError("fused aggregation: the rows must be in segment order with segments of at most 32 rows")
+    io.seg_off = _lib.ptr(csr.off)
     io.agg, io.agg_ld, io.agg_mode = _lib.ptr(agg_out), _ld(agg_out), _agg_mode(agg_mean, csr)
+    if ranges and DENSE_ANY and not 4 <= csr.uniform_deg <= 8:
+        plan = csr.row_ranges(ws_grid(agg_out))
+        if plan is not None:
+            io.wg_rows, io.wg_seg, io.n_wg, io.wg_pairs, io.wg_max_seg = _lib.ptr(plan[0]), _lib.ptr(plan[1]), int(plan[0].numel()) - 1, plan[2], plan[3]
 
 
 def _set_heads(io, head_outs: Sequence[Tensor]) -> None:
@@ -1443,7 +1482,7 @@
         raise ValueError(f"{n_heads} head outputs for a packing with {upd.n_heads} heads")
     io = _lib.g4c_mlp_io_t(row_count=n_rows, out=_lib.ptr(e_out), out_ld=128 if e_out is None else _ld(e_out), upd=C.pointer(upd.desc),
                            v=_lib.ptr(v), v_ld=_ld(v), v_act=act, v_out=_lib.ptr(v_out), v_out_ld=_ld(v_out))
-    _set_agg(io, csr, agg, agg_mean)
+    _set_agg(io, csr, agg, agg_mean, ranges=True)
     if n_heads:
         _set_heads(io, head_outs)
     in_b = 4.0 * 128 * (n_rows * (2 if store_rows else 1) + n_t * (2 + n_heads))
@@ -1559,7 +1598,8 @@
                 a.additive, a.w = 2, packed.narrow_w[j].data_ptr()
             j += 1
     fusable = (agg is not None and FUSE_AGG and packed.precision in ("bf16x6", "bf16") and packed.n_out == 128 and head_outs is None
-               and rows is None and out_idx32 is None and resid is None and n_rows == agg[0].n and agg[0].tiles() is not None)
+               and rows is None and out_idx32 is None and resid is None and n_rows == agg[0].n
+               and (agg[0].tiles() is not None or _ranges_only(packed, sources, agg[0], agg[1])))
     if not store_rows and not fusable:
         raise ValueError("store_rows=False needs an aggregation the launch can fuse (ops.can_fuse_aggregation)")
     reduce_after = None
@@ -1601,7 +1641,7 @@
         _lib.require_hip(agg_out)
         if agg_out.dtype not in (torch.float32, torch.bfloat16):
             raise TypeError(f"aggregate: expected float32 (or bfloat16 on the row-split kernel), got {agg_out.dtype}")
-        _set_agg(io, csr, agg_out, agg_mean)
+        _set_agg(io, csr, agg_out, agg_mean, ranges=packed.split == "f16x2" and save is None)
         if agg_out.dtype == torch.bfloat16:
             io.agg_mode |= 1 << 16
         out_b = 0 if not store_rows else packed.n_out * (2 if out.dtype == torch.bfloat16 else 4)
diff --git a/graphs4cfd_amd/partition.py b/graphs4cfd_amd/partition.py
--- a/graphs4cfd_amd/partition.py
+++ b/graphs4cfd_amd/partition.py
@@ -373,6 +373,10 @@
         return self.impl.new(m.n_own[level - 1] + m.n_halo[level - 1], self.width, m.device)
 
     def forward(self) -> torch.Tensor:
+        with ops.dense_any(False):
+            return self._forward()
+
+    def _forward(self) -> torch.Tensor:
         m, impl = self.mesh, self.impl
         level = 1
         v = self._buf(1)
diff --git a/graphs4cfd_amd/partition_remus.py b/graphs4cfd_amd/partition_remus.py
--- a/graphs4cfd_amd/partition_remus.py
+++ b/graphs4cfd_amd/partition_remus.py
@@ -300,6 +300,10 @@
         self.program, self.mesh, self.impl, self.xch = program, mesh, impl, exchanger
 
     def forward(self) -> torch.Tensor:
+        with ops.dense_any(False):
+            return self._forward()
+
+    def _forward(self) -> torch.Tensor:
         impl, x = self.impl, self.xch
         e, a, ax = impl.encode()
         fresh = {l: False for l in e}
diff --git a/graphs4cfd_amd/plan.py b/graphs4cfd_amd/plan.py
--- a/graphs4cfd_amd/plan.py
+++ b/graphs4cfd_amd/plan.py
@@ -20,6 +20,7 @@
     max_deg: int
     uniform_deg: int = 0
     _tiles: object = False
+    _ranges: object = None
 
     def tiles(self, max_rows: int = 32):
         if self._tiles is False:
@@ -34,6 +35,34 @@
                     dev = self.off.device
                     self._tiles = (_upload(rows[: nt + 1].copy(), dev), _upload(seg[: nt + 1].copy(), dev), nt)
         return self._tiles
+
+    def row_ranges(self, n_wg: int):
+        if self._ranges is None:
+            self._ranges = {}
+        if n_wg not in self._ranges:
+            out = None
+            if self.perm is None and self.n > 0 and n_wg >= 1:
+                off = np.ascontiguousarray(_host_i64(self.off).astype(np.int32))
+                rows, seg, pairs, max_seg = row_ranges_host(off, n_wg)
+                if pairs <= RANGE_MAX_PAIRS and max_seg <= RANGE_MAX_SEGS:
+                    dev = self.off.device
+                    out = (_upload(rows, dev), _upload(seg, dev), pairs, max_seg)
+            self._ranges[n_wg] = out
+        return self._ranges[n_wg]
+
+
+RANGE_MAX_PAIRS, RANGE_MAX_SEGS = 256, 2048
+
+
+def row_ranges_host(off: np.ndarray, n_wg: int):
+    lib = _lib.load()
+    off = np.ascontiguousarray(off, dtype=np.int32)
+    rows, seg = np.empty(n_wg + 1, np.int32), np.empty(n_wg + 1, np.int32)
+    max_seg = C.c_int32(0)
+    pairs = int(lib.g4c_plan_row_ranges(off.ctypes.data, int(off.shape[0]) - 1, n_wg, rows.ctypes.data, seg.ctypes.data, C.byref(max_seg)))
+    if pairs < 0:
+        _lib.check(pairs)
+    return rows, seg, pairs, int(max_seg.value)
 
 
 @dataclass
diff --git a/include/g4c.h b/include/g4c.h
--- a/include/g4c.h
+++ b/include/g4c.h
@@ -129,6 +129,8 @@
     int32_t *range_flag;
     int32_t save_dtype;
     int32_t mul_dtype;
+    const int32_t *wg_rows, *wg_seg;
+    int32_t n_wg, wg_pairs, wg_max_seg;
 } g4c_mlp_io_t;
 
 int g4c_mlp_run(const g4c_mlp_t *mlp , const g4c_src_t *srcs , int32_t n_src, int64_t n_rows,
@@ -151,6 +153,7 @@
 #define G4C_KERNEL_MLP_WS_CERT 8
 #define G4C_KERNEL_MLP_WS_PRE 9
 int g4c_mlp_last_kernel(void);
+int g4c_mlp_last_row_ranges(void);
 
 #define G4C_TILE_SHAPE_GENERIC 0
 #define G4C_TILE_SHAPE_NODE 1
@@ -161,6 +164,9 @@
 
 int64_t g4c_plan_tiles(const int32_t *off , int32_t n_seg, int32_t max_rows, int32_t *tile_rows ,
                        int32_t *tile_seg , int64_t capacity);
+int64_t g4c_plan_row_ranges(const int32_t *off , int32_t n_seg, int32_t n_wg, int32_t *wg_rows ,
+                            int32_t *wg_seg , int32_t *max_seg );
+int g4c_mlp_ws_grid(const void *device_ptr, int32_t *n_wg);
 
 int g4c_layer_norm(const float *x, int32_t x_ld, int64_t n_rows, int32_t width, const float *gamma, const float *beta, float eps,
                    int32_t act, float *out, int32_t out_ld, void *stream);
```

After: 266.8 (median of 6 runs). 1.01x the previous value.
